# zengyan-97/X2-VLM

Hardware: AMD Instinct MI355X
Metric: image-text pairs/sec (fwd+bwd) X2VLM-base 224px bs=64/GPU (higher is better)
Workload: dtype bf16

## Files before the change

### include/x2vlm_hip.h

```cpp
#ifndef X2VLM_HIP_H
#define X2VLM_HIP_H
#include <stdint.h>
#ifdef __cplusplus
extern "C" {
#endif

const char* x2_last_error(void);
int x2_abi_version(void);
int x2_device_cus(void);
int x2_tune(int key, int value);
int x2_tune_get(int key);

int x2_gemm_nt(const void* A, const void* B, void* C, int M, int N, int K, int lda, int ldb, int ldc,
               const float* bias, const float* gamma, const float* resid, int ldr, void* aux, int ldaux,
               int act, int out_f32, unsigned drop_thr16, unsigned drop_seed, float drop_scale, const unsigned* drop_epoch,
               const float* rowscale, float* colsum, void* stream);

int x2_gemm_nt_dgelu_colparts(const void* A, const void* B, void* C, int M, int N, int K, int lda, int ldb, int ldc,
                              const void* aux, int ldaux, float* colparts, int* nrows_out, void* stream);
int x2_gemm_nt_splitk(const void* A, const void* B, float* C, int M, int N, int K, int lda, int ldb, int ldc,
                      int slices, float* ws, long ws_floats, void* stream);

int x2_gemm_tn_grouped(const int64_t* problems, int count, int accumulate, int split, float* ws, long ws_floats,
                       void* stream);

typedef struct X2AttnArgs {
  const void *Q, *K, *V, *O, *dO;
  void *Out, *dQ, *dK, *dV, *dS;
  float *LSE, *Delta;
  long q_bs, q_rs, k_bs, k_rs, v_bs, v_rs, o_bs, o_rs;
  long dq_bs, dq_rs, dk_bs, dk_rs, dv_bs, dv_rs, do_bs, do_rs;
  int B, Bkv, H, Lq, Lk;
  float scale;
  const float* bias;  int bias_ld;
  const float* biasT; int biasT_ld;
  const float* mask;  int mask_ld;
  const int* kv_idx;
  const int* seq_off; const int* seq_ids;
  int ds_ld;
  unsigned drop_thr16, drop_seed; float drop_scale;
  int dbg;
  int head_dim;
  const unsigned* drop_epoch;
  int grid_nx, grid_ny, grid_nz, grid_map;
  int phase;
  float* ws; long ws_floats;
  float* colsum_ws;
} X2AttnArgs;
int x2_attn_fwd(const X2AttnArgs* args, void* stream);
int x2_attn_bwd(const X2AttnArgs* args, void* stream);
int x2_attn_bwd_one_pass(const X2AttnArgs* args);

int x2_layernorm_fwd(const float* x, const float* w, const float* b, void* y_bf16, float* y_f32, float* mean,
                     float* rstd, int rows, int D, float eps, int period, unsigned drop_thr16, unsigned drop_seed,
                     float drop_scale, const unsigned* drop_epoch, void* stream);
int x2_layernorm_bwd(const void* dy , int dy_is_bf16, const float* x, const float* mean, const float* rstd, const float* w,
                     const float* dres, float* dx, void* dx_bf16, float* dw, float* db, float* dcol, int rows, int D,
                     int period, unsigned in_thr16, unsigned in_seed, float in_scale, unsigned out_thr16,
                     unsigned out_seed, float out_scale, const unsigned* drop_epoch, float* ws ,
                     int defer, int post, const float* post_rowscale, void* stream);
int x2_colsum_bf16(const void* y, float* out, int M, int N, int ld, float* ws , int defer, void* stream);
int x2_reduce_partials(const float* part, int nblk, int nk, int width, float* o0, float* o1, float* o2, void* stream);
int x2_reduce_partials_multi(const int64_t* desc, int count, void* stream);
int x2_layerscale_finish(const int64_t* desc, int count, void* stream);
int x2_rowscale_cast_colsum(const float* dx, const float* rowscale, void* dx_bf16, float* colsum, int M, int D,
                            float* ws , int defer, void* stream);
int x2_cast_bf16(const float* src, void* dst, long n, void* stream);
int x2_cast_transpose_bf16(const float* src, void* dst, void* dstT, int R, int C, int ldt, void* stream);
int x2_cast_transpose_multi(const int64_t* desc, int count, void* stream);
int x2_copy_f32_multi(const int64_t* desc, int count, void* stream);
int x2_patchify(const float* image, void* cols, int B, int R, int ps, void* stream);
int x2_assemble_tokens(const float* patch, const float* cls, float* x, int B, int P, int D, void* stream);
int x2_assemble_tokens_bwd(const float* dx, void* dpatch_bf16, float* dcls, int B, int P, int D, void* stream);
int x2_pool_tokens(float* x, const float* w, int B, int P, int D, int bwd, void* stream);
int x2_relpos_bias(const float* table, const long* index, const long* indexT , float* bias, float* biasT, int N, int H, int ld, int ldT,
                   float scale, void* stream);
int x2_relpos_bias_bwd(const void* dS, const int* inv_off, const int* inv_pos, float* dtable, int B, int N, int H, int ld,
                       int T, float* ws, int slices, void* stream);

int x2_embed_fwd(const long* ids, const float* word, const float* pos, const float* type0, float* out, int R, int L,
                 int D, void* stream);
int x2_embed_bwd(const long* ids, const float* g, float* dword, float* dpos, float* dtype0, int R, int L, int D,
                 float* scratch, void* stream);
int x2_gather_rows(const float* src, const int* idx, float* dst, void* dst_bf16, int R, long len, void* stream);
int x2_scatter_rows(const float* src, const int* idx, float* dst, int R, int D, long len, void* stream);
int x2_linear_f32(const float* A, const float* B, float* C, const float* bias, const float* alpha_ptr, float alpha,
                  int M, int N, int K, long sam, long sak, long sbn, long sbk, long ldc, int accumulate,
                  int ksplit ,
                  float* ws , void* stream);
int x2_l2norm(const float* x, const float* dy, float* out, int R, int D, int bwd, void* stream);
int x2_ce_fwd(const float* logits, long ld, const long* labels, int R, int C, float* lse, float* loss_row, float* out2,
              void* stream);
int x2_ce_bwd(const float* logits, long ld, const long* labels, const float* lse, const float* g, const float* stat,
              float gscale, int R, int C, float* dl_f32, void* dl_bf16, long ldd, void* stream);
int x2_mlm_ce_fwd(const void* X, const void* E, const float* bias, const long* labels, int R, int Vp, int V, int Hd,
                  int ldx, int lde, float* part, float* zlab, void* stream);
int x2_ce_combine(const float* part, int chunks, const float* zlab, const long* labels, int R, float* lse, float* loss_row,
                  float* out2, void* stream);
int x2_mlm_ce_bwd(const void* X, const void* E, const float* bias, const long* labels, const float* lse, const float* g,
                  const float* stat, float gscale, int R, int Vp, int V, int Hd, int ldx, int lde, void* dl_bf16, long ldd,
                  void* stream);
int x2_mask_tokens(const long* text_ids, const long* text_atts, int B, int L, const unsigned char* is_subword, int vocab,
                   const unsigned* words, int words_ld, unsigned seed, const unsigned* epoch, double mask_prob, int max_masks,
                   double skipgram_prb, int skipgram_size, int mask_whole_word, long cls_id, long mask_id, long pad_id, long pad_mask,
                   long* text_ids_masked, long* masked_pos, long* masked_ids, void* stream);
int x2_sample_negatives(const float* sim, int n, const long* group, const float* u, int* out, void* stream);
int x2_additive_mask(const long* atts, float* out, int S, int L, int Lp, float neg, void* stream);

int x2_attn_fwd_mask2d(const X2AttnArgs* args, const float* mask2d, int mask2d_ld, void* stream);
int x2_attn_bwd_mask2d(const X2AttnArgs* args, const float* mask2d, int mask2d_ld, void* stream);
int x2_additive_mask2d(const long* m, float* out, int S, int L, int Lp, float neg, void* stream);
int x2_embed_fwd_pid(const long* ids, const long* pids, const float* word, const float* pos, const float* type0, float* out, int R, int D,
                     void* stream);
int x2_embed_bwd_pid(const long* ids, const long* pids, const float* g, float* dword, float* dpos, float* dtype0, int R, int L, int D,
                     float* scratch, void* stream);
int x2_mlm_ls_fwd(const void* X, const void* E, const float* bias, const long* labels, long ignore, int R, int Vp, int V, int Hd, int ldx,
                  int lde, float* part, float* sumz, float* zlab, float* zign, void* stream);
int x2_ls_combine(const float* part, const float* sumz, int chunks, const float* zlab, const float* zign, const long* labels, const float* w,
                  int R, int V, long ignore, float ls, float* lse, float* kl_row, float* out2, void* stream);
int x2_mlm_ls_bwd(const void* X, const void* E, const float* bias, const long* labels, const float* w, const float* lse, const float* g,
                  const float* stat, float gscale, float ls, long ignore, int R, int Vp, int V, int Hd, int ldx, int lde, void* dl_bf16,
                  long ldd, void* stream);
int x2_kv_csr(const int* kv, int S, int Bi, int* off, int* order, void* stream);
int x2_tail_index(const int* ineg, const int* tneg, const long* text_atts , const long* image_atts , int B, int L,
                  int T, int with_match, int* t_idx, int* kv, long* atts_out , long* enc_out , void* stream);
int x2_droppath_rows(const float* rates, unsigned seed, const unsigned* epoch, int depth, int B, int T, float* out, void* stream);
int x2_frame_mean(const float* x, const float* pos, const float* dy, float* out, float* dpos, int Bc, int F, int T, int D, int bwd,
                  void* stream);
int x2_gelu_f32(const float* x, const float* dy, float* out, long n, void* stream);
int x2_colsum_f32(const float* x, float* out, int M, int N, void* stream);

int x2_grad_norm(const void* table, int ntensors, int nblocks, float max_norm, float* partial, float* out2, void* stream);
int x2_adamw_multi(const void* table, int ntensors, int nblocks, const float* lr, const float* wd, int ngroups, float b1,
                   float b2, float eps, const float* clip2 , void* stream);

int x2_comm_unique_id(void* out128);
int x2_comm_init(const void* id128, int rank, int world, void** comm_out);
int x2_comm_info(void* comm, int* rank, int* world);
int x2_comm_allreduce_bucket(void* comm, void* buf, long count, int dtype, int average, void* done_event, void* stream);
int x2_comm_allgather(void* comm, const void* send, void* recv, long count_per_rank, int dtype, void* done_event, void* stream);
int x2_comm_broadcast(void* comm, void* buf, long count, int dtype, int root, void* done_event, void* stream);
int x2_comm_destroy(void* comm);

#ifdef __cplusplus
}
#endif
#endif
```

### probes/ab_step.py

```python
import argparse, importlib, os, sys, tempfile, time
ROOT = os.path.dirname(os.path.dirname(os.path.abspath(__file__)))
sys.path.insert(0, ROOT)
import torch
import bench

ap = argparse.ArgumentParser()
ap.add_argument("--config", default="base")
ap.add_argument("--variants", nargs="+", default=["default:"])
ap.add_argument("--rounds", type=int, default=3)
ap.add_argument("--steps", type=int, default=20)
ap.add_argument("--warmup", type=int, default=4)
args = ap.parse_args()
conf = bench.CONFIGS[args.config]
mp = importlib.import_module("x2-vlm_amd.model_pretrain")
cfgs = importlib.import_module("x2-vlm_amd.configs")
graph = importlib.import_module("x2-vlm_amd.graph")
lib = importlib.import_module("x2-vlm_amd._lib").lib()
dev = torch.device("cuda", 0)
torch.manual_seed(0)
cfg = cfgs.pretrain_config(tempfile.mkdtemp(), conf["size"], conf["res"])
if conf["frames"]:
    cfg.update(video_encoding="avgpool", frame_len=conf["frames"], add_frame_pos=True)
model = mp.XVLM(config=cfg, load_vision_params=False, load_text_params=False, pretraining=True).to(dev).train()
batch = {k: v.to(dev) for k, v in bench.synthetic_batch(0, conf["batch"], 30, conf["res"], frames=conf["frames"]).items()}
variants = []
for v in args.variants:
    name, _, kv = v.partition(":")
    env = {}
    knobs = {}
    for item in filter(None, kv.split(",")):
        k, val = item.split("=")
        if k.isdigit():
            knobs[int(k)] = int(val)
        else:
            env[k] = val.replace("+", ",")
    variants.append((name, knobs, env))
res = {n: [] for n, _, _ in variants}
for rnd in range(args.rounds):
    for name, knobs, env in variants:
        for k, val in knobs.items():
            assert lib.x2_tune(k, val) == 0, lib.x2_last_error()
        old = {k: os.environ.get(k) for k in env}
        os.environ.update(env)
        step = graph.SegmentedStep(model, batch, warmup=1)
        assert step.mode == "hipgraph-segments", step.error
        for _ in range(args.warmup):
            step()
        torch.cuda.synchronize()
        a, b = torch.cuda.Event(enable_timing=True), torch.cuda.Event(enable_timing=True)
        a.record()
        for _ in range(args.steps):
            step()
        b.record()
        torch.cuda.synchronize()
        res[name].append(a.elapsed_time(b) / args.steps)
        del step
        for k in knobs:
            lib.x2_tune(k, 0)
        for k, v in old.items():
            if v is None:
                os.environ.pop(k, None)
            else:
                os.environ[k] = v
        import gc
        gc.collect()
        torch.cuda.empty_cache()
print("config %s, %d steps per timing, ms per step by round:" % (args.config, args.steps))
for name, knobs, env in variants:
    r = res[name]
    print("  %-12s %-28s %s   min %.3f  mean %.3f" % (name, ",".join("%s=%s" % kv for kv in list(knobs.items()) + list(env.items())) or "-",
                                                       " ".join("%.3f" % x for x in r), min(r), sum(r) / len(r)))
```

### x2-vlm_amd/_lib.py

```python
import ctypes as C
import os

import torch

_HERE = os.path.dirname(os.path.abspath(__file__))
LIB_PATH = os.environ.get("X2VLM_HIP_LIB") or os.path.join(_HERE, "libx2vlm_hip.so")

P, I, L, F, U = C.c_void_p, C.c_int, C.c_long, C.c_float, C.c_uint


class AttnArgs(C.Structure):
    _fields_ = [(n, P) for n in ("Q", "K", "V", "O", "dO", "Out", "dQ", "dK", "dV", "dS", "LSE", "Delta")] + \
               [(n, L) for n in ("q_bs", "q_rs", "k_bs", "k_rs", "v_bs", "v_rs", "o_bs", "o_rs",
                                 "dq_bs", "dq_rs", "dk_bs", "dk_rs", "dv_bs", "dv_rs", "do_bs", "do_rs")] + \
               [(n, I) for n in ("B", "Bkv", "H", "Lq", "Lk")] + [("scale", F)] + \
               [("bias", P), ("bias_ld", I), ("biasT", P), ("biasT_ld", I), ("mask", P), ("mask_ld", I),
                ("kv_idx", P), ("seq_off", P), ("seq_ids", P), ("ds_ld", I),
                ("drop_thr16", C.c_uint), ("drop_seed", C.c_uint), ("drop_scale", F), ("dbg", I), ("head_dim", I), ("drop_epoch", P),
                ("grid_nx", I), ("grid_ny", I), ("grid_nz", I), ("grid_map", I),
                ("phase", I), ("ws", P), ("ws_floats", L), ("colsum_ws", P)]


_SIGS = {
    "x2_gemm_nt": [P, P, P, I, I, I, I, I, I, P, P, P, I, P, I, I, I, U, U, F, P, P, P, P],
    "x2_gemm_nt_splitk": [P, P, P, I, I, I, I, I, I, I, P, L, P],
    "x2_gemm_nt_dgelu_colparts": [P, P, P, I, I, I, I, I, I, P, I, P, C.POINTER(I), P],
    "x2_gemm_tn_grouped": [P, I, I, I, P, L, P],
    "x2_attn_fwd": [C.POINTER(AttnArgs), P],
    "x2_attn_bwd": [C.POINTER(AttnArgs), P],
    "x2_layernorm_fwd": [P, P, P, P, P, P, P, I, I, F, I, U, U, F, P, P],
    "x2_layernorm_bwd": [P, I, P, P, P, P, P, P, P, P, P, P, I, I, I, U, U, F, U, U, F, P, P, I, I, P, P],
    "x2_colsum_bf16": [P, P, I, I, I, P, I, P],
    "x2_reduce_partials": [P, I, I, I, P, P, P, P],
    "x2_reduce_partials_multi": [P, I, P],
    "x2_cast_transpose_multi": [P, I, P],
    "x2_copy_f32_multi": [P, I, P],
    "x2_layerscale_finish": [P, I, P],
    "x2_rowscale_cast_colsum": [P, P, P, P, I, I, P, I, P],
    "x2_cast_bf16": [P, P, L, P],
    "x2_cast_transpose_bf16": [P, P, P, I, I, I, P],
    "x2_patchify": [P, P, I, I, I, P],
    "x2_assemble_tokens": [P, P, P, I, I, I, P],
    "x2_assemble_tokens_bwd": [P, P, P, I, I, I, P],
    "x2_pool_tokens": [P, P, I, I, I, I, P],
    "x2_relpos_bias": [P, P, P, P, P, I, I, I, I, F, P],
    "x2_relpos_bias_bwd": [P, P, P, P, I, I, I, I, I, P, I, P],
    "x2_embed_fwd": [P, P, P, P, P, I, I, I, P],
    "x2_embed_bwd": [P, P, P, P, P, I, I, I, P, P],
    "x2_gather_rows": [P, P, P, P, I, L, P],
    "x2_scatter_rows": [P, P, P, I, I, L, P],
    "x2_linear_f32": [P, P, P, P, P, F, I, I, I, L, L, L, L, L, I, I, P, P],
    "x2_l2norm": [P, P, P, I, I, I, P],
    "x2_ce_fwd": [P, L, P, I, I, P, P, P, P],
    "x2_ce_bwd": [P, L, P, P, P, P, F, I, I, P, P, L, P],
    "x2_mlm_ce_fwd": [P, P, P, P, I, I, I, I, I, I, P, P, P],
    "x2_ce_combine": [P, I, P, P, I, P, P, P, P],
    "x2_mlm_ce_bwd": [P, P, P, P, P, P, P, F, I, I, I, I, I, I, P, L, P],
    "x2_sample_negatives": [P, I, P, P, P, P],
    "x2_mask_tokens": [P, P, I, I, P, I, P, I, U, P, C.c_double, I, C.c_double, I, I, L, L, L, L, P, P, P, P],
    "x2_additive_mask": [P, P, I, I, I, F, P],
    "x2_kv_csr": [P, I, I, P, P, P],
    "x2_tail_index": [P, P, P, P, I, I, I, I, P, P, P, P, P],
    "x2_droppath_rows": [P, U, P, I, I, I, P, P],
    "x2_frame_mean": [P, P, P, P, P, I, I, I, I, I, P],
    "x2_gelu_f32": [P, P, P, L, P],
    "x2_grad_norm": [P, I, I, F, P, P, P],
    "x2_adamw_multi": [P, I, I, P, P, I, F, F, F, P, P],
    "x2_colsum_f32": [P, P, I, I, P],
    "x2_attn_fwd_mask2d": [C.POINTER(AttnArgs), P, I, P],
    "x2_attn_bwd_mask2d": [C.POINTER(AttnArgs), P, I, P],
    "x2_additive_mask2d": [P, P, I, I, I, F, P],
    "x2_embed_fwd_pid": [P, P, P, P, P, P, I, I, P],
    "x2_embed_bwd_pid": [P, P, P, P, P, P, I, I, I, P, P],
    "x2_mlm_ls_fwd": [P, P, P, P, L, I, I, I, I, I, I, P, P, P, P, P],
    "x2_ls_combine": [P, P, I, P, P, P, P, I, I, L, F, P, P, P, P],
    "x2_mlm_ls_bwd": [P, P, P, P, P, P, P, P, F, F, L, I, I, I, I, I, I, P, L, P],
}
_COMM_SIGS = {
    "x2_comm_unique_id": [P],
    "x2_comm_init": [P, I, I, C.POINTER(P)],
    "x2_comm_info": [P, C.POINTER(I), C.POINTER(I)],
    "x2_comm_allreduce_bucket": [P, P, L, I, I, P, P],
    "x2_comm_allgather": [P, P, P, L, I, P, P],
    "x2_comm_broadcast": [P, P, L, I, I, P, P],
    "x2_comm_destroy": [P],
}
EXPORTS = sorted(list(_SIGS) + list(_COMM_SIGS) + ["x2_last_error", "x2_abi_version", "x2_device_cus", "x2_tune", "x2_tune_get",
                                                         "x2_attn_bwd_one_pass"])

_lib = None


class X2HipError(RuntimeError):
    pass


def lib():
    global _lib
    if _lib is None:
        if not os.path.exists(LIB_PATH):
            raise X2HipError("HIP extension %s not built: run `python -c 'import __graft_entry__ as g; g.build()'`"
                             % LIB_PATH)
        try:
            h = C.CDLL(LIB_PATH)
        except OSError as e:
            raise X2HipError("cannot load %s: %s" % (LIB_PATH, e))
        for name, sig in list(_SIGS.items()) + list(_COMM_SIGS.items()):
            fn = getattr(h, name)
            fn.argtypes, fn.restype = sig, I
        h.x2_last_error.restype = C.c_char_p
        h.x2_abi_version.restype = I
        h.x2_device_cus.restype = I
        h.x2_tune.argtypes, h.x2_tune.restype = [I, I], I
        h.x2_tune_get.argtypes, h.x2_tune_get.restype = [I], I
        h.x2_attn_bwd_one_pass.argtypes, h.x2_attn_bwd_one_pass.restype = [C.POINTER(AttnArgs)], I
        for kv in filter(None, os.environ.get("X2_TUNE", "").split(",")):
            k, v = kv.split("=")
            if h.x2_tune(int(k), int(v)) != 0:
                raise X2HipError("X2_TUNE=%s: %s" % (kv, h.x2_last_error().decode()))
        _lib = h
    return _lib


_get_device = torch._C._cuda_getDevice if hasattr(torch._C, "_cuda_getDevice") else None
_get_raw_stream = getattr(torch._C, "_cuda_getCurrentRawStream", None)


def raw_stream():
    return _get_raw_stream(_get_device())


def call(name, *args):
    h = _lib or lib()
    rc = getattr(h, name)(*args, _get_raw_stream(_get_device()))
    if rc != 0:
        raise X2HipError("%s failed (%d): %s" % (name, rc, h.x2_last_error().decode()))


def ptr(t):
    return None if t is None else t.data_ptr()
```

### x2-vlm_amd/csrc/gemm.hip

```cpp
#include "x2_common.h"
#include <type_traits>

#define BM 128
#define BN 128
#define BK 64
#define TILE_BYTES (128 * 128)
#define STAGE_BYTES (2 * TILE_BYTES)
#define GEMM_LDS_BYTES (2 * STAGE_BYTES)

struct GemmNT {
  const bf16_t* A; const bf16_t* B; void* C;
  const float* bias; const float* gamma; const float* resid; bf16_t* aux;
  int M, N, K;
  int lda, ldb, ldc, ldr, ldaux;
  int act;
  int out_f32;
  int group_m;
  DropSpec drop;
  const uint32_t* drop_epoch;
  const float* rowscale;
  float* colsum;
  int dbg;
  int ksplit;
  const long* ce_labels;
  const float* ce_lse;
  const float* ce_g;
  const float* ce_stat;
  float* ce_part;
  float* ce_zlab;
  float ce_gscale;
  int ce_C;
  float* ce_sumz;
  float* ce_zign;
  long ce_ignore;
  float ce_ls;
  const float* ce_w;
};

__device__ __forceinline__ void tile_coords(int t, int tiles_m, int tiles_n, int gm, int& tm, int& tn) {
  const int gsz = gm * tiles_n, g = t / gsz, first = g * gm;
  const int rows = min(gm, tiles_m - first), r = t - g * gsz;
  tm = first + r % rows;
  tn = r / rows;
}

__device__ __forceinline__ void st16(void* p, u32x4 v, bool wt) {
  if (wt) asm volatile("global_store_dwordx4 %0, %1, off sc1\n\ts_nop 1" ::"v"(p), "v"(v) : "memory");
  else *reinterpret_cast<u32x4*>(p) = v;
}

#ifdef X2_PROBE
#define NT_DBG(p, bit) (((p).dbg & (bit)) != 0)
static __device__ unsigned long long* g_nt_probe = nullptr;
#define NT_STAMP(i) do { if (g_nt_probe && threadIdx.x == 0) g_nt_probe[(size_t)blockIdx.x * 4 + (i)] = wall_clock64(); } while (0)
#define NT_ABL_DECL(p) const bool abl_dma_ = NT_DBG(p, 32), abl_rd_ = NT_DBG(p, 64), abl_mm_ = NT_DBG(p, 128); bool rd_ = true
#define NT_ABL_NO_DMA(kt) if (abl_dma_ && (kt) >= 2) return
#define NT_ABL_NO_READ() if (!rd_) return
#define NT_ABL_NO_MFMA() if (abl_mm_) return
#define NT_ABL_STEP(kt) if (abl_rd_ && (kt) > 0) rd_ = false
#else
#define NT_ABL_DECL(p)
#define NT_ABL_NO_DMA(kt)
#define NT_ABL_NO_READ()
#define NT_ABL_NO_MFMA()
#define NT_ABL_STEP(kt)
#define NT_DBG(p, bit) false
#define NT_STAMP(i) do { } while (0)
#endif
typedef __attribute__((ext_vector_type(16))) float f32x16;
template <int TM>
__device__ __forceinline__ void epi_stage_half(f32x4 (&acc)[TM][4], int half, bool full, float* stg, int lane) {
  const int frow = lane & 15, fg = lane >> 4;
#pragma unroll
  for (int ii = 0; ii < 2; ++ii)
#pragma unroll
    for (int j = 0; j < 4; ++j)
      if (full || ii == 0) *reinterpret_cast<f32x4*>(stg + (ii * 16 + frow) * 68 + j * 16 + fg * 4) = acc[full ? half * 2 + ii : half * 2][j];
}
template <int RT>
__device__ __forceinline__ void epi_stage_half(f32x16 (&acc)[RT][2], int half, bool, float* stg, int lane) {
  const int row = lane & 31, h = lane >> 5;
#pragma unroll
  for (int tj = 0; tj < 2; ++tj)
#pragma unroll
    for (int g = 0; g < 4; ++g)
      *reinterpret_cast<f32x4*>(stg + row * 68 + tj * 32 + g * 8 + h * 4) =
          f32x4{acc[half][tj][4 * g], acc[half][tj][4 * g + 1], acc[half][tj][4 * g + 2], acc[half][tj][4 * g + 3]};
}
template <int V> struct EpiTraits {
  static constexpr bool generic = V == 4;
  static constexpr int act = V == 2 ? 1 : (V == 3 || V == 10) ? 2 : 0;
  static constexpr bool out_f32 = V == 1 || V == 5 || V == 6 || V == 7;
  static constexpr bool resid = V == 5 || V == 6;
  static constexpr bool scale = V == 6;
  static constexpr bool aux0 = false;
  static constexpr bool drop = V == 5;
  static constexpr bool colsum = false;
  static constexpr bool colparts = V == 10;
};
template <int TM, int VAR, class Acc>
__device__ __forceinline__ void nt_epilogue(const GemmNT& p, Acc& acc, char* smem, int wave, int lane, int mw0, int nw0, int prow = 0) {
  using E = EpiTraits<VAR>;
  const int act = E::generic ? p.act : E::act;
  const bool out_f32 = E::generic ? p.out_f32 != 0 : E::out_f32;
  const bool has_resid = E::generic ? p.resid != nullptr : E::resid;
  const bool has_scale = E::generic ? (p.gamma != nullptr || p.rowscale != nullptr) : E::scale;
  const bool has_aux0 = E::generic ? (p.act == 0 && p.aux != nullptr) : E::aux0;
  const bool has_drop = (E::generic || E::drop) ? p.drop.thr16 != 0 : false;
  const bool has_colsum = E::generic ? p.colsum != nullptr : (E::colsum && p.colsum != nullptr);
  float* stg = reinterpret_cast<float*>(smem) + wave * (32 * 68);
  const int er = lane >> 3, ec = (lane & 7) * 8;
  const int n = nw0 + ec;
  const bool nok = n < p.N;
  float bb[8], gg[8];
#pragma unroll
  for (int e = 0; e < 8; ++e) { bb[e] = 0.f; gg[e] = 1.f; }
  if (nok && p.bias) { const float4 b0 = *reinterpret_cast<const float4*>(p.bias + n), b1 = *reinterpret_cast<const float4*>(p.bias + n + 4);
    bb[0] = b0.x; bb[1] = b0.y; bb[2] = b0.z; bb[3] = b0.w; bb[4] = b1.x; bb[5] = b1.y; bb[6] = b1.z; bb[7] = b1.w; }
  if (nok && has_scale && p.gamma) { const float4 g0 = *reinterpret_cast<const float4*>(p.gamma + n), g1 = *reinterpret_cast<const float4*>(p.gamma + n + 4);
// ... 26 lines not shown
    }
    epi_stage_half(acc, half, full, stg, lane);
#pragma unroll
    for (int rr = 0; rr < 4; ++rr) {
      if (!full && rr >= 2) continue;
      const int row = rr * 8 + er;
      const int m = mw0 + half * 32 + row;
      const float4 a0 = *reinterpret_cast<const float4*>(stg + row * 68 + ec), a1 = *reinterpret_cast<const float4*>(stg + row * 68 + ec + 4);
      if (m >= p.M || !nok) continue;
      float v[8] = {a0.x + bb[0], a0.y + bb[1], a0.z + bb[2], a0.w + bb[3], a1.x + bb[4], a1.y + bb[5], a1.z + bb[6], a1.w + bb[7]};
      if constexpr (VAR == 8) {
        const long lab = p.ce_labels[m];
        float mx = -INFINITY;
#pragma unroll
        for (int e = 0; e < 8; ++e) mx = n + e < p.ce_C ? fmaxf(mx, v[e]) : mx;
        mx = fmaxf(mx, __shfl_xor(mx, 1, 64)); mx = fmaxf(mx, __shfl_xor(mx, 2, 64)); mx = fmaxf(mx, __shfl_xor(mx, 4, 64));
        float se = 0.f;
#pragma unroll
        for (int e = 0; e < 8; ++e) {
          se += n + e < p.ce_C ? __expf(v[e] - mx) : 0.f;
          if ((long)(n + e) == lab) p.ce_zlab[m] = v[e];
        }
        se += __shfl_xor(se, 1, 64); se += __shfl_xor(se, 2, 64); se += __shfl_xor(se, 4, 64);
        if ((lane & 7) == 0) *reinterpret_cast<float2*>(p.ce_part + ((size_t)m * (p.N >> 6) + (nw0 >> 6)) * 2) = float2{mx, se};
        continue;
      }
      if constexpr (VAR == 11) {
        const long lab = p.ce_labels[m];
        float mx = -INFINITY, sz = 0.f;
#pragma unroll
        for (int e = 0; e < 8; ++e) { mx = n + e < p.ce_C ? fmaxf(mx, v[e]) : mx; sz += n + e < p.ce_C ? v[e] : 0.f; }
        mx = fmaxf(mx, __shfl_xor(mx, 1, 64)); mx = fmaxf(mx, __shfl_xor(mx, 2, 64)); mx = fmaxf(mx, __shfl_xor(mx, 4, 64));
        sz += __shfl_xor(sz, 1, 64); sz += __shfl_xor(sz, 2, 64); sz += __shfl_xor(sz, 4, 64);
        float se = 0.f;
#pragma unroll
        for (int e = 0; e < 8; ++e) {
          se += n + e < p.ce_C ? __expf(v[e] - mx) : 0.f;
          if ((long)(n + e) == lab) p.ce_zlab[m] = v[e];
          if ((long)(n + e) == p.ce_ignore) p.ce_zign[m] = v[e];
        }
        se += __shfl_xor(se, 1, 64); se += __shfl_xor(se, 2, 64); se += __shfl_xor(se, 4, 64);
        if ((lane & 7) == 0) {
          *reinterpret_cast<float2*>(p.ce_part + ((size_t)m * (p.N >> 6) + (nw0 >> 6)) * 2) = float2{mx, se};
          p.ce_sumz[(size_t)m * (p.N >> 6) + (nw0 >> 6)] = sz;
        }
        continue;
      }
      if constexpr (VAR == 12) {
        const long lab = p.ce_labels[m];
        const bool live = lab >= 0 && lab != p.ce_ignore;
        const float conf = 1.f - p.ce_ls, sm = p.ce_ls / (float)(p.ce_C - 2), qsum = conf + sm * (float)(p.ce_C - 2);
        const float sc = live ? p.ce_gscale * p.ce_g[0] * p.ce_w[m] / (p.ce_stat[1] + 1e-5f) : 0.f, l = p.ce_lse[m];
#pragma unroll
        for (int e = 0; e < 8; ++e) {
          const long c = n + e;
          const float q = c == lab ? conf : (c == p.ce_ignore ? 0.f : sm);
          v[e] = c < p.ce_C ? (qsum * __expf(v[e] - l) - q) * sc : 0.f;
        }
        st16(reinterpret_cast<bf16_t*>(p.C) + (size_t)m * p.ldc + n,
             u32x4{pack_bf16(v[0], v[1]), pack_bf16(v[2], v[3]), pack_bf16(v[4], v[5]), pack_bf16(v[6], v[7])}, false);
        continue;
      }
      if constexpr (VAR == 9) {
        const long lab = p.ce_labels[m];
        const float sc = lab >= 0 ? p.ce_gscale * p.ce_g[0] / p.ce_stat[1] : 0.f, l = p.ce_lse[m];
#pragma unroll
        for (int e = 0; e < 8; ++e) v[e] = n + e < p.ce_C ? (__expf(v[e] - l) - ((long)(n + e) == lab ? 1.f : 0.f)) * sc : 0.f;
        st16(reinterpret_cast<bf16_t*>(p.C) + (size_t)m * p.ldc + n,
             u32x4{pack_bf16(v[0], v[1]), pack_bf16(v[2], v[3]), pack_bf16(v[4], v[5]), pack_bf16(v[6], v[7])}, false);
        continue;
      }
      if (act == 1) {
        st16(p.aux + (size_t)m * p.ldaux + n, u32x4{pack_bf16(v[0], v[1]), pack_bf16(v[2], v[3]), pack_bf16(v[4], v[5]), pack_bf16(v[6], v[7])}, wt);
#pragma unroll
        for (int r = 0; r < 8; ++r) v[r] = gelu_f(v[r]);
      } else if (act == 2) {
#pragma unroll
        for (int r = 0; r < 4; ++r) { v[2 * r] *= dgelu_f(bf_lo(pre[rr][r])); v[2 * r + 1] *= dgelu_f(bf_hi(pre[rr][r])); }
      } else if (has_aux0) {
        st16(p.aux + (size_t)m * p.ldaux + n, u32x4{pack_bf16(v[0], v[1]), pack_bf16(v[2], v[3]), pack_bf16(v[4], v[5]), pack_bf16(v[6], v[7])}, wt);
      }
      if (has_drop) {
        float dm[4];
        drop_mul4(drop_, (uint32_t)m * (uint32_t)p.N + (uint32_t)n, dm);
        v[0] *= dm[0]; v[1] *= dm[1]; v[2] *= dm[2]; v[3] *= dm[3];
        drop_mul4(drop_, (uint32_t)m * (uint32_t)p.N + (uint32_t)n + 4u, dm);
        v[4] *= dm[0]; v[5] *= dm[1]; v[6] *= dm[2]; v[7] *= dm[3];
      }
      if (has_scale) {
        const float rs_ = p.rowscale ? p.rowscale[m] : 1.f;
#pragma unroll
        for (int r = 0; r < 8; ++r) v[r] *= gg[r] * rs_;
      }
      if (has_resid) {
        v[0] += r0[rr].x; v[1] += r0[rr].y; v[2] += r0[rr].z; v[3] += r0[rr].w;
        v[4] += r1[rr].x; v[5] += r1[rr].y; v[6] += r1[rr].z; v[7] += r1[rr].w;
      }
      if (has_colsum || E::colparts) {
#pragma unroll
        for (int r = 0; r < 8; ++r) cs[r] += v[r];
      }
      if (out_f32) {
        float* c = reinterpret_cast<float*>(p.C) + (size_t)m * p.ldc + n;
        st16(c, u32x4{__float_as_uint(v[0]), __float_as_uint(v[1]), __float_as_uint(v[2]), __float_as_uint(v[3])}, wt);
        st16(c + 4, u32x4{__float_as_uint(v[4]), __float_as_uint(v[5]), __float_as_uint(v[6]), __float_as_uint(v[7])}, wt);
      } else {
        st16(reinterpret_cast<bf16_t*>(p.C) + (size_t)m * p.ldc + n,
             u32x4{pack_bf16(v[0], v[1]), pack_bf16(v[2], v[3]), pack_bf16(v[4], v[5]), pack_bf16(v[6], v[7])}, wt);
      }
    }
  }
  if constexpr (E::colparts) {
#pragma unroll
    for (int e = 0; e < 8; ++e) { cs[e] += __shfl_xor(cs[e], 8, 64); cs[e] += __shfl_xor(cs[e], 16, 64); cs[e] += __shfl_xor(cs[e], 32, 64); }
    if (er == 0 && nok) {
      float* dst = p.colsum + (size_t)prow * p.N + n;
      *reinterpret_cast<float4*>(dst) = float4{cs[0], cs[1], cs[2], cs[3]};
      *reinterpret_cast<float4*>(dst + 4) = float4{cs[4], cs[5], cs[6], cs[7]};
    }
  }
  if (has_colsum) {
#pragma unroll
    for (int e = 0; e < 8; ++e) { cs[e] += __shfl_xor(cs[e], 8, 64); cs[e] += __shfl_xor(cs[e], 16, 64); cs[e] += __shfl_xor(cs[e], 32, 64); }
    if (er == 0 && nok) {
#pragma unroll
      for (int e = 0; e < 8; ++e) atomicAdd(p.colsum + n + e, cs[e]);
    }
  }
}

template <int TM, int VAR, class Acc>
__device__ __forceinline__ void nt_epilogue_f4(const GemmNT& p, Acc& acc, char* smem, int wave, int lane, int mw0, int nw0) {
  using E = EpiTraits<VAR>;
  static_assert(!E::generic && E::out_f32 && E::act == 0 && VAR <= 6, "nt_epilogue_f4: feature sets 1, 5, 6");
  const bool has_drop = E::drop ? p.drop.thr16 != 0 : false;
  float* stg = reinterpret_cast<float*>(smem) + wave * (32 * 68);
  const int er = lane >> 4, ec = (lane & 15) * 4;
  const int n = nw0 + ec;
  const bool nok = n < p.N;
  float bb[4] = {0.f, 0.f, 0.f, 0.f}, gg[4] = {1.f, 1.f, 1.f, 1.f};
  if (nok && p.bias) { const float4 b0 = *reinterpret_cast<const float4*>(p.bias + n); bb[0] = b0.x; bb[1] = b0.y; bb[2] = b0.z; bb[3] = b0.w; }
  if (E::scale && nok && p.gamma) { const float4 g0 = *reinterpret_cast<const float4*>(p.gamma + n); gg[0] = g0.x; gg[1] = g0.y; gg[2] = g0.z; gg[3] = g0.w; }
  const DropSpec drop_ = drop_at_epoch(p.drop, p.drop_epoch);
#pragma unroll
  for (int half = 0; half < (TM + 1) / 2; ++half) {
    const bool full = half * 2 + 1 < TM;
    float4 rs[4][2];
    const int nc = nok ? n : 0;
    if (E::resid) {
#pragma unroll
      for (int rr = 0; rr < 4; ++rr) {
        if (!full && rr >= 2) continue;
#pragma unroll
        for (int h = 0; h < 2; ++h) {
          const int mc = min(mw0 + half * 32 + rr * 8 + h * 4 + er, p.M - 1);
          rs[rr][h] = *reinterpret_cast<const float4*>(p.resid + (size_t)mc * p.ldr + nc);
        }
      }
    }
    epi_stage_half(acc, half, full, stg, lane);
#pragma unroll
    for (int rr = 0; rr < 4; ++rr) {
      if (!full && rr >= 2) continue;
#pragma unroll
      for (int h = 0; h < 2; ++h) {
        const int row = rr * 8 + h * 4 + er;
        const int m = mw0 + half * 32 + row;
        const float4 a0 = *reinterpret_cast<const float4*>(stg + row * 68 + ec);
        if (m >= p.M || !nok) continue;
        float v[4] = {a0.x + bb[0], a0.y + bb[1], a0.z + bb[2], a0.w + bb[3]};
        if (has_drop) {
          float dm[4];
          drop_mul4(drop_, (uint32_t)m * (uint32_t)p.N + (uint32_t)n, dm);
          v[0] *= dm[0]; v[1] *= dm[1]; v[2] *= dm[2]; v[3] *= dm[3];
        }
        if (E::scale) {
          const float rs_ = p.rowscale ? p.rowscale[m] : 1.f;
#pragma unroll
          for (int r = 0; r < 4; ++r) v[r] *= gg[r] * rs_;
        }
        if (E::resid) { v[0] += rs[rr][h].x; v[1] += rs[rr][h].y; v[2] += rs[rr][h].z; v[3] += rs[rr][h].w; }
        st16(reinterpret_cast<float*>(p.C) + (size_t)m * p.ldc + n,
             u32x4{__float_as_uint(v[0]), __float_as_uint(v[1]), __float_as_uint(v[2]), __float_as_uint(v[3])}, false);
      }
    }
  }
}

template <int TM, int VAR, bool F4 = false>
__global__ __launch_bounds__(256, 2) void gemm_nt_kernel(GemmNT p) {
  constexpr int BMT = 32 * TM;
  if constexpr (VAR == 7) {
    const int koff = blockIdx.y * p.ksplit;
    p.A += koff; p.B += koff;
    p.K = min(p.ksplit, p.K - koff);
    p.C = reinterpret_cast<float*>(p.C) + (size_t)blockIdx.y * p.M * p.ldc;
  }
  constexpr int A_BYTES = BMT * 128, STG = A_BYTES + TILE_BYTES;
  extern __shared__ __attribute__((aligned(16))) char smem[];
  const int tid = threadIdx.x, lane = tid & 63;
  const int wave = __builtin_amdgcn_readfirstlane(tid >> 6);
  const int wm = wave >> 1, wn = wave & 1;
  const int tiles_n = (p.N + BN - 1) / BN, tiles_m = (p.M + BMT - 1) / BMT;
  int tm, tn;
  tile_coords(xcd_remap(blockIdx.x, gridDim.x), tiles_m, tiles_n, p.group_m, tm, tn);
  const int m0 = tm * BMT, n0 = tn * BN;

  const bf16_t* srcA[TM]; const bf16_t* srcB[4];
#pragma unroll
  for (int i = 0; i < TM; ++i) {
    const int q = i * 256 + tid, row = q >> 3, c = (q & 7) ^ (row & 7);
    int ra = m0 + row; ra = ra < p.M ? ra : p.M - 1;
    srcA[i] = p.A + (size_t)ra * p.lda + c * 8;
  }
#pragma unroll
  for (int i = 0; i < 4; ++i) {
    const int q = i * 256 + tid, row = q >> 3, c = (q & 7) ^ (row & 7);
    int rb = n0 + row; rb = rb < p.N ? rb : p.N - 1;
    srcB[i] = p.B + (size_t)rb * p.ldb + c * 8;
  }
  auto stage = [&](int kt, int buf) {
    char* base = smem + buf * STG;
#pragma unroll
    for (int i = 0; i < TM; ++i) glds16(srcA[i] + (size_t)kt * BK, base + (i * 256 + wave * 64) * 16);
#pragma unroll
    for (int i = 0; i < 4; ++i) glds16(srcB[i] + (size_t)kt * BK, base + A_BYTES + (i * 256 + wave * 64) * 16);
  };

  f32x4 acc[TM][4];
#pragma unroll
  for (int i = 0; i < TM; ++i)
#pragma unroll
    for (int j = 0; j < 4; ++j) acc[i][j] = f32x4{0.f, 0.f, 0.f, 0.f};

  const uint32_t lds0 = lds_addr(smem);
  const int frow = lane & 15, fg = lane >> 4, fsw = lane & 7;
  const uint32_t offA = (uint32_t)((wm * 16 * TM + frow) * 128);
  const uint32_t offB = (uint32_t)(A_BYTES + (wn * 64 + frow) * 128);

  const int nk = p.K / BK;
  bf16x8 a0[TM], b0[4], a1[TM], b1[4];
  auto frags = [&](uint32_t sb, int ks, bf16x8 (&a)[TM], bf16x8 (&b)[4]) {
    const uint32_t cs = (uint32_t)(((ks * 4 + fg) ^ fsw) << 4);
#pragma unroll
    for (int j = 0; j < 4; ++j) b[j] = lds_read_b128(sb + offB + j * 2048 + cs);
#pragma unroll
    for (int i = 0; i < TM; ++i) a[i] = lds_read_b128(sb + offA + i * 2048 + cs);
  };
  auto mma = [&](bf16x8 (&a)[TM], bf16x8 (&b)[4], auto first, auto last) {
#pragma unroll
    for (int t = decltype(first)::value; t < decltype(last)::value; ++t)
      acc[t >> 2][t & 3] = __builtin_amdgcn_mfma_f32_16x16x32_bf16(b[t & 3], a[t >> 2], acc[t >> 2][t & 3], 0, 0, 0);
  };
  using I0 = std::integral_constant<int, 0>; using I1 = std::integral_constant<int, 1>; using IN = std::integral_constant<int, 4 * TM>;
  auto step = [&](int kt, auto refill, auto has_next) {
    mma(a0, b0, I0{}, I1{});
// ... 535 lines not shown
extern "C" int x2_tune_get(int key) {
  if (key >= 9 && key <= 15) return g_tune_x[key - 8];
  if (key < 0 || key >= 8) return -1;
  return g_tune[key];
}

static int nt256_plan(int M, int N, double* eff) {
  const int cus = x2_cus(), tiles_n = (N + 255) / 256;
  const double ideal = (double)M * N / (512.0 * 256.0 * cus);
  int best = 8; double best_cost = 1e30;
  for (int t = 8; t >= 5; --t) {
    const long tiles = (long)((M + 32 * t - 1) / (32 * t)) * tiles_n;
    const double cost = (double)((tiles + cus - 1) / cus) * t / 16.0;
    if (cost < best_cost - 1e-9) { best_cost = cost; best = t; }
  }
  if (eff) *eff = ideal / best_cost;
  return best;
}
template <int TMW, int V>
static void launch_nt256(const GemmNT& p, hipStream_t stream) {
  static bool raised = false;
  if (!raised) {
    (void)hipFuncSetAttribute(reinterpret_cast<const void*>(gemm_nt256_kernel<TMW, V>), hipFuncAttributeMaxDynamicSharedMemorySize, N2_LDS_BYTES);
    raised = true;
  }
  const int tiles = ((p.M + 32 * TMW - 1) / (32 * TMW)) * ((p.N + 255) / 256);
  hipLaunchKernelGGL((gemm_nt256_kernel<TMW, V>), dim3(tiles), dim3(512), N2_LDS_BYTES, stream, p);
}
template <int V>
static void launch_nt256s3(const GemmNT& p, hipStream_t stream) {
  static bool raised = false;
  if (!raised) {
    (void)hipFuncSetAttribute(reinterpret_cast<const void*>(gemm_nt256s3_kernel<V, true>), hipFuncAttributeMaxDynamicSharedMemorySize, N3_LDS_BYTES);
    (void)hipFuncSetAttribute(reinterpret_cast<const void*>(gemm_nt256s3_kernel<V, false>), hipFuncAttributeMaxDynamicSharedMemorySize, N3_LDS_BYTES);
    raised = true;
  }
  const int tiles = ((p.M + 159) / 160) * ((p.N + 255) / 256);
  if (g_tune_x[2] == 2) hipLaunchKernelGGL((gemm_nt256s3_kernel<V, false>), dim3(tiles), dim3(512), N3_LDS_BYTES, stream, p);
  else hipLaunchKernelGGL((gemm_nt256s3_kernel<V, true>), dim3(tiles), dim3(512), N3_LDS_BYTES, stream, p);
}
template <int V>
static void launch_nt256_h(const GemmNT& p, int tmw, hipStream_t stream) {
  switch (tmw) {
    case 5: if (g_tune_x[2] == 1) launch_nt256<5, V>(p, stream); else launch_nt256s3<V>(p, stream); break;
    case 6: launch_nt256<6, V>(p, stream); break;
    case 7: launch_nt256<7, V>(p, stream); break;
    default: launch_nt256<8, V>(p, stream); break;
  }
}

template <int RT0, int RT1, int V, int NST>
static void launch_nt_pp(const GemmNT& p, hipStream_t stream) {
  constexpr int lds = NST * ((RT0 + RT1) * 4096 + 2 * PP_BHALF);
  static bool raised = false;
  if (!raised) {
    (void)hipFuncSetAttribute(reinterpret_cast<const void*>(gemm_nt_pp_kernel<RT0, RT1, V, NST>), hipFuncAttributeMaxDynamicSharedMemorySize, lds);
    raised = true;
  }
  constexpr int BMT = 32 * (RT0 + RT1);
  const int tiles = ((p.M + BMT - 1) / BMT) * ((p.N + 255) / 256);
  hipLaunchKernelGGL((gemm_nt_pp_kernel<RT0, RT1, V, NST>), dim3(tiles), dim3(512), lds, stream, p);
}
template <int V>
static void launch_nt_pp_h(const GemmNT& p, int h, hipStream_t stream) {
  switch (h) {
    case 3: launch_nt_pp<1, 2, V, 3>(p, stream); break;
    case 4: if (g_tune_x[2] == 1) launch_nt_pp<2, 2, V, 2>(p, stream); else launch_nt_pp<2, 2, V, 3>(p, stream); break;
    case 5: if (g_tune_x[2] == 1) launch_nt_pp<2, 3, V, 2>(p, stream); else launch_nt_pp<2, 3, V, 3>(p, stream); break;
    default: launch_nt_pp<3, 3, V, 2>(p, stream); break;
  }
}

template <int TM, int V, bool F4>
static void launch_nt(const GemmNT& p, int tiles, hipStream_t stream) {
  constexpr int lds = 2 * (32 * TM * 128 + TILE_BYTES);
  static bool raised = false;
  if (lds > 65536 && !raised) {
    (void)hipFuncSetAttribute(reinterpret_cast<const void*>(gemm_nt_kernel<TM, V, F4>), hipFuncAttributeMaxDynamicSharedMemorySize, lds);
    raised = true;
  }
  hipLaunchKernelGGL((gemm_nt_kernel<TM, V, F4>), dim3(tiles), dim3(256), lds, stream, p);
}

extern "C" int x2_gemm_nt(const void* A, const void* B, void* C, int M, int N, int K, int lda, int ldb, int ldc,
                          const float* bias, const float* gamma, const float* resid, int ldr, void* aux, int ldaux,
                          int act, int out_f32, unsigned drop_thr16, unsigned drop_seed, float drop_scale, const unsigned* drop_epoch,
                          const float* rowscale, float* colsum, void* stream) {
  X2_REQUIRE(M > 0 && N > 0 && K > 0, "x2_gemm_nt: empty problem M=%d N=%d K=%d", M, N, K);
  X2_REQUIRE(drop_thr16 < 65536u, "x2_gemm_nt: drop_thr16=%u", drop_thr16);
  X2_REQUIRE(K % BK == 0, "x2_gemm_nt: K=%d must be a multiple of %d", K, BK);
  X2_REQUIRE(N % 8 == 0, "x2_gemm_nt: N=%d must be a multiple of 8", N);
  X2_REQUIRE(lda % 8 == 0 && ldb % 8 == 0 && ldc % 8 == 0, "x2_gemm_nt: leading dims must keep 16-byte rows");
  X2_REQUIRE(act == 0 || aux, "x2_gemm_nt: act=%d needs aux", act);
  X2_REQUIRE((!resid || ldr % 4 == 0) && (!aux || ldaux % 8 == 0), "x2_gemm_nt: ldr/ldaux alignment");
  GemmNT p{(const bf16_t*)A, (const bf16_t*)B, C, bias, gamma, resid, (bf16_t*)aux, M, N, K, lda, ldb, ldc, ldr, ldaux, act, out_f32,
           g_tune[0] > 0 ? g_tune[0] : 8, DropSpec{drop_thr16, drop_seed, drop_scale}, drop_epoch, rowscale, colsum, g_tune[2], 0};
  int var = 4;
  {
    const bool plain = !gamma && !rowscale && !drop_thr16 && !colsum;
    if (g_tune[6] == 1) var = 4;
    else if (act == 1 && !out_f32 && !resid && plain) var = 2;
    else if (act == 2 && !out_f32 && !resid && plain) var = 3;
    else if (act == 0 && !aux && !resid && plain) var = out_f32 ? 1 : 0;
    else if (act == 0 && !aux && resid && out_f32 && !gamma && !rowscale && !colsum) var = 5;
    else if (act == 0 && !aux && resid && out_f32 && gamma && !drop_thr16 && !colsum) var = 6;
  }
  double eff256 = 0.0;
  int tmw = nt256_plan(M, N, &eff256);
  if (g_tune[3] >= 5 && g_tune[3] <= 8) tmw = g_tune[3];
  const bool light = var == 0 || var == 1;
  bool auto256 = (light || K >= 2048) && eff256 * 100.0 >= (g_tune_x[1] > 0 ? g_tune_x[1] : 80) && !(resid && M < 8192);
  if (g_tune_x[3] != 1) {
    if ((var == 5 || var == 6) && M >= 8192 && eff256 * 100.0 >= (g_tune_x[1] > 0 ? g_tune_x[1] : 80)) auto256 = true;
    if (var == 2 && eff256 * 100.0 >= 90.0) auto256 = true;
  }
  const bool use256 = var != 4 && N % 8 == 0 && (g_tune[1] == 3 || ((g_tune[1] == 0 || g_tune[1] == 4) && g_tune[3] == 0 && auto256));
  const bool pp_ok = var != 4 && ((size_t)(M - 1) * lda + K) * 2 < (1ull << 31) && ((size_t)(N - 1) * ldb + K) * 2 < (1ull << 31);
  int pp_h = 0;
  if (g_tune_x[7] >= 3 && g_tune_x[7] <= 6) pp_h = g_tune_x[7];
  else if (g_tune_x[7] == 0 && g_tune[1] == 0 && g_tune[3] == 0 && !use256 && K >= 2048 && (var == 0 || var == 1 || var == 5)) {
    const int cus = x2_cus(), tn256 = (N + 255) / 256;
    for (int h = 3; h <= 4 && !pp_h; ++h) {
      const int tiles = ((M + 32 * h - 1) / (32 * h)) * tn256;
      if (tiles <= cus && tiles * 10 >= cus * 7) pp_h = h;
    }
  }
  if (pp_ok && pp_h) {
    switch (var) {
      case 0: launch_nt_pp_h<0>(p, pp_h, (hipStream_t)stream); break;
      case 1: launch_nt_pp_h<1>(p, pp_h, (hipStream_t)stream); break;
      case 2: launch_nt_pp_h<2>(p, pp_h, (hipStream_t)stream); break;
      case 3: launch_nt_pp_h<3>(p, pp_h, (hipStream_t)stream); break;
      case 5: launch_nt_pp_h<5>(p, pp_h, (hipStream_t)stream); break;
      default: launch_nt_pp_h<6>(p, pp_h, (hipStream_t)stream); break;
    }
    return x2_check_launch("x2_gemm_nt");
  }
  if (use256) {
    switch (var) {
      case 0: launch_nt256_h<0>(p, tmw, (hipStream_t)stream); break;
      case 1: launch_nt256_h<1>(p, tmw, (hipStream_t)stream); break;
      case 2: launch_nt256_h<2>(p, tmw, (hipStream_t)stream); break;
      case 3: launch_nt256_h<3>(p, tmw, (hipStream_t)stream); break;
      case 5: launch_nt256_h<5>(p, tmw, (hipStream_t)stream); break;
      default: launch_nt256_h<6>(p, tmw, (hipStream_t)stream); break;
    }
  } else {
    const int t128 = ((M + 127) / 128) * ((N + BN - 1) / BN), t192 = ((M + 191) / 192) * ((N + BN - 1) / BN);
    const int t64 = ((M + 63) / 64) * ((N + BN - 1) / BN);
    const int slots = 2 * x2_cus();
    const bool use64 = g_tune[3] == 3 || (g_tune[3] == 0 && (t128 <= slots || (t128 <= slots + slots / 6 && K <= 1024)));
    const bool use192 = !use64 && (g_tune[3] == 2 || (g_tune[3] == 0 && t128 > slots && t192 <= slots));
    const int t160 = ((M + 159) / 160) * ((N + BN - 1) / BN);
    const bool use160 = g_tune[3] == 4 || (use192 && g_tune[3] == 0 && g_tune[7] != 1 && t160 <= slots);
#define X2_NT_LAUNCH(V, SW)                                                                          \
    do {                                                                                              \
      if (use64) launch_nt<2, V, SW>(p, t64, (hipStream_t)stream);                                    \
      else if (use160) launch_nt<5, V, SW>(p, t160, (hipStream_t)stream);                             \
      else if (use192) launch_nt<6, V, SW>(p, t192, (hipStream_t)stream);                             \
      else launch_nt<4, V, SW>(p, t128, (hipStream_t)stream);                                         \
    } while (0)
    switch (var) {
      case 0: X2_NT_LAUNCH(0, false); break;
      case 2: X2_NT_LAUNCH(2, false); break;
      case 3: X2_NT_LAUNCH(3, false); break;
      case 1: X2_NT_LAUNCH(1, true); break;
      case 5: X2_NT_LAUNCH(5, true); break;
      case 6: X2_NT_LAUNCH(6, true); break;
      default: X2_NT_LAUNCH(4, false); break;
    }
#undef X2_NT_LAUNCH
  }
  return x2_check_launch("x2_gemm_nt");
}

extern "C" int x2_gemm_nt_dgelu_colparts(const void* A, const void* B, void* C, int M, int N, int K, int lda, int ldb, int ldc,
                                         const void* aux, int ldaux, float* colparts, int* nrows_out, void* stream) {
  X2_REQUIRE(A && B && C && aux && colparts && nrows_out, "x2_gemm_nt_dgelu_colparts: null argument");
  X2_REQUIRE(M > 0 && N > 0 && K > 0 && K % BK == 0 && N % 8 == 0, "x2_gemm_nt_dgelu_colparts: M=%d N=%d K=%d", M, N, K);
// ... 474 lines not shown
```

### x2-vlm_amd/csrc/heads.hip

```cpp
#include "x2_common.h"
#define SCATTER_MAX_R_E 8192

__global__ __launch_bounds__(256) void embed_fwd_kernel(const long* __restrict__ ids, const float* __restrict__ word,
                                                        const float* __restrict__ pos, const float* __restrict__ type0,
                                                        float* __restrict__ out, int R, int L, int D) {
  const int r = blockIdx.x;
  const long id = ids[r];
  const int l = r % L;
  for (int d = threadIdx.x * 4; d < D; d += 1024) {
    const float4 a = *reinterpret_cast<const float4*>(word + id * D + d), b = *reinterpret_cast<const float4*>(pos + (long)l * D + d),
                 c = *reinterpret_cast<const float4*>(type0 + d);
    *reinterpret_cast<float4*>(out + (long)r * D + d) = float4{a.x + b.x + c.x, a.y + b.y + c.y, a.z + b.z + c.z, a.w + b.w + c.w};
  }
}
extern "C" int x2_embed_fwd(const long* ids, const float* word, const float* pos, const float* type0, float* out, int R, int L, int D,
                            void* stream) {
  X2_REQUIRE(R > 0 && L > 0 && D % 4 == 0, "x2_embed_fwd: R=%d L=%d D=%d", R, L, D);
  hipLaunchKernelGGL(embed_fwd_kernel, dim3(R), dim3(256), 0, (hipStream_t)stream, ids, word, pos, type0, out, R, L, D);
  return x2_check_launch("x2_embed_fwd");
}
__global__ __launch_bounds__(1024) void embed_bwd_word_kernel(const long* __restrict__ ids, const float* __restrict__ g, float* dword, int R,
                                                              int D) {
  __shared__ uint32_t bm[SCATTER_MAX_R_E / 32];
  __shared__ uint16_t lst[SCATTER_MAX_R_E];
// ... 351 lines not shown
    float tot = 0.f;
    for (int c = 0; c < n; ++c) tot += w[c];
    const float t = u[b] * tot;
    float cum = 0.f; int pick = -1;
    for (int c = 0; c < n; ++c) { cum += w[c]; if (w[c] > 0.f && cum > t) { pick = c; break; } }
    if (pick < 0) for (int c = n - 1; c >= 0; --c) if (w[c] > 0.f) { pick = c; break; }
    out[b] = pick < 0 ? b : pick;
  }
}
extern "C" int x2_sample_negatives(const float* sim, int n, const long* group, const float* u, int* out, void* stream) {
  X2_REQUIRE(n > 1 && n <= 1024, "x2_sample_negatives: n=%d not in (1,1024]", n);
  hipLaunchKernelGGL(sample_negatives_kernel, dim3(n), dim3(256), 0, (hipStream_t)stream, sim, n, group, u, out);
  return x2_check_launch("x2_sample_negatives");
}

__global__ __launch_bounds__(256) void additive_mask_kernel(const long* __restrict__ atts, float* __restrict__ out, int S, int L, int Lp, float neg) {
  const long e = blockIdx.x * 256L + threadIdx.x;
  if (e >= (long)S * Lp) return;
  const int s_ = (int)(e / Lp), l = (int)(e % Lp);
  out[e] = l < L ? (1.0f - (float)atts[(long)s_ * L + l]) * neg : 0.f;
}
extern "C" int x2_additive_mask(const long* atts, float* out, int S, int L, int Lp, float neg, void* stream) {
  X2_REQUIRE(atts && out && S > 0 && L > 0 && Lp >= L, "x2_additive_mask: S=%d L=%d Lp=%d", S, L, Lp);
  hipLaunchKernelGGL(additive_mask_kernel, dim3((unsigned)(((long)S * Lp + 255) / 256)), dim3(256), 0, (hipStream_t)stream, atts, out, S, L, Lp, neg);
  return x2_check_launch("x2_additive_mask");
}
__global__ __launch_bounds__(256) void kv_csr_kernel(const int* __restrict__ kv, int S, int Bi, int* __restrict__ off, int* __restrict__ order) {
  extern __shared__ int cnt[];
  __shared__ int part[256];
  for (int b = threadIdx.x; b <= Bi; b += 256) cnt[b] = 0;
  __syncthreads();
  for (int e = threadIdx.x; e < S; e += 256) atomicAdd(&cnt[kv[e]], 1);
  __syncthreads();
  const int per = (Bi + 255) / 256, b0 = threadIdx.x * per, b1 = min(Bi, b0 + per);
  int sum = 0;
  for (int b = b0; b < b1; ++b) sum += cnt[b];
  part[threadIdx.x] = sum;
  __syncthreads();
  if (threadIdx.x == 0) { int run = 0; for (int t = 0; t < 256; ++t) { const int v = part[t]; part[t] = run; run += v; } }
  __syncthreads();
  int run = part[threadIdx.x];
  for (int b = b0; b < b1; ++b) { const int v = cnt[b]; cnt[b] = run; run += v; }
  __syncthreads();
  if (threadIdx.x == 0) cnt[Bi] = S;
  __syncthreads();
  for (int b = threadIdx.x; b <= Bi; b += 256) off[b] = cnt[b];
  for (int b = threadIdx.x; b < Bi; b += 256) {
    int pos = cnt[b];
    const int end = cnt[b + 1];
    for (int e = 0; e < S && pos < end; ++e) if (kv[e] == b) order[pos++] = e;
  }
}
extern "C" int x2_kv_csr(const int* kv, int S, int Bi, int* off, int* order, void* stream) {
  X2_REQUIRE(kv && off && order && S > 0 && Bi > 0 && Bi <= 8192, "x2_kv_csr: S=%d Bi=%d (Bi <= 8192)", S, Bi);
  hipLaunchKernelGGL(kv_csr_kernel, dim3(1), dim3(256), (size_t)(Bi + 1) * sizeof(int), (hipStream_t)stream, kv, S, Bi, off, order);
  return x2_check_launch("x2_kv_csr");
}

__global__ __launch_bounds__(256) void gelu_f32_kernel(const float* __restrict__ x, const float* __restrict__ dy, float* out, long n) {
  const long i = blockIdx.x * 256L + threadIdx.x;
  if (i < n) out[i] = dy ? dy[i] * dgelu_f(x[i]) : gelu_f(x[i]);
}
extern "C" int x2_gelu_f32(const float* x, const float* dy, float* out, long n, void* stream) {
  X2_REQUIRE(n > 0, "x2_gelu_f32: n=%ld", n);
  hipLaunchKernelGGL(gelu_f32_kernel, dim3((int)((n + 255) / 256)), dim3(256), 0, (hipStream_t)stream, x, dy, out, n);
  return x2_check_launch("x2_gelu_f32");
}
__global__ __launch_bounds__(256) void colsum_f32_kernel(const float* __restrict__ x, float* out, int M, int N) {
  const int n = blockIdx.x * 256 + threadIdx.x;
  if (n >= N) return;
  float s = 0.f;
  for (int m = 0; m < M; ++m) s += x[(long)m * N + n];
  out[n] += s;
}
extern "C" int x2_colsum_f32(const float* x, float* out, int M, int N, void* stream) {
  X2_REQUIRE(M > 0 && N > 0, "x2_colsum_f32: M=%d N=%d", M, N);
  hipLaunchKernelGGL(colsum_f32_kernel, dim3((N + 255) / 256), dim3(256), 0, (hipStream_t)stream, x, out, M, N);
  return x2_check_launch("x2_colsum_f32");
}

__global__ __launch_bounds__(256) void tail_index_kernel(const int* __restrict__ ineg, const int* __restrict__ tneg,
                                                         const long* __restrict__ text_atts, const long* __restrict__ image_atts, int B, int L,
                                                         int T, int with_match, int* __restrict__ t_idx, int* __restrict__ kv,
                                                         long* __restrict__ atts_out, long* __restrict__ enc_out) {
  const int r = blockIdx.x, q = with_match ? r / B : 3, b = r % B;
  const int ti = q == 2 ? tneg[b] : (q == 3 ? B + b : b), ki = q == 1 ? ineg[b] : b;
  if (threadIdx.x == 0) { t_idx[r] = ti; kv[r] = ki; }
  const long* ta = text_atts + (long)(ti % B) * L;
  for (int l = threadIdx.x; l < L; l += 256) atts_out[(long)r * L + l] = ta[l];
  const long* ia = image_atts + (long)ki * T;
  for (int t = threadIdx.x; t < T; t += 256) enc_out[(long)r * T + t] = ia[t];
}
extern "C" int x2_tail_index(const int* ineg, const int* tneg, const long* text_atts, const long* image_atts, int B, int L, int T,
                             int with_match, int* t_idx, int* kv, long* atts_out, long* enc_out, void* stream) {
  X2_REQUIRE(text_atts && image_atts && t_idx && kv && atts_out && enc_out && B > 0 && L > 0 && T > 0, "x2_tail_index: B=%d L=%d T=%d", B, L, T);
  X2_REQUIRE(!with_match || (ineg && tneg), "x2_tail_index: with_match needs the negative indices");
  hipLaunchKernelGGL(tail_index_kernel, dim3(with_match ? 4 * B : B), dim3(256), 0, (hipStream_t)stream, ineg, tneg, text_atts, image_atts, B, L, T,
                     with_match, t_idx, kv, atts_out, enc_out);
  return x2_check_launch("x2_tail_index");
}

__global__ __launch_bounds__(256) void droppath_rows_kernel(const float* __restrict__ rates, uint32_t seed, const uint32_t* __restrict__ epoch,
                                                            int depth, int B, int T, float* __restrict__ out) {
  const long e = blockIdx.x * 256L + threadIdx.x, rows = (long)B * T;
  if (e >= 2L * depth * rows) return;
  const int lb = (int)(e / rows), b = (int)((e % rows) / T), l = lb >> 1;
  uint32_t s_ = seed;
  if (epoch) s_ = x2_hash(s_ + 0x9E3779B1u * epoch[0]);
  const uint32_t h = x2_hash(((uint32_t)lb * (uint32_t)B + (uint32_t)b) ^ s_);
  const float rate = rates[l], u = (float)(h >> 8) * (1.0f / 16777216.0f);
  out[e] = u >= rate ? 1.0f / (1.0f - rate) : 0.0f;
}
extern "C" int x2_droppath_rows(const float* rates, unsigned seed, const unsigned* epoch, int depth, int B, int T, float* out, void* stream) {
  X2_REQUIRE(rates && out && depth > 0 && B > 0 && T > 0, "x2_droppath_rows: depth=%d B=%d T=%d", depth, B, T);
  const long n = 2L * depth * B * T;
  hipLaunchKernelGGL(droppath_rows_kernel, dim3((unsigned)((n + 255) / 256)), dim3(256), 0, (hipStream_t)stream, rates, seed, epoch, depth, B, T, out);
  return x2_check_launch("x2_droppath_rows");
}

__global__ __launch_bounds__(256) void frame_mean_fwd_kernel(const float* __restrict__ x, const float* __restrict__ pos, float* __restrict__ out,
                                                             int Bc, int F, long TD, int D) {
  const long e = (blockIdx.x * 256L + threadIdx.x) * 4;
  if (e >= (long)Bc * TD) return;
  const long b = e / TD, o = e % TD;
  const int d = (int)(o % D);
  float4 a = float4{0.f, 0.f, 0.f, 0.f};
  for (int f = 0; f < F; ++f) {
    const float4 v = *reinterpret_cast<const float4*>(x + (b * F + f) * TD + o);
    float4 pp = float4{0.f, 0.f, 0.f, 0.f};
    if (pos) pp = *reinterpret_cast<const float4*>(pos + (long)f * D + d);
    a.x += v.x + pp.x; a.y += v.y + pp.y; a.z += v.z + pp.z; a.w += v.w + pp.w;
  }
  const float inv = 1.0f / (float)F;
  *reinterpret_cast<float4*>(out + e) = float4{a.x * inv, a.y * inv, a.z * inv, a.w * inv};
}
__global__ __launch_bounds__(256) void frame_mean_bwd_kernel(const float* __restrict__ dy, float* __restrict__ dx, int Bc, int F, long TD) {
  const long e = (blockIdx.x * 256L + threadIdx.x) * 4;
  if (e >= (long)Bc * TD) return;
  const long b = e / TD, o = e % TD;
  const float inv = 1.0f / (float)F;
  float4 g = *reinterpret_cast<const float4*>(dy + e);
  g.x *= inv; g.y *= inv; g.z *= inv; g.w *= inv;
  for (int f = 0; f < F; ++f) *reinterpret_cast<float4*>(dx + (b * F + f) * TD + o) = g;
}
__global__ __launch_bounds__(256) void frame_pos_grad_kernel(const float* __restrict__ dy, float* __restrict__ dpos, long rows, int D, int F) {
  __shared__ float sh[4][64];
  const int c = blockIdx.x * 64 + (threadIdx.x & 63), sl = threadIdx.x >> 6;
  float s = 0.f;
  if (c < D) for (long r = sl; r < rows; r += 4) s += dy[r * D + c];
  sh[sl][threadIdx.x & 63] = s;
  __syncthreads();
  if (sl == 0 && c < D) {
    const float v = (sh[0][threadIdx.x] + sh[1][threadIdx.x] + sh[2][threadIdx.x] + sh[3][threadIdx.x]) / (float)F;
    for (int f = 0; f < F; ++f) dpos[(long)f * D + c] = v;
  }
}
extern "C" int x2_frame_mean(const float* x, const float* pos, const float* dy, float* out, float* dpos, int Bc, int F, int T, int D, int bwd,
                             void* stream) {
  X2_REQUIRE(Bc > 0 && F > 0 && T > 0 && D > 0 && D % 4 == 0, "x2_frame_mean: Bc=%d F=%d T=%d D=%d", Bc, F, T, D);
  const long TD = (long)T * D, n4 = (long)Bc * TD / 4;
  if (!bwd) {
    X2_REQUIRE(x && out, "x2_frame_mean: forward needs x and out");
    hipLaunchKernelGGL(frame_mean_fwd_kernel, dim3((unsigned)((n4 + 255) / 256)), dim3(256), 0, (hipStream_t)stream, x, pos, out, Bc, F, TD, D);
  } else {
    X2_REQUIRE(dy && out, "x2_frame_mean: backward needs dy and out (= dx)");
    hipLaunchKernelGGL(frame_mean_bwd_kernel, dim3((unsigned)((n4 + 255) / 256)), dim3(256), 0, (hipStream_t)stream, dy, out, Bc, F, TD);
    if (dpos) hipLaunchKernelGGL(frame_pos_grad_kernel, dim3((D + 63) / 64), dim3(256), 0, (hipStream_t)stream, dy, dpos, (long)Bc * T, D, F);
  }
  return x2_check_launch("x2_frame_mean");
}

__global__ __launch_bounds__(256) void embed_fwd_pid_kernel(const long* __restrict__ ids, const long* __restrict__ pids, const float* __restrict__ word,
                                                            const float* __restrict__ pos, const float* __restrict__ type0, float* __restrict__ out, int D) {
  const int r = blockIdx.x;
  const long id = ids[r], l = pids[r];
  for (int d = threadIdx.x * 4; d < D; d += 1024) {
    const float4 a = *reinterpret_cast<const float4*>(word + id * D + d), b = *reinterpret_cast<const float4*>(pos + l * D + d),
                 c = *reinterpret_cast<const float4*>(type0 + d);
    *reinterpret_cast<float4*>(out + (long)r * D + d) = float4{a.x + b.x + c.x, a.y + b.y + c.y, a.z + b.z + c.z, a.w + b.w + c.w};
  }
}
extern "C" int x2_embed_fwd_pid(const long* ids, const long* pids, const float* word, const float* pos, const float* type0, float* out, int R, int D,
// ... 93 lines not shown
```

### x2-vlm_amd/csrc/rowwise.hip

```cpp
#include "x2_common.h"

__device__ __forceinline__ long remap_row(int r, int period) { return period > 0 ? (long)r + r / period + 1 : r; }

#define LN_MAXV 8
#define LN_DISPATCH(D, CALL) do { const int nv_ = ((D) + 255) / 256; \
  if (nv_ <= 1) { CALL(1); } else if (nv_ == 2) { CALL(2); } else if (nv_ == 3) { CALL(3); } else if (nv_ == 4) { CALL(4); } \
  else if (nv_ <= 6) { CALL(6); } else { CALL(8); } } while (0)
template <int NV>
__global__ __launch_bounds__(256) void layernorm_fwd_kernel(const float* __restrict__ x, const float* __restrict__ w,
                                                            const float* __restrict__ bsh, bf16_t* yb, float* yf,
                                                            float* mean, float* rstd, int rows, int D, float eps, int period,
                                                            DropSpec drop_in_, const uint32_t* __restrict__ epoch) {
  const int row = blockIdx.x * 4 + (threadIdx.x >> 6), lane = threadIdx.x & 63;
  if (row >= rows) return;
  const DropSpec drop = drop_at_epoch(drop_in_, epoch);
  const long gr = remap_row(row, period);
  const float* xr = x + gr * D;
  float4 v[NV];
  float s = 0.f;
  const int nv = D >> 2;
#pragma unroll
  for (int i = 0; i < NV; ++i) {
    const int c = lane + i * 64;
    if (c < nv) { v[i] = *reinterpret_cast<const float4*>(xr + c * 4); s += v[i].x + v[i].y + v[i].z + v[i].w; }
// ... 122 lines not shown
}
extern "C" int x2_reduce_partials(const float* part, int nblk, int nk, int width, float* o0, float* o1, float* o2, void* stream) {
  X2_REQUIRE(part && nblk > 0 && nk >= 1 && nk <= 3 && width > 0, "x2_reduce_partials: nblk=%d nk=%d width=%d", nblk, nk, width);
  launch_reduce(part, nblk, nk, width, o0, o1, o2, (hipStream_t)stream);
  return x2_check_launch("x2_reduce_partials");
}

#define RPM_MAX 16
struct ReduceDesc { const float* part; float* o[4]; int nblk, nk, width, blk0; };
struct ReduceGroup { ReduceDesc d[RPM_MAX]; int count; };
#define RPM_COLS 16
__global__ __launch_bounds__(256) void reduce_partials_multi_kernel(ReduceGroup g) {
  int e = 0;
#pragma unroll
  for (int i = 1; i < RPM_MAX; ++i) if (i < g.count && (int)blockIdx.x >= g.d[i].blk0) e = i;
  const ReduceDesc d = g.d[e];
  const int local = blockIdx.x - d.blk0, ctiles = (d.width + RPM_COLS - 1) / RPM_COLS;
  const int k = local / ctiles, cg = threadIdx.x & 3, sl = threadIdx.x >> 2;
  const int c = (local % ctiles) * RPM_COLS + cg * 4;
  __shared__ float4 red[63][4];
  float4 s = float4{0.f, 0.f, 0.f, 0.f};
  float* o = d.o[k];
  const bool vec = (d.width & 3) == 0;
  if (o && c < d.width) {
    const float* base = d.part + (size_t)k * d.width + c;
    const size_t rs = (size_t)d.nk * d.width;
    if (vec) {
      int b = sl;
      for (; b + 192 < d.nblk; b += 256) {
        const float4 v0 = *reinterpret_cast<const float4*>(base + (size_t)b * rs), v1 = *reinterpret_cast<const float4*>(base + (size_t)(b + 64) * rs),
                     v2 = *reinterpret_cast<const float4*>(base + (size_t)(b + 128) * rs), v3 = *reinterpret_cast<const float4*>(base + (size_t)(b + 192) * rs);
        s.x += (v0.x + v1.x) + (v2.x + v3.x); s.y += (v0.y + v1.y) + (v2.y + v3.y);
        s.z += (v0.z + v1.z) + (v2.z + v3.z); s.w += (v0.w + v1.w) + (v2.w + v3.w);
      }
      for (; b < d.nblk; b += 64) {
        const float4 v = *reinterpret_cast<const float4*>(base + (size_t)b * rs);
        s.x += v.x; s.y += v.y; s.z += v.z; s.w += v.w;
      }
    } else {
      for (int b = sl; b < d.nblk; b += 64) {
        const float* r = base + (size_t)b * rs;
        s.x += r[0]; if (c + 1 < d.width) s.y += r[1]; if (c + 2 < d.width) s.z += r[2]; if (c + 3 < d.width) s.w += r[3];
      }
    }
  }
  if (sl > 0) red[sl - 1][cg] = s;
  __syncthreads();
  if (sl == 0 && o && c < d.width) {
#pragma unroll 9
    for (int i = 0; i < 63; ++i) { const float4 v = red[i][cg]; s.x += v.x; s.y += v.y; s.z += v.z; s.w += v.w; }
    o[c] += s.x;
    if (c + 1 < d.width) o[c + 1] += s.y;
    if (c + 2 < d.width) o[c + 2] += s.z;
    if (c + 3 < d.width) o[c + 3] += s.w;
  }
}
extern "C" int x2_reduce_partials_multi(const int64_t* desc, int count, void* stream) {
  X2_REQUIRE(desc && count >= 1, "x2_reduce_partials_multi: count=%d", count);
  for (int i0 = 0; i0 < count; i0 += RPM_MAX) {
    ReduceGroup g; g.count = count - i0 < RPM_MAX ? count - i0 : RPM_MAX;
    int blocks = 0;
    for (int i = 0; i < g.count; ++i) {
      const int64_t* q = desc + (size_t)(i0 + i) * 8;
      ReduceDesc& d = g.d[i];
      d.part = (const float*)q[0]; d.nblk = (int)q[1]; d.nk = (int)q[2]; d.width = (int)q[3];
      d.o[0] = (float*)q[4]; d.o[1] = (float*)q[5]; d.o[2] = (float*)q[6]; d.o[3] = (float*)q[7];
      X2_REQUIRE(d.part && d.nblk > 0 && d.nk >= 1 && d.nk <= 4 && d.width > 0, "x2_reduce_partials_multi[%d]: nblk=%d nk=%d width=%d",
                 i0 + i, d.nblk, d.nk, d.width);
      d.blk0 = blocks;
      blocks += ((d.width + RPM_COLS - 1) / RPM_COLS) * d.nk;
    }
    hipLaunchKernelGGL(reduce_partials_multi_kernel, dim3(blocks), dim3(256), 0, (hipStream_t)stream, g);
  }
  return x2_check_launch("x2_reduce_partials_multi");
}

#define LNB_ROWS 16
template <int NV, int MODE>
__global__ __launch_bounds__(256, NV <= 3 ? 4 : 1) void layernorm_bwd_kernel(const void* __restrict__ dy_, const float* __restrict__ x,
                                                            const float* __restrict__ mean, const float* __restrict__ rstd,
                                                            const float* __restrict__ w, const float* dres, float* dx, bf16_t* dxb,
                                                            float* ws, int rows, int D, int period,
                                                            DropSpec din_, DropSpec dout_, const uint32_t* __restrict__ epoch,
                                                            const float* __restrict__ post_rs) {
  constexpr int NSET = 3;
  constexpr bool DYB = MODE != 0;
  extern __shared__ __attribute__((aligned(16))) float red[];
  const DropSpec din = drop_at_epoch(din_, epoch), dout = drop_at_epoch(dout_, epoch);
  const int lane = threadIdx.x & 63, wv = threadIdx.x >> 6;
  const int nv = D >> 2;
  float4 ww[NV], aw[NV], ab[NV], ac[NV];
#pragma unroll
  for (int i = 0; i < NV; ++i) {
    const int c = lane + i * 64;
    ww[i] = c < nv ? *reinterpret_cast<const float4*>(w + c * 4) : float4{0.f, 0.f, 0.f, 0.f};
    aw[i] = float4{0.f, 0.f, 0.f, 0.f}; ab[i] = float4{0.f, 0.f, 0.f, 0.f}; ac[i] = float4{0.f, 0.f, 0.f, 0.f};
  }
  const int r0 = blockIdx.x * LNB_ROWS, r1 = min(rows, r0 + LNB_ROWS);
  for (int row = r0 + wv; row < r1; row += 4) {
    const long gr = remap_row(row, period);
    const float mu = mean[row], rs = rstd[row];
    float4 g[NV], xh[NV];
    float s1 = 0.f, s2 = 0.f;
#pragma unroll
    for (int i = 0; i < NV; ++i) {
      const int c = lane + i * 64;
      if (c < nv) {
        float4 d;
        if constexpr (DYB) {
          const u32x2 raw = *reinterpret_cast<const u32x2*>(reinterpret_cast<const bf16_t*>(dy_) + gr * D + c * 4);
          d = float4{bf_lo(raw.x), bf_hi(raw.x), bf_lo(raw.y), bf_hi(raw.y)};
        } else {
          d = *reinterpret_cast<const float4*>(reinterpret_cast<const float*>(dy_) + gr * D + c * 4);
        }
        const float4 xv = *reinterpret_cast<const float4*>(x + gr * D + c * 4);
        if (din.thr16) {
          float dm[4];
          drop_mul4(din, (uint32_t)gr * (uint32_t)D + (uint32_t)(c * 4), dm);
          d.x *= dm[0]; d.y *= dm[1]; d.z *= dm[2]; d.w *= dm[3];
        }
        xh[i] = float4{(xv.x - mu) * rs, (xv.y - mu) * rs, (xv.z - mu) * rs, (xv.w - mu) * rs};
        g[i] = float4{d.x * ww[i].x, d.y * ww[i].y, d.z * ww[i].z, d.w * ww[i].w};
        s1 += g[i].x + g[i].y + g[i].z + g[i].w;
        s2 += g[i].x * xh[i].x + g[i].y * xh[i].y + g[i].z * xh[i].z + g[i].w * xh[i].w;
        aw[i].x += d.x * xh[i].x; aw[i].y += d.y * xh[i].y; aw[i].z += d.z * xh[i].z; aw[i].w += d.w * xh[i].w;
        ab[i].x += d.x; ab[i].y += d.y; ab[i].z += d.z; ab[i].w += d.w;
      }
    }
    const float m1 = wave_sum(s1) / D, m2 = wave_sum(s2) / D;
#pragma unroll
    for (int i = 0; i < NV; ++i) {
      const int c = lane + i * 64;
      if (c < nv) {
        float4 o{rs * (g[i].x - m1 - xh[i].x * m2), rs * (g[i].y - m1 - xh[i].y * m2), rs * (g[i].z - m1 - xh[i].z * m2), rs * (g[i].w - m1 - xh[i].w * m2)};
        float4 om = o;
        if (dout.thr16) {
          float dm[4];
          drop_mul4(dout, (uint32_t)gr * (uint32_t)D + (uint32_t)(c * 4), dm);
          om.x *= dm[0]; om.y *= dm[1]; om.z *= dm[2]; om.w *= dm[3];
        }
        if (dres) { const float4 rr = *reinterpret_cast<const float4*>(dres + gr * D + c * 4); o.x += rr.x; o.y += rr.y; o.z += rr.z; o.w += rr.w; }
        if (dx) *reinterpret_cast<float4*>(dx + gr * D + c * 4) = o;
        if constexpr (MODE == 2) { om = o; if (post_rs) { const float f = post_rs[gr]; om.x *= f; om.y *= f; om.z *= f; om.w *= f; } }
        ac[i].x += om.x; ac[i].y += om.y; ac[i].z += om.z; ac[i].w += om.w;
        if (dxb) *reinterpret_cast<u32x2*>(dxb + gr * D + c * 4) = u32x2{pack_bf16(om.x, om.y), pack_bf16(om.z, om.w)};
      }
    }
  }
  if (wv > 0) {
#pragma unroll
    for (int i = 0; i < NV; ++i) {
      const int c = lane + i * 64;
      if (c < nv) {
        *reinterpret_cast<float4*>(red + ((0 * 3 + wv - 1) * D) + c * 4) = aw[i];
        *reinterpret_cast<float4*>(red + ((1 * 3 + wv - 1) * D) + c * 4) = ab[i];
        *reinterpret_cast<float4*>(red + ((2 * 3 + wv - 1) * D) + c * 4) = ac[i];
      }
    }
  }
  __syncthreads();
  if (wv == 0) {
#pragma unroll
    for (int i = 0; i < NV; ++i) {
      const int c = lane + i * 64;
      if (c < nv) {
#pragma unroll
        for (int k = 0; k < 3; ++k) {
          const float4 a = *reinterpret_cast<const float4*>(red + ((0 * 3 + k) * D) + c * 4), b = *reinterpret_cast<const float4*>(red + ((1 * 3 + k) * D) + c * 4),
                       cc = *reinterpret_cast<const float4*>(red + ((2 * 3 + k) * D) + c * 4);
          aw[i].x += a.x; aw[i].y += a.y; aw[i].z += a.z; aw[i].w += a.w;
          ab[i].x += b.x; ab[i].y += b.y; ab[i].z += b.z; ab[i].w += b.w;
          ac[i].x += cc.x; ac[i].y += cc.y; ac[i].z += cc.z; ac[i].w += cc.w;
        }
        float* wp = ws + (long)blockIdx.x * NSET * D + c * 4;
        *reinterpret_cast<float4*>(wp) = aw[i];
        *reinterpret_cast<float4*>(wp + D) = ab[i];
        *reinterpret_cast<float4*>(wp + 2 * D) = ac[i];
      }
    }
  }
}

extern "C" int x2_layernorm_bwd(const void* dy, int dy_is_bf16, const float* x, const float* mean, const float* rstd, const float* w,
                                const float* dres, float* dx, void* dx_bf16, float* dw, float* db, float* dcol, int rows, int D,
                                int period, unsigned in_thr16, unsigned in_seed, float in_scale, unsigned out_thr16,
                                unsigned out_seed, float out_scale, const unsigned* drop_epoch, float* ws, int defer, int post,
                                const float* post_rowscale, void* stream) {
  X2_REQUIRE(rows > 0 && D > 0 && D % 4 == 0 && D <= 256 * LN_MAXV, "x2_layernorm_bwd: rows=%d D=%d", rows, D);
  X2_REQUIRE(dw && db && ws, "x2_layernorm_bwd: dw/db and the workspace ws[ceil(rows/%d)*3*D] are required", LNB_ROWS);
  X2_REQUIRE(post || !(dcol && dres), "x2_layernorm_bwd: dcol sums the LN-input gradient, which excludes dres (post = 0)");
  X2_REQUIRE(!(out_thr16 && dres), "x2_layernorm_bwd: an output mask applies to the bf16 copy, which excludes dres");
  X2_REQUIRE(!post || (dy_is_bf16 && dx_bf16 && dcol && !out_thr16 && period == 0),
             "x2_layernorm_bwd: post = 1 (by-products of the final output) takes a bf16 dy, dx_bf16 and dcol, no output mask, period 0");
#define X2_LNB_T(NV, B) hipLaunchKernelGGL((layernorm_bwd_kernel<NV, B>), dim3((rows + LNB_ROWS - 1) / LNB_ROWS), dim3(256), 9 * D * sizeof(float), \
                     (hipStream_t)stream, dy, x, mean, rstd, w, dres, dx, (bf16_t*)dx_bf16, ws, rows, D, period,                \
                     DropSpec{in_thr16, in_seed, in_scale}, DropSpec{out_thr16, out_seed, out_scale}, drop_epoch, post_rowscale)
#define X2_LNB(NV) do { if (post) X2_LNB_T(NV, 2); else if (dy_is_bf16) X2_LNB_T(NV, 1); else X2_LNB_T(NV, 0); } while (0)
  LN_DISPATCH(D, X2_LNB);
  if (!defer) launch_reduce(ws, (rows + LNB_ROWS - 1) / LNB_ROWS, 3, D, dw, db, dcol, (hipStream_t)stream);
  return x2_check_launch("x2_layernorm_bwd");
}

#define CS_ROWS 64
__global__ __launch_bounds__(256) void colsum_bf16_kernel(const bf16_t* __restrict__ y, float* ws, int M, int N, int ld) {
  __shared__ float red[3][512];
  const int tx = threadIdx.x & 63, ty = threadIdx.x >> 6;
  const int c0 = blockIdx.y * 512 + tx * 8;
  const int r0 = blockIdx.x * CS_ROWS, r1 = min(M, r0 + CS_ROWS);
  float acc[8] = {0.f, 0.f, 0.f, 0.f, 0.f, 0.f, 0.f, 0.f};
  if (c0 < N) {
#pragma unroll 4
    for (int r = r0 + ty; r < r1; r += 4) {
      const u32x4 v = *reinterpret_cast<const u32x4*>(y + (long)r * ld + c0);
#pragma unroll
      for (int e = 0; e < 4; ++e) { acc[2 * e] += bf_lo(v[e]); acc[2 * e + 1] += bf_hi(v[e]); }
    }
  }
  if (ty > 0) {
#pragma unroll
    for (int e = 0; e < 8; ++e) red[ty - 1][tx * 8 + e] = acc[e];
  }
  __syncthreads();
  if (ty == 0 && c0 < N) {
#pragma unroll
    for (int e = 0; e < 8; ++e) {
      const float v = acc[e] + red[0][tx * 8 + e] + red[1][tx * 8 + e] + red[2][tx * 8 + e];
      if (c0 + e < N) ws[(long)blockIdx.x * N + c0 + e] = v;
    }
  }
}
extern "C" int x2_colsum_bf16(const void* y, float* out, int M, int N, int ld, float* ws, int defer, void* stream) {
  X2_REQUIRE(M > 0 && N > 0 && N % 8 == 0 && ld % 8 == 0, "x2_colsum_bf16: M=%d N=%d ld=%d (N, ld multiples of 8)", M, N, ld);
  X2_REQUIRE(ws, "x2_colsum_bf16: workspace ws[ceil(M/%d)*N] required", CS_ROWS);
  hipLaunchKernelGGL(colsum_bf16_kernel, dim3((M + CS_ROWS - 1) / CS_ROWS, (N + 511) / 512), dim3(256), 0, (hipStream_t)stream,
                     (const bf16_t*)y, ws, M, N, ld);
  if (!defer) launch_reduce(ws, (M + CS_ROWS - 1) / CS_ROWS, 1, N, out, nullptr, nullptr, (hipStream_t)stream);
  return x2_check_launch("x2_colsum_bf16");
}

#define LS_ROWS 32
__global__ __launch_bounds__(256) void rowscale_cast_colsum_kernel(const float* __restrict__ dx, const float* __restrict__ rowscale,
                                                                   bf16_t* dxb, float* ws, int M, int D) {
  __shared__ float red[3][256];
  const int tx = threadIdx.x & 63, ty = threadIdx.x >> 6;
  const int c0 = blockIdx.y * 256 + tx * 4;
  const int r0 = blockIdx.x * LS_ROWS, r1 = min(M, r0 + LS_ROWS);
  float ab[4] = {0.f, 0.f, 0.f, 0.f};
  if (c0 < D) {
#pragma unroll 4
    for (int r = r0 + ty; r < r1; r += 4) {
      float4 d = *reinterpret_cast<const float4*>(dx + (long)r * D + c0);
      if (rowscale) { const float rs_ = rowscale[r]; d.x *= rs_; d.y *= rs_; d.z *= rs_; d.w *= rs_; }
      *reinterpret_cast<u32x2*>(dxb + (long)r * D + c0) = u32x2{pack_bf16(d.x, d.y), pack_bf16(d.z, d.w)};
      ab[0] += d.x; ab[1] += d.y; ab[2] += d.z; ab[3] += d.w;
    }
  }
  if (ty > 0) {
#pragma unroll
    for (int e = 0; e < 4; ++e) red[ty - 1][tx * 4 + e] = ab[e];
  }
  __syncthreads();
  if (ty == 0 && c0 < D) {
#pragma unroll
    for (int e = 0; e < 4; ++e) ws[(long)blockIdx.x * D + c0 + e] = ab[e] + red[0][tx * 4 + e] + red[1][tx * 4 + e] + red[2][tx * 4 + e];
  }
}
extern "C" int x2_rowscale_cast_colsum(const float* dx, const float* rowscale, void* dx_bf16, float* colsum, int M, int D, float* ws,
                                       int defer, void* stream) {
  X2_REQUIRE(dx && dx_bf16 && colsum && M > 0 && D > 0 && D % 4 == 0 && ws,
             "x2_rowscale_cast_colsum: M=%d D=%d (workspace ws[ceil(M/%d)*D] required)", M, D, LS_ROWS);
  hipLaunchKernelGGL(rowscale_cast_colsum_kernel, dim3((M + LS_ROWS - 1) / LS_ROWS, (D + 255) / 256), dim3(256), 0, (hipStream_t)stream, dx,
                     rowscale, (bf16_t*)dx_bf16, ws, M, D);
  if (!defer) launch_reduce(ws, (M + LS_ROWS - 1) / LS_ROWS, 1, D, colsum, nullptr, nullptr, (hipStream_t)stream);
  return x2_check_launch("x2_rowscale_cast_colsum");
}

#define LSF_MAX 8
struct LsfDesc { float* G; const float* W; const float* bias; const float* gamma; const float* cs; float* dgamma; float* dbias; int N, K, blk0; };
struct LsfGroup { LsfDesc d[LSF_MAX]; int count; };
// ... 410 lines not shown
```

### x2-vlm_amd/engine.py

```python
import itertools
import math
import os
import weakref

import torch

from . import kernels as K
from ._lib import raw_stream

BF16, F32 = torch.bfloat16, torch.float32



_SERIAL = itertools.count(1)


def _tok(w):
    t = w.__dict__.get("_x2_serial")
    if t is None:
        t = w.__dict__["_x2_serial"] = next(_SERIAL)
    return t


class TScale:
# ... 68 lines not shown
        if not todo:
            return
        total = sum(2 * t[3] * t[4] for t in todo)
        flat = torch.empty(total, device=todo[0][2][0].device, dtype=BF16)
        desc, o = [], 0
        for key, vers, ws, R, C_, sc, own in todo:
            plain = flat[o:o + R * C_].view(R, C_)
            tr = flat[o + R * C_:o + 2 * R * C_].view(C_, R)
            o += 2 * R * C_
            roff = 0
            for w in ws:
                desc.append((w.data_ptr(), plain.data_ptr(), tr.data_ptr(), w.shape[0], C_, R, roff, 0 if sc is None else sc.data_ptr()))
                roff += w.shape[0]
            self._c[key] = (vers, (plain, tr), tuple(weakref.ref(w) for w in own))
        K.cast_transpose_multi(desc)

    def prepare_vectors(self, groups):
        self._maybe_expire()
        todo, total = [], 0
        for items in groups:
            key = ("vec",) + tuple(it if isinstance(it, int) else _tok(it) for it in items)
            vers = tuple(0 if isinstance(it, int) else (it._version, it.data_ptr()) for it in items)
            ent = self._c.get(key)
            if ent is not None and ent[0] == vers:
                continue
            if any(not isinstance(it, int) and (it.dtype != F32 or not it.is_contiguous()) for it in items):
                continue
            n = sum(it if isinstance(it, int) else it.numel() for it in items)
            todo.append((key, vers, items, n))
            total += (n + 3) // 4 * 4
        if not todo:
            return
        dev = next(it for _, _, items, _ in todo for it in items if not isinstance(it, int)).device
        flat = torch.empty(total, device=dev, dtype=F32)
        desc, o = [], 0
        for key, vers, items, n in todo:
            out = flat[o:o + n]
            oo = o
            for it in items:
                m = it if isinstance(it, int) else it.numel()
                desc.append((0 if isinstance(it, int) else it.data_ptr(), flat.data_ptr() + 4 * oo, m))
                oo += m
            o += (n + 3) // 4 * 4
            self._c[key] = (vers, out, tuple(weakref.ref(it) for it in items if not isinstance(it, int)))
        K.copy_f32_multi(desc)

    def vector(self, *items):
        self._maybe_expire()
        key = ("vec",) + tuple(it if isinstance(it, int) else _tok(it) for it in items)
        vers = tuple(0 if isinstance(it, int) else (it._version, it.data_ptr()) for it in items)

        ent = self._c.get(key)
        if ent is None or ent[0] != vers:
            tens = [it for it in items if not isinstance(it, int)]
            if tens[0].is_cuda and all(it.dtype == F32 and it.is_contiguous() for it in tens):
                self.prepare_vectors([items])
                ent = self._c[key]
            else:
                dev = next(it for it in items if not isinstance(it, int)).device
                val = torch.cat([torch.zeros(it, device=dev, dtype=F32) if isinstance(it, int) else it.detach().reshape(-1).to(F32) for it in items])
                ent = self._c[key] = (vers, val, tuple(weakref.ref(it) for it in items if not isinstance(it, int)))
        return ent[1]

    def vocab(self, w):
        self._maybe_expire()

        def build():
            V, Hd = w.shape
            Vp = K.round_up(V, 64)
            src = torch.zeros(Vp, Hd, device=w.device, dtype=F32)
            src[:V] = w.detach()
            return K.cast_transpose_bf16(src)
        return self._get(("vocab", _tok(w)), (w._version, w.data_ptr()), build, (w,))

    def invalidate(self):
        self._c.clear()
        self.backward_seen = False


BANK = WeightBank()
SPLIT_DECODER_DGRAD = os.environ.get("X2_SPLIT_DECODER_DGRAD", "1") == "1"
FUSED_MLM_CE = os.environ.get("X2_FUSED_MLM_CE", "1") == "1"
FUSE_DGELU_COLSUM = os.environ.get("X2_FUSE_DGELU_COLSUM", "1") == "1"
KEEP_MLM_LOGITS = False
TIE_WORD_GRAD = False
_TIED_DWORD = {}


class Grads:

    def __init__(self, device, spec, key=None, params=(), zero=True):
        self.params = list(params)
        spec = [s for s in spec if s[2]] + [s for s in spec if not s[2]]
        offs, o = [], 0
        for _, shape, _z in spec:
            offs.append(o)
            o += (int(torch.Size(shape).numel()) + 3) // 4 * 4
        self.nzero = sum((int(torch.Size(sh).numel()) + 3) // 4 * 4 for _, sh, z in spec if z)
        self.flat = torch.empty(o, device=device, dtype=F32)
        if zero and self.nzero:
            self.flat[:self.nzero].zero_()
        self.g = {n: self.flat[of:of + torch.Size(sh).numel()].view(sh) for (n, sh, _z), of in zip(spec, offs)}
        self.key = key

    @staticmethod
    def zero_all(arenas, extra=()):
        desc = [(0, g.flat.data_ptr(), g.nzero) for g in arenas if g.nzero] + [(0, t.data_ptr(), t.numel()) for t in extra]
        if not desc:
            return
        if arenas[0].flat.is_cuda if arenas else extra[0].is_cuda:
            K.copy_f32_multi(desc)
        else:
            for g in arenas:
                g.flat[:g.nzero].zero_()
            for t in extra:
                t.zero_()

    def __getitem__(self, name):
        return self.g[name]

    def alias(self, name, view):
        self.g[name] = view

    def publish(self, also_after=None):
        if GRAD_READY_HOOK is not None:
            GRAD_READY_HOOK(self.flat, self.key, also_after, self.params)

    def take(self, names):
        return [self.g.pop(n) for n in names]


class SideStream:

    def __init__(self):
        self.streams = {}
        self.held = {}
        self.enabled = True
        self.only_from = None

    @property
    def stream(self):
        key = raw_stream()
        if key not in self.streams:
            self.streams[key] = torch.cuda.Stream()
        return self.streams[key]

    def launch(self, fn, tensors):
        if not self.enabled or not torch.cuda.is_available() or (self.only_from is not None and raw_stream() != self.only_from):
            fn()
            return None
        side = self.stream
        ev = torch.cuda.Event()
        ev.record()
        side.wait_event(ev)
        done = torch.cuda.Event()
        with torch.cuda.stream(side):
            fn()
            done.record()
        self.held.setdefault(raw_stream(), []).append(tensors)
        return done

    def join(self):
        if self.enabled and torch.cuda.is_available():
            key = raw_stream()
            if key in self.streams and (self.only_from is None or key == self.only_from):
                torch.cuda.current_stream().wait_stream(self.streams[key])
# ... 320 lines not shown
            K.colsum_bf16(dpatch, Gs["patch_embed.proj.bias"])
            K.gemm_tn_grouped([(dpatch, ctx.cols, Gs["patch_embed.proj.weight"].view(D, -1))], accumulate=True,
                              split=8 if B * P_ >= 4096 else 1)
            SIDE.join()
            Gs.publish()
            out.update(Gs.g)
            return (None, None) + tuple(out[n] for n in names)
        SIDE.join()
        return (dx.view(B, T, D), None) + tuple(out[n] for n in names)



_ATT = ("self.query.weight", "self.query.bias", "self.key.weight", "self.key.bias", "self.value.weight", "self.value.bias",
        "output.dense.weight", "output.dense.bias", "output.LayerNorm.weight", "output.LayerNorm.bias")
_FFN = ("intermediate.dense.weight", "intermediate.dense.bias", "output.dense.weight", "output.dense.bias",
        "output.LayerNorm.weight", "output.LayerNorm.bias")


def bert_layer_param_names(lo, hi, fusion_at, with_cross):
    names = []
    for i in range(lo, hi):
        b = "layer.%d." % i
        names += [b + "attention." + s for s in _ATT]
        if with_cross and i >= fusion_at:
            names += [b + "crossattention." + s for s in _ATT]
        names += [b + s for s in _FFN]
    return names


class BertLayersFn(torch.autograd.Function):

    @staticmethod
    def prepare_weights(p, lo, hi, fusion_at, cross):
        groups, vecs = [], []
        for i in range(lo, hi):
            b = "layer.%d." % i
            a, c = b + "attention.", b + "crossattention."
            groups += [(p[a + "self.query.weight"], p[a + "self.key.weight"], p[a + "self.value.weight"]),
                       (p[a + "output.dense.weight"],), (p[b + "intermediate.dense.weight"],), (p[b + "output.dense.weight"],)]
            vecs.append((p[a + "self.query.bias"], p[a + "self.key.bias"], p[a + "self.value.bias"]))
            if cross and i >= fusion_at:
                groups += [(p[c + "self.query.weight"],), (p[c + "self.key.weight"], p[c + "self.value.weight"]),
                           (p[c + "output.dense.weight"],)]
                vecs.append((p[c + "self.key.bias"], p[c + "self.value.bias"]))
        BANK.prepare(groups)
        BANK.prepare_vectors(vecs)

    @staticmethod
    def _drop(meta, layer, kind):
        d = meta.get("drop")
        if not d:
            return K.NO_DROP
        return K.dropout_spec(d["p_attn"] if kind in (0, 2) else d["p_hidden"], d["seed"], 8 * layer + kind)

    @staticmethod
    def forward(ctx, hidden, enc, meta, *params):
        cross = enc is not None
        names = bert_layer_param_names(meta["lo"], meta["hi"], meta["fusion_at"], cross)
        p = dict(zip(names, params))
        S, L, Hd = hidden.shape
        H, eps = meta["heads"], meta["eps"]
        M = S * L
        assert Hd == 64 * H, "hidden size %d / %d heads: the attention kernels are built for head dim 64" % (Hd, H)
        scale = 1.0 / math.sqrt(Hd // H)
        dev = hidden.device
        h = hidden.contiguous().view(M, Hd)
        hb = K.cast_bf16(h)
        encb = None
        if cross:
            Bi, T, Dv = enc.shape
            encb = K.cast_bf16(enc.contiguous().view(Bi * T, Dv))
        BertLayersFn.prepare_weights(p, meta["lo"], meta["hi"], meta["fusion_at"], cross)
        saved = []
        kv_ahead = {}
        use_aux = cross and AUX.enabled and not (AUX.auto and K.attn_bwd_form(L, enc.shape[1], shared_kv=meta.get("seq_off") is not None,
                                                                               dropout=BertLayersFn._drop(meta, meta["hi"] - 1, 2)[0] != 0) == 2)
        if use_aux:
            for i in range(max(meta["lo"], meta["fusion_at"]), meta["hi"]):
                c = "layer.%d.crossattention." % i
                wkv, _ = BANK.linear(p[c + "self.key.weight"], p[c + "self.value.weight"])
                bkv = BANK.vector(p[c + "self.key.bias"], p[c + "self.value.bias"])
                kv = torch.empty(Bi * T, wkv.shape[0], device=dev, dtype=BF16)
                kv_ahead[i] = (kv, AUX.launch(lambda kv=kv, wkv=wkv, bkv=bkv: K.gemm_nt(encb, wkv, bias=bkv, out=kv), [encb, wkv, bkv, kv]))
        for i in range(meta["lo"], meta["hi"]):
            b = "layer.%d." % i
            a = b + "attention."
            wqkv, _ = BANK.linear(p[a + "self.query.weight"], p[a + "self.key.weight"], p[a + "self.value.weight"])
            bqkv = BANK.vector(p[a + "self.query.bias"], p[a + "self.key.bias"], p[a + "self.value.bias"])
            qkv = K.gemm_nt(hb, wqkv, bias=bqkv)
            att = torch.empty(M, Hd, device=dev, dtype=BF16)
            lse = torch.empty(S * H * L, device=dev, dtype=F32)
            dr = BertLayersFn._drop
            if meta.get("self_mask2d") is not None:
                K.attn_fwd_mask2d(K.view3(qkv, S, L, 0), K.view3(qkv, S, L, Hd), K.view3(qkv, S, L, 2 * Hd), S, H, L, scale,
                                  K.view3(att, S, L), lse, meta["self_mask2d"], drop=dr(meta, i, 0))
            else:
                K.attn_fwd(K.view3(qkv, S, L, 0), K.view3(qkv, S, L, Hd), K.view3(qkv, S, L, 2 * Hd), S, S, H, L, L, scale,
                           K.view3(att, S, L), lse, mask=meta["self_mask"], drop=dr(meta, i, 0))
            wo, _ = BANK.linear(p[a + "output.dense.weight"])
            s1 = K.gemm_nt(att, wo, bias=p[a + "output.dense.bias"], resid=h, out_dtype=F32, drop=dr(meta, i, 1))
            h1b, h1, m1, r1 = K.layernorm_fwd(s1, p[a + "output.LayerNorm.weight"], p[a + "output.LayerNorm.bias"], eps, want_f32=True)
            cr = None
            h2b, h2 = h1b, h1
            if cross and i >= meta["fusion_at"]:
                c = b + "crossattention."
                wq, _ = BANK.linear(p[c + "self.query.weight"])
                wkv, _ = BANK.linear(p[c + "self.key.weight"], p[c + "self.value.weight"])
                bkv = BANK.vector(p[c + "self.key.bias"], p[c + "self.value.bias"])
                q2 = K.gemm_nt(h1b, wq, bias=p[c + "self.query.bias"])
                if i in kv_ahead:
                    kv, ev = kv_ahead.pop(i)
                    if ev is not None:
                        torch.cuda.current_stream().wait_event(ev)
                else:
                    kv = K.gemm_nt(encb, wkv, bias=bkv)
                att2 = torch.empty(M, Hd, device=dev, dtype=BF16)
                lse2 = torch.empty(S * H * L, device=dev, dtype=F32)
                K.attn_fwd(K.view3(q2, S, L), K.view3(kv, Bi, T, 0), K.view3(kv, Bi, T, Hd), S, Bi, H, L, T, scale,
                           K.view3(att2, S, L), lse2, mask=meta["enc_mask"], kv_idx=meta["kv_idx"], seq_off=meta.get("seq_off"),
                           seq_ids=meta.get("seq_ids"), drop=dr(meta, i, 2))
                wo2, _ = BANK.linear(p[c + "output.dense.weight"])
                s2 = K.gemm_nt(att2, wo2, bias=p[c + "output.dense.bias"], resid=h1, out_dtype=F32, drop=dr(meta, i, 3))
                h2b, h2, m2, r2 = K.layernorm_fwd(s2, p[c + "output.LayerNorm.weight"], p[c + "output.LayerNorm.bias"], eps, want_f32=True)
                cr = (q2, kv, att2, lse2, s2, m2, r2)
            wi, _ = BANK.linear(p[b + "intermediate.dense.weight"])
            wout, _ = BANK.linear(p[b + "output.dense.weight"])
            pre = torch.empty(M, wi.shape[0], device=dev, dtype=BF16)
            act = K.gemm_nt(h2b, wi, bias=p[b + "intermediate.dense.bias"], aux=pre, act=1)
            s3 = K.gemm_nt(act, wout, bias=p[b + "output.dense.bias"], resid=h2, out_dtype=F32, drop=dr(meta, i, 4))
            h3b, h3, m3, r3 = K.layernorm_fwd(s3, p[b + "output.LayerNorm.weight"], p[b + "output.LayerNorm.bias"], eps, want_f32=True)
            saved.append((hb, qkv, att, lse, s1, m1, r1, h1b, cr, h2b, pre, act, s3, m3, r3))
            h, hb = h3, h3b
        AUX.join()
        for i in range(meta["lo"], meta["hi"]):
            _count_call(("bert", id(p["layer.%d.attention.self.query.weight" % i])))
        ctx.meta, ctx.saved, ctx.params, ctx.encb = meta, saved, params, encb
        ctx.dims = (S, L, Hd, H, M, scale, cross, enc.shape if cross else None)
        return h.view(S, L, Hd)

    @staticmethod
    def backward(ctx, dh_out):
        meta, params, encb = ctx.meta, ctx.params, ctx.encb
        BANK.note_backward()
        S, L, Hd, H, M, scale, cross, enc_shape = ctx.dims
        names = bert_layer_param_names(meta["lo"], meta["hi"], meta["fusion_at"], cross)
        p = dict(zip(names, params))
        dev = dh_out.device
        dh = dh_out.contiguous().view(M, Hd)
        denc = None
        out = {}
        if cross:
            Bi, T, Dv = enc_shape
        pairs = _LayerPairs()
        arenas = {}
        for li, i in enumerate(range(meta["lo"], meta["hi"])):
            b = "layer.%d." % i
            Ff = p[b + "intermediate.dense.weight"].shape[0]
            spec = [("a.qkv_bias", (3 * Hd,), True), ("attention.output.dense.bias", (Hd,), True),
                    ("attention.output.LayerNorm.weight", (Hd,), True), ("attention.output.LayerNorm.bias", (Hd,), True),
                    ("intermediate.dense.bias", (Ff,), True), ("output.dense.bias", (Hd,), True),
                    ("output.LayerNorm.weight", (Hd,), True), ("output.LayerNorm.bias", (Hd,), True),
                    ("a.qkv_weight", (3 * Hd, Hd), False), ("attention.output.dense.weight", (Hd, Hd), False),
                    ("intermediate.dense.weight", (Ff, Hd), False), ("output.dense.weight", (Hd, Ff), False)]
            if ctx.saved[li][8] is not None:
                spec += [("crossattention.self.query.bias", (Hd,), True), ("c.kv_bias", (2 * Hd,), True),
                         ("crossattention.output.dense.bias", (Hd,), True), ("crossattention.output.LayerNorm.weight", (Hd,), True),
                         ("crossattention.output.LayerNorm.bias", (Hd,), True), ("crossattention.self.query.weight", (Hd, Hd), False),
                         ("c.kv_weight", (2 * Hd, Dv), False), ("crossattention.output.dense.weight", (Hd, Hd), False)]
            arenas[i] = Grads(dev, spec, key=("bert", id(p[b + "attention.self.query.weight"])), params=[p[n] for n in names if n.startswith(b)],
                              zero=False)
        Grads.zero_all(list(arenas.values()))
        for li, i in reversed(list(enumerate(range(meta["lo"], meta["hi"])))):
            b = "layer.%d." % i
            a = b + "attention."
            hb, qkv, att, lse, s1, m1, r1, h1b, cr, h2b, pre, act, s3, m3, r3 = ctx.saved[li]
            ctx.saved[li] = None
            Ff = p[b + "intermediate.dense.weight"].shape[0]
            G = arenas.pop(i)
            tn, po = [], []
            _begin_layer_backward()
            ds3, ds3b = K.layernorm_bwd(dh, s3, m3, r3, p[b + "output.LayerNorm.weight"], G["output.LayerNorm.weight"],
                                        G["output.LayerNorm.bias"], dcol=G["output.dense.bias"], want_bf16=True,
                                        drop_out=BertLayersFn._drop(meta, i, 4))
            _, woutT = BANK.linear(p[b + "output.dense.weight"])
            _, wiT = BANK.linear(p[b + "intermediate.dense.weight"])
            if FUSE_DGELU_COLSUM:
                dpre = K.gemm_nt_dgelu_colsum(ds3b, woutT, pre, G["intermediate.dense.bias"])
            else:
                dpre = K.gemm_nt(ds3b, woutT, aux=pre, act=2)
                K.colsum_bf16(dpre, G["intermediate.dense.bias"])
            dh2 = K.gemm_nt(dpre, wiT, resid=ds3, out_dtype=F32)
            tn += [(ds3b, act, G["output.dense.weight"]), (dpre, h2b, G["intermediate.dense.weight"])]
            if cr is not None:
                c = b + "crossattention."
                q2, kv, att2, lse2, s2, m2, r2 = cr
                ds2, ds2b = K.layernorm_bwd(dh2, s2, m2, r2, p[c + "output.LayerNorm.weight"], G["crossattention.output.LayerNorm.weight"],
                                            G["crossattention.output.LayerNorm.bias"], dcol=G["crossattention.output.dense.bias"],
                                            want_bf16=True, drop_out=BertLayersFn._drop(meta, i, 3))
                _, wo2T = BANK.linear(p[c + "output.dense.weight"])
                datt2 = K.gemm_nt(ds2b, wo2T)
                dq2 = torch.empty_like(q2)
                dkv = torch.empty_like(kv)
                delta2 = torch.empty_like(lse2)
                kv_done = None

                def attn2(phase, ask_form=False):
                    return K.attn_bwd(K.view3(q2, S, L), K.view3(kv, Bi, T, 0), K.view3(kv, Bi, T, Hd), K.view3(att2, S, L),
                                      K.view3(datt2, S, L), S, Bi, H, L, T, scale, lse2, delta2, K.view3(dq2, S, L), K.view3(dkv, Bi, T, 0),
                                      K.view3(dkv, Bi, T, Hd), mask=meta["enc_mask"], kv_idx=meta["kv_idx"], seq_off=meta["seq_off"],
                                      seq_ids=meta["seq_ids"], drop=BertLayersFn._drop(meta, i, 2), phase=phase, ask_form=ask_form)
                one_pass = attn2(0, ask_form=True) != 0
                aux = AUX.enabled and not (AUX.auto and one_pass)
                attn2(1 if aux and not one_pass else 0)
                _param_only(po, K.colsum_bf16, dq2, G["crossattention.self.query.bias"])
                G.alias("crossattention.self.key.bias", G["c.kv_bias"][:Hd])
                G.alias("crossattention.self.value.bias", G["c.kv_bias"][Hd:])
                G.alias("crossattention.self.key.weight", G["c.kv_weight"][:Hd])
                G.alias("crossattention.self.value.weight", G["c.kv_weight"][Hd:])
                _, wqT = BANK.linear(p[c + "self.query.weight"])
                _, wkvT = BANK.linear(p[c + "self.key.weight"], p[c + "self.value.weight"])
                dh1 = K.gemm_nt(dq2, wqT, resid=ds2, out_dtype=F32)
                if aux:
                    first = denc is None
                    if first:
                        denc = torch.empty(Bi * T, Dv, device=dev, dtype=F32)

                    def kv_side(attn2=attn2, dkv=dkv, wkvT=wkvT, first=first, denc=denc, one_pass=one_pass):
                        if not one_pass:
                            attn2(2)
                        K.gemm_nt(dkv, wkvT, resid=None if first else denc, out=denc)
                    kv_done = AUX.launch(kv_side, [q2, kv, att2, datt2, lse2, delta2, dq2, dkv, wkvT, denc])
                else:
                    denc = K.gemm_nt(dkv, wkvT, resid=denc, out_dtype=F32)
                tn = [(dkv, encb, G["c.kv_weight"])] + tn + [(ds2b, att2, G["crossattention.output.dense.weight"]),
                                                            (dq2, h1b, G["crossattention.self.query.weight"])]
            else:
                dh1 = dh2
            ds1, ds1b = K.layernorm_bwd(dh1, s1, m1, r1, p[a + "output.LayerNorm.weight"], G["attention.output.LayerNorm.weight"],
                                        G["attention.output.LayerNorm.bias"], dcol=G["attention.output.dense.bias"], want_bf16=True,
                                        drop_out=BertLayersFn._drop(meta, i, 1))
            _, woT = BANK.linear(p[a + "output.dense.weight"])
            datt = K.gemm_nt(ds1b, woT)
            dqkv = torch.empty_like(qkv)
            delta = torch.empty_like(lse)
            if meta.get("self_mask2d") is not None:
                K.attn_bwd_mask2d(K.view3(qkv, S, L, 0), K.view3(qkv, S, L, Hd), K.view3(qkv, S, L, 2 * Hd), K.view3(att, S, L),
                                  K.view3(datt, S, L), S, H, L, scale, lse, delta, K.view3(dqkv, S, L, 0), K.view3(dqkv, S, L, Hd),
                                  K.view3(dqkv, S, L, 2 * Hd), meta["self_mask2d"], drop=BertLayersFn._drop(meta, i, 0))
            else:
                K.attn_bwd(K.view3(qkv, S, L, 0), K.view3(qkv, S, L, Hd), K.view3(qkv, S, L, 2 * Hd), K.view3(att, S, L), K.view3(datt, S, L),
                           S, S, H, L, L, scale, lse, delta, K.view3(dqkv, S, L, 0), K.view3(dqkv, S, L, Hd), K.view3(dqkv, S, L, 2 * Hd),
                           mask=meta["self_mask"], drop=BertLayersFn._drop(meta, i, 0))
            _param_only(po, K.colsum_bf16, dqkv, G["a.qkv_bias"])
            for k3, nm in enumerate(("query", "key", "value")):
                G.alias("attention.self.%s.bias" % nm, G["a.qkv_bias"][k3 * Hd:(k3 + 1) * Hd])
                G.alias("attention.self.%s.weight" % nm, G["a.qkv_weight"][k3 * Hd:(k3 + 1) * Hd])
            _, wqkvT = BANK.linear(p[a + "self.query.weight"], p[a + "self.key.weight"], p[a + "self.value.weight"])
            dh = K.gemm_nt(dqkv, wqkvT, resid=ds1, out_dtype=F32)
            tn += [(ds1b, att, G["attention.output.dense.weight"]), (dqkv, hb, G["a.qkv_weight"])]
            if cr is not None:
                if kv_done is not None and WGRAD_QUEUE is None:
                    torch.cuda.current_stream().wait_event(kv_done)
                _param_only(po, K.colsum_bf16, dkv, G["c.kv_bias"])
            pairs.add(G, tn, po)
            for n in names:
                if n.startswith(b):
                    out[n] = G.g[n[len(b):]]
        pairs.flush()
        SIDE.join()
        AUX.join()
        d_enc = denc.view(enc_shape) if denc is not None else None
        return (dh.view(S, L, Hd), d_enc, None) + tuple(out[n] for n in names)


# ... 231 lines not shown
```

### x2-vlm_amd/kernels.py

```python
import ctypes as C

import torch

from . import _lib
from ._lib import AttnArgs, call, ptr, raw_stream

BF16, F32 = torch.bfloat16, torch.float32


GEMM_TIMER = None


class _timed:

    def __init__(self, flops, name="gemm_nt"):
        self.flops = flops
        self.name = name

    def __enter__(self):
        if GEMM_TIMER is not None:
            self.a = torch.cuda.Event(enable_timing=True)
            self.b = torch.cuda.Event(enable_timing=True)
            self.a.record()

# ... 17 lines not shown

def _hash32_int(x):
    x &= 0xFFFFFFFF
    x ^= x >> 16; x = (x * 0x7feb352d) & 0xFFFFFFFF
    x ^= x >> 15; x = (x * 0x846ca68b) & 0xFFFFFFFF
    x ^= x >> 16
    return x


def dropout_keep(spec, index):
    thr, seed, scale = spec[:3]
    if len(spec) > 3 and spec[3] is not None:
        seed = _hash32_int((seed + 0x9E3779B1 * (int(spec[3].item()) & 0xFFFFFFFF)) & 0xFFFFFFFF)
    e = index.to(torch.int64) & 0xFFFFFFFF
    x = ((e >> 1) ^ seed) & 0xFFFFFFFF
    x = x ^ (x >> 16); x = (x * 0x7feb352d) & 0xFFFFFFFF
    x = x ^ (x >> 15); x = (x * 0x846ca68b) & 0xFFFFFFFF
    x = x ^ (x >> 16)
    u = torch.where((e & 1) == 1, x >> 16, x & 0xFFFF)
    return (u >= thr).to(torch.float32) * scale


_WS = {}
_WS_RETIRED = []
_WS_CAPTURED = set()


def workspace(device, nfloats):
    key = (device, raw_stream())
    buf = _WS.get(key)
    if buf is None or buf.numel() < nfloats:
        if buf is not None and buf.data_ptr() in _WS_CAPTURED:
            _WS_RETIRED.append(buf)
        buf = torch.empty(max(nfloats, 1 << 22, 0 if buf is None else 2 * buf.numel()), device=device, dtype=F32)
        _WS[key] = buf
    if buf.is_cuda and torch.cuda.is_current_stream_capturing():
        _WS_CAPTURED.add(buf.data_ptr())
    return buf


DEFERRED = None


def _ws_and_defer(device, nfloats):
    if DEFERRED is not None:
        return torch.empty(nfloats, device=device, dtype=F32), 1
    return workspace(device, nfloats), 0


def reduce_partials(ws, nblk, nk, width, outs):
    o = list(outs) + [None] * (3 - len(outs))
    call("x2_reduce_partials", ptr(ws), nblk, nk, width, ptr(o[0]), ptr(o[1]), ptr(o[2]))


def reduce_partials_multi(items):
    flat = []
    for ws, nblk, nk, width, outs in items:
        o = list(outs) + [None] * (4 - len(outs))
        flat += [ws.data_ptr(), nblk, nk, width] + [0 if t is None else t.data_ptr() for t in o]
    call("x2_reduce_partials_multi", (C.c_int64 * len(flat))(*flat), len(items))


def cast_transpose_multi(desc):
    flat = [v for d in desc for v in (tuple(d) + (0,) if len(d) == 7 else d)]
    call("x2_cast_transpose_multi", (C.c_int64 * len(flat))(*flat), len(desc))


def copy_f32_multi(desc):
    flat = [v for d in desc for v in d]
    call("x2_copy_f32_multi", (C.c_int64 * len(flat))(*flat), len(desc))


def _rows(t):
    assert t.dim() == 2 and t.stride(1) == 1, "expected a row-major 2-D tensor (got strides %s)" % (t.stride(),)
    return t.stride(0)


def round_up(x, m):
    return (x + m - 1) // m * m



def gemm_nt(A, B, *, bias=None, gamma=None, resid=None, aux=None, act=0, out=None, out_dtype=BF16, drop=NO_DROP,
            rowscale=None, colsum=None):
    assert A.dtype == BF16 and B.dtype == BF16 and A.shape[1] == B.shape[1]
    M, K = A.shape
    N = B.shape[0]
    if out is None:
        out = torch.empty(M, N, device=A.device, dtype=out_dtype)
    assert out.shape == (M, N) and out.dtype in (BF16, F32)
    for t in (bias, gamma):
        assert t is None or (t.dtype == F32 and t.numel() == N and t.is_contiguous())
    assert resid is None or (resid.dtype == F32 and resid.shape == (M, N))
    assert aux is None or (aux.dtype == BF16 and aux.shape == (M, N))
    assert rowscale is None or (rowscale.dtype == F32 and rowscale.numel() == M and rowscale.is_contiguous())
    with _timed(2.0 * M * N * K):
        call("x2_gemm_nt", ptr(A), ptr(B), ptr(out), M, N, K, _rows(A), _rows(B), _rows(out), ptr(bias), ptr(gamma),
             ptr(resid), _rows(resid) if resid is not None else 0, ptr(aux), _rows(aux) if aux is not None else 0,
             act, 1 if out.dtype == F32 else 0, drop[0], drop[1], drop[2], ptr(drop[3]), ptr(rowscale), ptr(colsum))
    return out


def gemm_nt_dgelu_colsum(A, B, pre, colsum):
    assert A.dtype == BF16 and B.dtype == BF16 and A.shape[1] == B.shape[1] and pre.dtype == BF16
    M, K = A.shape
    N = B.shape[0]
    assert pre.shape == (M, N) and colsum.dtype == F32 and colsum.numel() == N
    out = torch.empty(M, N, device=A.device, dtype=BF16)
    ws, defer = _ws_and_defer(A.device, 2 * ((M + 63) // 64) * N)
    nrows = C.c_int(0)
    with _timed(2.0 * M * N * K):
        call("x2_gemm_nt_dgelu_colparts", ptr(A), ptr(B), ptr(out), M, N, K, _rows(A), _rows(B), _rows(out), ptr(pre), _rows(pre),
             ptr(ws), C.byref(nrows))
    if defer:
        DEFERRED.append((ws, nrows.value, 1, N, (colsum,)))
    else:
        reduce_partials(ws, nrows.value, 1, N, (colsum,))
    return out


def gemm_nt_splitk(A, B, out=None, slices=0):
    assert A.dtype == BF16 and B.dtype == BF16 and A.shape[1] == B.shape[1]
    M, K = A.shape
    N = B.shape[0]
    if out is None:
        out = torch.empty(M, N, device=A.device, dtype=F32)
    assert out.shape == (M, N) and out.dtype == F32
    ws = workspace(A.device, min(32, max(1, K // 64)) * M * N)
    with _timed(2.0 * M * N * K):
        call("x2_gemm_nt_splitk", ptr(A), ptr(B), ptr(out), M, N, K, _rows(A), _rows(B), _rows(out), slices, ptr(ws), ws.numel())
    return out


def gemm_tn_grouped(problems, accumulate=False, split=0):
    rows = []
    for pr in problems:
        dY, X, dW = pr[:3]
        assert dY.dtype == BF16 and X.dtype == BF16 and dW.dtype == F32 and dY.shape[0] == X.shape[0]
        N, K = dW.shape
        n_ld, k_ld = (pr[3], pr[4]) if len(pr) == 5 else (dY.shape[1], X.shape[1])
        assert dY.shape[1] >= N or n_ld >= N
        rows.append([dY.data_ptr(), X.data_ptr(), dW.data_ptr(), dY.shape[0], N, K, _rows(dY), _rows(X), _rows(dW),
                     n_ld, k_ld])
    dev = problems[0][0].device
    for i in range(0, len(rows), 8):
        chunk = rows[i:i + 8]
        arr = (C.c_int64 * (11 * len(chunk)))(*[v for r in chunk for v in r])
        tiles256 = sum(((r[4] + 255) // 256) * ((r[5] + 255) // 256) for r in chunk)
        want = (split if split else 4) * tiles256 * 65536
        ws = workspace(dev, want) if split != 1 else None
        with _timed(sum(2.0 * r[3] * r[4] * r[5] for r in chunk), "gemm_tn"):
            call("x2_gemm_tn_grouped", arr, len(chunk), 1 if accumulate else 0, split, ptr(ws), 0 if ws is None else ws.numel())



def _attn_args(q, k, v, B, Bkv, H, Lq, Lk, scale, bias=None, biasT=None, mask=None, kv_idx=None, seq_off=None,
               seq_ids=None, drop=NO_DROP, head_dim=64, bias_log2=False):
    a = AttnArgs()
    a.Q, a.q_bs, a.q_rs = q
    a.K, a.k_bs, a.k_rs = k
    a.V, a.v_bs, a.v_rs = v
    a.B, a.Bkv, a.H, a.Lq, a.Lk, a.scale = B, Bkv, H, Lq, Lk, scale
    a.head_dim = head_dim
    a.dbg = 16 if bias_log2 else 0
    a.drop_thr16, a.drop_seed, a.drop_scale = drop[:3]
    a.drop_epoch = ptr(drop[3])
    if bias is not None:
        assert bias.dtype == F32 and bias.dim() == 3 and bias.is_contiguous()
        a.bias, a.bias_ld = bias.data_ptr(), bias.shape[2]
    if biasT is not None:
        assert biasT.dtype == F32 and biasT.dim() == 3 and biasT.is_contiguous()
        a.biasT, a.biasT_ld = biasT.data_ptr(), biasT.shape[2]
    if mask is not None:
        assert mask.dtype == F32 and mask.dim() == 2 and mask.is_contiguous() and mask.shape[0] == B
        a.mask, a.mask_ld = mask.data_ptr(), mask.shape[1]
    if kv_idx is not None:
        assert kv_idx.dtype == torch.int32 and kv_idx.numel() == B
        a.kv_idx = kv_idx.data_ptr()
    if seq_off is not None:
        assert seq_off.dtype == torch.int32 and seq_ids.dtype == torch.int32
        a.seq_off, a.seq_ids = seq_off.data_ptr(), seq_ids.data_ptr()
    return a
# ... 18 lines not shown
    a.Lq, a.Lk, a.head_dim, a.scale = Lq, Lk, 64, 0.125
    for f in ("q_bs", "q_rs", "k_bs", "k_rs", "v_bs", "v_rs", "o_bs", "o_rs", "dq_bs", "dq_rs", "dk_bs", "dk_rs", "dv_bs", "dv_rs", "do_bs", "do_rs"):
        setattr(a, f, 64)
    if shared_kv:
        a.kv_idx = a.seq_off = a.seq_ids = 8
    a.drop_thr16 = 1 if dropout else 0
    if workspace:
        a.ws, a.ws_floats = 8, ((Lq + 127) // 128) * 8192
    return _lib.lib().x2_attn_bwd_one_pass(C.byref(a))


def attn_bwd(q, k, v, o, do, B, Bkv, H, Lq, Lk, scale, lse, delta, dq, dk, dv, dS=None, phase=0, ask_form=False, colsum_ws=None, **kw):
    a = _attn_args(q, k, v, B, Bkv, H, Lq, Lk, scale, **kw)
    a.phase = phase
    a.O, a.o_bs, a.o_rs = o
    a.dO, a.do_bs, a.do_rs = do
    a.dQ, a.dq_bs, a.dq_rs = dq
    a.dK, a.dk_bs, a.dk_rs = dk
    a.dV, a.dv_bs, a.dv_rs = dv
    a.LSE, a.Delta = lse.data_ptr(), delta.data_ptr()
    if dS is not None:
        assert dS.dtype == BF16 and dS.is_contiguous() and dS.shape[:3] == (B, H, Lq)
        a.dS, a.ds_ld = dS.data_ptr(), dS.shape[3]
    if phase == 0 and Lq > 208 and Lk > 208 and a.kv_idx is None and not a.drop_thr16:
        ws = workspace(lse.device, B * H * ((Lq + 127) // 128) * 8192)
        a.ws, a.ws_floats = ws.data_ptr(), ws.numel()
    if ask_form:
        return _lib.lib().x2_attn_bwd_one_pass(C.byref(a))
    if colsum_ws is not None:
        assert colsum_ws.dtype == F32 and colsum_ws.is_contiguous() and colsum_ws.shape == (B, 2, H * 64)
        form = _lib.lib().x2_attn_bwd_one_pass(C.byref(a))
        if form in (1, 3):
            a.colsum_ws = colsum_ws.data_ptr()
        call("x2_attn_bwd", C.byref(a))
        return form
    call("x2_attn_bwd", C.byref(a))


def _check_mask2d(mask2d, B, L):
    assert mask2d.dtype == F32 and mask2d.dim() == 3 and mask2d.is_contiguous() and mask2d.shape[:2] == (B, L)
    assert mask2d.shape[2] % 64 == 0 and mask2d.shape[2] >= L


def attn_fwd_mask2d(q, k, v, B, H, L, scale, out, lse, mask2d, drop=NO_DROP, head_dim=64):
    _check_mask2d(mask2d, B, L)
    a = _attn_args(q, k, v, B, B, H, L, L, scale, drop=drop, head_dim=head_dim)
    a.Out, a.o_bs, a.o_rs = out
    assert lse.dtype == F32 and lse.numel() == B * H * L
    a.LSE = lse.data_ptr()
    call("x2_attn_fwd_mask2d", C.byref(a), mask2d.data_ptr(), mask2d.shape[2])


def attn_bwd_mask2d(q, k, v, o, do, B, H, L, scale, lse, delta, dq, dk, dv, mask2d, drop=NO_DROP, head_dim=64):
    _check_mask2d(mask2d, B, L)
    a = _attn_args(q, k, v, B, B, H, L, L, scale, drop=drop, head_dim=head_dim)
    a.O, a.o_bs, a.o_rs = o
    a.dO, a.do_bs, a.do_rs = do
    a.dQ, a.dq_bs, a.dq_rs = dq
    a.dK, a.dk_bs, a.dk_rs = dk
    a.dV, a.dv_bs, a.dv_rs = dv
    a.LSE, a.Delta = lse.data_ptr(), delta.data_ptr()
    call("x2_attn_bwd_mask2d", C.byref(a), mask2d.data_ptr(), mask2d.shape[2])



def layernorm_fwd(x, w, b, eps, *, rows=None, period=0, want_bf16=True, want_f32=False, y_bf16=None, y_f32=None,
                  drop=NO_DROP):
    assert x.dtype == F32 and x.is_contiguous()
    D = x.shape[-1]
    x2 = x.view(-1, D)
    R = x2.shape[0] if rows is None else rows
    if want_bf16 and y_bf16 is None:
        y_bf16 = torch.empty_like(x2, dtype=BF16)
    if want_f32 and y_f32 is None:
        y_f32 = torch.empty_like(x2)
    mean = torch.empty(R, device=x.device, dtype=F32)
    rstd = torch.empty(R, device=x.device, dtype=F32)
    call("x2_layernorm_fwd", ptr(x2), ptr(w), ptr(b), ptr(y_bf16), ptr(y_f32), ptr(mean), ptr(rstd), R, D, eps, period,
         drop[0], drop[1], drop[2], ptr(drop[3]))
    return y_bf16, y_f32, mean, rstd


def layernorm_bwd(dy, x, mean, rstd, w, dw, db, *, dres=None, dcol=None, period=0, want_f32=True, want_bf16=False, dx=None,
                  drop_in=NO_DROP, drop_out=NO_DROP, post=None):
    assert dy.dtype in (F32, BF16) and x.dtype == F32 and dy.is_contiguous() and x.is_contiguous()
    D = x.shape[-1]
    R = mean.numel()
    if want_f32 and dx is None:
        dx = torch.empty_like(x) if period == 0 else torch.zeros_like(x)
    prs = None
    if post is not None:
        assert dcol is None and dy.dtype == BF16 and period == 0
        prs, dcol = post
        assert prs is None or (prs.dtype == F32 and prs.numel() == R and prs.is_contiguous())
        want_bf16 = True
    dxb = torch.empty(x.shape, device=x.device, dtype=BF16) if want_bf16 else None
    nblk = (R + 15) // 16
    ws, defer = _ws_and_defer(x.device, nblk * 3 * D)
    call("x2_layernorm_bwd", ptr(dy), 1 if dy.dtype == BF16 else 0, ptr(x), ptr(mean), ptr(rstd), ptr(w), ptr(dres), ptr(dx), ptr(dxb), ptr(dw), ptr(db),
         ptr(dcol), R, D, period, drop_in[0], drop_in[1], drop_in[2], drop_out[0], drop_out[1], drop_out[2],
         ptr(drop_in[3] if drop_in[3] is not None else drop_out[3]), ptr(ws), defer, 0 if post is None else 1, ptr(prs))
    if defer:
        DEFERRED.append((ws, nblk, 3, D, (dw, db, dcol)))
    return dx, dxb


def colsum_bf16(y, out):
    nblk = (y.shape[0] + 63) // 64
    ws, defer = _ws_and_defer(y.device, nblk * y.shape[1])
    call("x2_colsum_bf16", ptr(y), ptr(out), y.shape[0], y.shape[1], _rows(y), ptr(ws), defer)
    if defer:
        DEFERRED.append((ws, nblk, 1, y.shape[1], (out,)))


def rowscale_cast_colsum(dx, colsum, rowscale=None):
    assert dx.dtype == F32 and dx.is_contiguous() and dx.dim() == 2
    dxb = torch.empty_like(dx, dtype=BF16)
    nblk = (dx.shape[0] + 31) // 32
    ws, defer = _ws_and_defer(dx.device, nblk * dx.shape[1])
    call("x2_rowscale_cast_colsum", ptr(dx), ptr(rowscale), ptr(dxb), ptr(colsum), dx.shape[0], dx.shape[1], ptr(ws), defer)
    if defer:
        DEFERRED.append((ws, nblk, 1, dx.shape[1], (colsum,)))
    return dxb


def layerscale_finish(items):
    flat = []
    for G, W, bias, gamma, cs, dgamma, dbias in items:
        N, Kd = G.shape
        assert G.dtype == F32 and W.dtype == F32 and G.is_contiguous() and W.is_contiguous() and W.numel() == G.numel() and Kd % 4 == 0
        flat += [G.data_ptr(), W.data_ptr(), 0 if bias is None else bias.data_ptr(), gamma.data_ptr(), cs.data_ptr(), dgamma.data_ptr(),
                 0 if dbias is None else dbias.data_ptr(), N, Kd]
    call("x2_layerscale_finish", (C.c_int64 * len(flat))(*flat), len(items))


def cast_bf16(src, out=None):
    assert src.dtype == F32 and src.is_contiguous() and src.numel() % 4 == 0
    if out is None:
        out = torch.empty_like(src, dtype=BF16)
    call("x2_cast_bf16", ptr(src), ptr(out), src.numel())
    return out


def cast_transpose_bf16(src, want_plain=True, ldt=None):
    assert src.dtype == F32 and src.dim() == 2 and src.is_contiguous()
    R, Cc = src.shape
    ldt = R if ldt is None else ldt
    plain = torch.empty(R, Cc, device=src.device, dtype=BF16) if want_plain else None
    tr = (torch.zeros if ldt > R else torch.empty)(Cc, ldt, device=src.device, dtype=BF16)
    call("x2_cast_transpose_bf16", ptr(src), ptr(plain), ptr(tr), R, Cc, ldt)
    return plain, tr


def patchify(image, ps):
    assert image.dtype == F32 and image.is_contiguous() and image.dim() == 4 and image.shape[1] == 3
    B, _, R, _ = image.shape
    g = R // ps
    cols = torch.empty(B * g * g, 3 * ps * ps, device=image.device, dtype=BF16)
    call("x2_patchify", ptr(image), ptr(cols), B, R, ps)
    return cols


def assemble_tokens(patch, cls, B, P):
    D = patch.shape[1]
    x = torch.empty(B, P + 1, D, device=patch.device, dtype=F32)
    call("x2_assemble_tokens", ptr(patch), ptr(cls), ptr(x), B, P, D)
    return x


def assemble_tokens_bwd(dx, dcls):
    B, T, D = dx.shape
    dpatch = torch.empty(B * (T - 1), D, device=dx.device, dtype=BF16)
    call("x2_assemble_tokens_bwd", ptr(dx), ptr(dpatch), ptr(dcls), B, T - 1, D)
    return dpatch


def pool_tokens(x, w=None, bwd=False):
    B, T, D = x.shape
    assert x.dtype == F32 and x.is_contiguous() and (w is None or (w.dtype == F32 and w.shape == (B, T - 1) and w.is_contiguous()))
    call("x2_pool_tokens", ptr(x), ptr(w), B, T - 1, D, 1 if bwd else 0)
    return x


LOG2E = 1.4426950408889634
# ... 177 lines not shown
        call("x2_mlm_ls_fwd", ptr(x), ptr(E), ptr(bias), ptr(labels), int(ignore), R, Vp, V, Hd, _rows(x), _rows(E), ptr(part), ptr(sumz),
             ptr(zlab), ptr(zign))
    call("x2_ls_combine", ptr(part), ptr(sumz), Vp // 64, ptr(zlab), ptr(zign), ptr(labels), ptr(weights), R, V, int(ignore), float(ls),
         ptr(lse), ptr(rows), ptr(stat))
    return stat, lse


def mlm_ls_bwd(x, E, bias, labels, weights, lse, g, stat, V, ignore, ls, gscale=1.0):
    R, Hd = x.shape
    Vp = E.shape[0]
    dl = torch.empty(R, Vp, device=x.device, dtype=BF16)
    with _timed(2.0 * R * Vp * Hd, "gemm_nt_recompute"):
        call("x2_mlm_ls_bwd", ptr(x), ptr(E), ptr(bias), ptr(labels), ptr(weights), ptr(lse), ptr(g), ptr(stat), gscale, float(ls), int(ignore),
             R, Vp, V, Hd, _rows(x), _rows(E), ptr(dl), Vp)
    return dl


def mask_words(seed, epoch, batch, count):
    seed = int(seed) & 0xFFFFFFFF
    if epoch is not None:
        seed = _hash32_int((seed + 0x9E3779B1 * (int(epoch) & 0xFFFFFFFF)) & 0xFFFFFFFF)
    out = torch.empty(batch, count, dtype=torch.int64)
    for b in range(batch):
        hb = _hash32_int((seed + 0x9E3779B1 * (b + 1)) & 0xFFFFFFFF)
        for k in range(count):
            out[b, k] = _hash32_int(hb ^ ((0x85EBCA6B * (k + 1)) & 0xFFFFFFFF))
    return out


def mask_tokens(text_ids, text_atts, is_subword, *, words=None, seed=0, epoch=None, mask_prob=0.5, max_masks=12, skipgram_prb=0.2, skipgram_size=3,
                mask_whole_word=True, cls_id=101, mask_id=103, pad_id=0, pad_mask=-100, out=None):
    assert text_ids.dtype == torch.int64 and text_atts.dtype == torch.int64 and text_ids.shape == text_atts.shape and text_ids.dim() == 2
    assert text_ids.is_contiguous() and text_atts.is_contiguous() and is_subword.dtype == torch.uint8 and is_subword.is_contiguous()
    B, L = text_ids.shape
    dev = text_ids.device
    if out is not None:
        idm, mpos, mids = out
        assert idm.shape == (B, L) and mpos.shape == (B, max_masks) and mids.shape == (B, max_masks)
        assert all(t.dtype == torch.int64 and t.is_contiguous() for t in out)
    else:
        idm = torch.empty(B, L, device=dev, dtype=torch.int64)
        mpos = torch.empty(B, max_masks, device=dev, dtype=torch.int64)
        mids = torch.empty(B, max_masks, device=dev, dtype=torch.int64)
    if words is not None:
        assert words.dtype in (torch.int32, torch.uint32) and words.dim() == 2 and words.shape[0] == B and words.is_contiguous()
    call("x2_mask_tokens", ptr(text_ids), ptr(text_atts), B, L, ptr(is_subword), is_subword.numel(), ptr(words), words.shape[1] if words is not None else 0,
         int(seed) & 0xFFFFFFFF, ptr(epoch), float(mask_prob), int(max_masks), float(skipgram_prb), int(skipgram_size), 1 if mask_whole_word else 0,
         int(cls_id), int(mask_id), int(pad_id), int(pad_mask), ptr(idm), ptr(mpos), ptr(mids))
    return idm, mpos, mids


def sample_negatives(sim, u, group=None):
    n = sim.shape[0]
    out = torch.empty(n, device=sim.device, dtype=torch.int32)
    call("x2_sample_negatives", ptr(sim), n, ptr(group), ptr(u), ptr(out))
    return out


def additive_mask(atts, neg):
    assert atts.dtype == torch.int64 and atts.dim() == 2 and atts.is_contiguous()
    S, L = atts.shape
    out = torch.empty(S, round_up(L, 64), device=atts.device, dtype=F32)
    call("x2_additive_mask", ptr(atts), ptr(out), S, L, out.shape[1], float(neg))
    return out


def additive_mask2d(atts, neg):
    assert atts.dtype == torch.int64 and atts.dim() == 3 and atts.shape[1] == atts.shape[2] and atts.is_contiguous()
    S, L = atts.shape[:2]
    out = torch.empty(S, L, round_up(L, 64), device=atts.device, dtype=F32)
    call("x2_additive_mask2d", ptr(atts), ptr(out), S, L, out.shape[2], float(neg))
    return out


def kv_csr(kv, Bi):
    assert kv.dtype == torch.int32 and kv.dim() == 1 and kv.is_contiguous()
    S = kv.numel()
    off = torch.empty(Bi + 1, device=kv.device, dtype=torch.int32)
    order = torch.empty(S, device=kv.device, dtype=torch.int32)
    call("x2_kv_csr", ptr(kv), S, Bi, ptr(off), ptr(order))
    return off, order


def tail_index(ineg, tneg, text_atts, image_atts, with_match=True):
    B, L = text_atts.shape
    T = image_atts.shape[1]
    assert text_atts.dtype == torch.int64 and image_atts.dtype == torch.int64 and text_atts.is_contiguous() and image_atts.is_contiguous()
    assert not with_match or (ineg.dtype == torch.int32 and tneg.dtype == torch.int32 and ineg.numel() == B and tneg.numel() == B)
    R = 4 * B if with_match else B
    dev = text_atts.device
    t_idx = torch.empty(R, device=dev, dtype=torch.int32)
    kv = torch.empty(R, device=dev, dtype=torch.int32)
    atts = torch.empty(R, L, device=dev, dtype=torch.int64)
    enc = torch.empty(R, T, device=dev, dtype=torch.int64)
    call("x2_tail_index", ptr(ineg) if with_match else None, ptr(tneg) if with_match else None, ptr(text_atts), ptr(image_atts), B, L, T,
         1 if with_match else 0, ptr(t_idx), ptr(kv), ptr(atts), ptr(enc))
    return t_idx, kv, atts, enc


def droppath_rows(rates, seed, B, T):
    depth = rates.numel()
    out = torch.empty(depth, 2, B * T, device=rates.device, dtype=F32)
    call("x2_droppath_rows", ptr(rates), int(seed) & 0xFFFFFFFF, ptr(DROP_EPOCH), depth, B, T, ptr(out))
    return out


def droppath_keep(rates, seed, B, epoch=None):
    s_ = int(seed) & 0xFFFFFFFF
    if epoch is not None:
        s_ = _hash32_int((s_ + 0x9E3779B1 * (int(epoch) & 0xFFFFFFFF)) & 0xFFFFFFFF)
    depth = len(rates)
    keep = torch.zeros(depth, 2, B)
    for lb in range(2 * depth):
        for b in range(B):
            h = _hash32_int(((lb * B + b) & 0xFFFFFFFF) ^ s_)
            u = torch.tensor(float(h >> 8), dtype=torch.float32) * torch.tensor(1.0 / 16777216.0, dtype=torch.float32)
            keep[lb >> 1, lb & 1, b] = 1.0 if float(u) >= float(torch.tensor(rates[lb >> 1], dtype=torch.float32)) else 0.0
    return keep


def frame_mean(x, pos, frames):
    BF, T, D = x.shape
    assert x.dtype == F32 and x.is_contiguous() and BF % frames == 0 and (pos is None or (pos.is_contiguous() and pos.numel() == frames * D))
    out = torch.empty(BF // frames, T, D, device=x.device, dtype=F32)
    call("x2_frame_mean", ptr(x), ptr(pos), None, ptr(out), None, BF // frames, frames, T, D, 0)
    return out


def frame_mean_bwd(dy, frames, want_dpos=True):
    B, T, D = dy.shape
    assert dy.dtype == F32 and dy.is_contiguous()
    dx = torch.empty(B * frames, T, D, device=dy.device, dtype=F32)
    dpos = torch.empty(frames, D, device=dy.device, dtype=F32) if want_dpos else None
    call("x2_frame_mean", None, None, ptr(dy), ptr(dx), ptr(dpos), B, frames, T, D, 1)
    return dx, dpos


def gelu_f32(x, dy=None):
    out = torch.empty_like(x)
    call("x2_gelu_f32", ptr(x), ptr(dy), ptr(out), x.numel())
    return out


def colsum_f32(x, out):
    call("x2_colsum_f32", ptr(x), ptr(out), x.shape[0], x.shape[1])
```

### x2-vlm_amd/model_pretrain.py

```python
import torch

from . import kernels as K
from . import ops
from .xvlm import XVLMBase


class XVLM(XVLMBase):
    def __init__(self, config, load_vision_params=True, load_text_params=True, pretraining=True):
        super().__init__(config, load_vision_params=load_vision_params, load_text_params=load_text_params,
                         use_contrastive_loss=True, use_matching_loss=True, use_mlm_loss=True, use_bbox_loss=True,
                         config_text=None, pretraining=pretraining)
        self.overlap_towers = True
        self._text_stream = None

    def tower_text(self, text_ids, text_atts, text_ids_masked):
        return self.get_text_embeds(torch.cat([text_ids, text_ids_masked]), torch.cat([text_atts, text_atts]))

    def tower_vision(self, image, image_atts=None, idx_to_group_img=None, ret_bbox_loss=False):
        if ret_bbox_loss:
            return self.get_vision_embeds(image, image_atts=image_atts, idx_to_group_img=idx_to_group_img)
        return self.get_vision_embeds(image) + (None,)

    def tail_features(self, image_embeds, both):
        return self.get_features(image_embeds, both[:image_embeds.shape[0]])

    def tail_losses(self, image_embeds, image_atts, both, image_feat, text_feat, text_atts, masked_pos, masked_ids,
                    image_embeds_fullatts=None, target_bbox=None, is_image=None, ret_bbox_loss=False, ret_match_loss=True,
                    gathered=None):
        B = image_embeds.shape[0]
        dev = both.device
        text_embeds = both[:B]
        loss_itc = self.get_contrastive_loss(image_feat, text_feat, gathered=gathered)
        ineg, tneg = self.get_hard_negatives(image_feat, text_feat) if ret_match_loss else (None, None)
        if both.is_cuda:
            t_idx, kv, atts, enc_atts = K.tail_index(ineg, tneg, text_atts.contiguous(), image_atts.contiguous(), with_match=ret_match_loss)
        else:
            ar = torch.arange(B, device=dev, dtype=torch.int32)
            t_idx, kv = (torch.cat([ar, ar, tneg, ar + B]), torch.cat([ar, ineg, ar, ar])) if ret_match_loss else (ar + B, ar)
            atts, enc_atts = torch.cat([text_atts, text_atts])[t_idx.long()], image_atts[kv.long()]
        h0 = ops.gather_rows(both, t_idx)
        fused = self.get_cross_embeds(image_embeds, enc_atts, text_embeds=h0, text_atts=atts, kv_idx=kv)
        if ret_match_loss:
            loss_itm = self._itm_loss(fused[:3 * B, 0, :], B)
        else:
            loss_itm = torch.tensor(0.0)
        loss_mlm, self.last_mlm_lse, self.last_mlm_logits = self.text_encoder.mlm_loss_from_hidden(fused[-B:], masked_pos, masked_ids)
        loss = {"loss_itc": loss_itc, "loss_itm": loss_itm, "loss_mlm": loss_mlm}
        self.last = dict(image_embeds=image_embeds.detach(), text_embeds=text_embeds.detach(), image_feat=image_feat.detach(),
                         text_feat=text_feat.detach())
        if ret_bbox_loss:
            output_coord = self.predict_bbox(image_embeds_fullatts, text_embeds, text_atts)
            self.last["bbox_coord"] = output_coord.detach()
            loss["loss_bbox"], loss["loss_giou"] = self.get_bbox_loss(output_coord, target_bbox, is_image=is_image)
        return loss

    def forward_multimodal(self, image, text_ids, text_atts, text_ids_masked=None, masked_pos=None, masked_ids=None,
                           image_atts=None, idx_to_group_img=None, target_bbox=None, is_image=None,
                           ret_bbox_loss=False, ret_match_loss=True):
        overlap = self.overlap_towers and image.is_cuda
        if overlap:
            if self._text_stream is None:
                self._text_stream = torch.cuda.Stream()
            main = torch.cuda.current_stream()
            self._text_stream.wait_stream(main)
            with torch.cuda.stream(self._text_stream):
                both = self.tower_text(text_ids, text_atts, text_ids_masked)
        image_embeds, image_atts, image_embeds_fullatts = self.tower_vision(image, image_atts, idx_to_group_img, ret_bbox_loss)
        if overlap:
            main.wait_stream(self._text_stream)
            both.record_stream(main)
        else:
            both = self.tower_text(text_ids, text_atts, text_ids_masked)
        image_feat, text_feat = self.tail_features(image_embeds, both)
        return self.tail_losses(image_embeds, image_atts, both, image_feat, text_feat, text_atts, masked_pos, masked_ids,
                                image_embeds_fullatts=image_embeds_fullatts, target_bbox=target_bbox, is_image=is_image,
                                ret_bbox_loss=ret_bbox_loss, ret_match_loss=ret_match_loss)

    def forward_text(self, text_ids=None, text_atts=None, text_ids_masked=None, masked_pos=None, masked_ids=None):
        seq = self._bert(text_ids_masked, attention_mask=text_atts, mode="multi_modal").last_hidden_state
        loss, self.last_mlm_lse, self.last_mlm_logits = self.text_encoder.mlm_loss_from_hidden(seq, masked_pos, masked_ids)
        self.last = dict(text_embeds=seq.detach())
        return {"loss_mlm": loss}

    def forward(self, image=None, text_ids=None, text_atts=None, text_ids_masked=None, masked_pos=None, masked_ids=None,
                image_atts=None, idx_to_group_img=None, target_bbox=None, is_image=None, ret_bbox_loss=False,
                ret_match_loss=True):
        if image is None:
            return self.forward_text(text_ids, text_atts, text_ids_masked, masked_pos, masked_ids)
        return self.forward_multimodal(image, text_ids, text_atts, text_ids_masked, masked_pos, masked_ids, image_atts,
                                       idx_to_group_img, target_bbox, is_image, ret_bbox_loss, ret_match_loss=ret_match_loss)
```

### x2-vlm_amd/xbert.py

```python
import json
import os
from types import SimpleNamespace

import torch
import torch.nn as nn

from . import kernels as K
from . import ops
from .engine import BertLayersFn, EmbeddingsFn, MlmLossFn, _mask_pad, bert_layer_param_names


_FIXED_SEEDS = []


def _key_mask(atts, neg):
    if atts.is_cuda and atts.dtype == torch.int64:
        return K.additive_mask(atts.contiguous(), neg)
    return _mask_pad((1.0 - atts.float()) * neg, atts.shape[1])


def _text_masks(atts):
    if atts.dim() == 3:
        return None, K.additive_mask2d(atts.to(torch.int64).contiguous(), -10000.0)
    return _key_mask(atts, -10000.0), None
# ... 19 lines not shown
    def from_json_file(cls, path):
        with open(path) as f:
            return cls(**json.load(f))


class BertEmbeddings(nn.Module):
    def __init__(self, config):
        super().__init__()
        self.word_embeddings = nn.Embedding(config.vocab_size, config.hidden_size, padding_idx=config.pad_token_id)
        self.position_embeddings = nn.Embedding(config.max_position_embeddings, config.hidden_size)
        self.token_type_embeddings = nn.Embedding(config.type_vocab_size, config.hidden_size)
        self.LayerNorm = nn.LayerNorm(config.hidden_size, eps=config.layer_norm_eps)
        self.register_buffer("position_ids", torch.arange(config.max_position_embeddings).expand((1, -1)))
        self.eps = config.layer_norm_eps
        self.config = config

    def forward(self, input_ids, position_ids=None):
        drop = K.NO_DROP
        if self.training and self.config.hidden_dropout_prob > 0:
            drop = K.dropout_spec(self.config.hidden_dropout_prob, next_dropout_seed(), 1000)
        args = (input_ids, self.eps, drop, self.word_embeddings.weight, self.position_embeddings.weight,
                self.token_type_embeddings.weight, self.LayerNorm.weight, self.LayerNorm.bias)
        if position_ids is None:
            return EmbeddingsFn.apply(*args)
        return EmbeddingsFn.apply(*args, position_ids)


class BertSelfAttention(nn.Module):
    def __init__(self, config, is_cross_attention):
        super().__init__()
        kin = config.encoder_width if is_cross_attention else config.hidden_size
        self.query = nn.Linear(config.hidden_size, config.hidden_size)
        self.key = nn.Linear(kin, config.hidden_size)
        self.value = nn.Linear(kin, config.hidden_size)


class BertSelfOutput(nn.Module):
    def __init__(self, config):
        super().__init__()
        self.dense = nn.Linear(config.hidden_size, config.hidden_size)
        self.LayerNorm = nn.LayerNorm(config.hidden_size, eps=config.layer_norm_eps)


class BertAttention(nn.Module):
    def __init__(self, config, is_cross_attention=False):
        super().__init__()
        self.self = BertSelfAttention(config, is_cross_attention)
        self.output = BertSelfOutput(config)


class BertIntermediate(nn.Module):
    def __init__(self, config):
        super().__init__()
        self.dense = nn.Linear(config.hidden_size, config.intermediate_size)


class BertOutput(nn.Module):
    def __init__(self, config):
        super().__init__()
        self.dense = nn.Linear(config.intermediate_size, config.hidden_size)
        self.LayerNorm = nn.LayerNorm(config.hidden_size, eps=config.layer_norm_eps)


class BertLayer(nn.Module):
    def __init__(self, config, layer_num):
        super().__init__()
        self.attention = BertAttention(config)
        self.has_cross_attention = layer_num >= config.fusion_layer
        if self.has_cross_attention:
            self.crossattention = BertAttention(config, is_cross_attention=True)
        self.intermediate = BertIntermediate(config)
        self.output = BertOutput(config)


_IDENTITY_CSR = {}


class BertEncoder(nn.Module):
    def __init__(self, config):
        super().__init__()
        self.config = config
        self.layer = nn.ModuleList([BertLayer(config, i) for i in range(config.num_hidden_layers)])

    def run(self, hidden, text_atts, enc=None, enc_atts=None, mode="multi_modal", kv_idx=None):
        cfg = self.config
        lo, hi = {"text": (0, cfg.fusion_layer), "fusion": (cfg.fusion_layer, cfg.num_hidden_layers),
                  "multi_modal": (0, cfg.num_hidden_layers)}[mode]
        S, L, _ = hidden.shape
        drop = None
        if self.training and (cfg.hidden_dropout_prob > 0 or cfg.attention_probs_dropout_prob > 0):
            drop = dict(seed=next_dropout_seed(), p_hidden=cfg.hidden_dropout_prob, p_attn=cfg.attention_probs_dropout_prob)
        meta = dict(lo=lo, hi=hi, fusion_at=cfg.fusion_layer, heads=cfg.num_attention_heads, eps=cfg.layer_norm_eps,
                    self_mask=None, self_mask2d=None, enc_mask=None, kv_idx=None,
                    seq_off=None, seq_ids=None, drop=drop)
        meta["self_mask"], meta["self_mask2d"] = _text_masks(text_atts)
        cross = enc is not None and hi > cfg.fusion_layer
        if cross:
            Bi = enc.shape[0]
            meta["enc_mask"] = _key_mask(enc_atts, -1e9)
            if kv_idx is None:
                assert Bi == S, "encoder batch %d != text batch %d and no kv_idx given" % (Bi, S)
                if enc.is_cuda and torch.is_grad_enabled() and (hidden.requires_grad or enc.requires_grad or self.training) \
                        and K.attn_bwd_form(L, enc.shape[1], shared_kv=True) == 2:
                    ident = _IDENTITY_CSR.get((S, enc.device))
                    if ident is None:
                        ar = torch.arange(S + 1, device=enc.device, dtype=torch.int32)
                        ident = (ar[:S].contiguous(), ar, ar[:S].contiguous())
                        if not torch.cuda.is_current_stream_capturing():
                            _IDENTITY_CSR[(S, enc.device)] = ident
                    meta.update(kv_idx=ident[0], seq_off=ident[1], seq_ids=ident[2])
            else:
                kv = kv_idx.to(torch.int32).contiguous()
                if kv.is_cuda:
                    off, order = K.kv_csr(kv, Bi)
                else:
                    order = torch.argsort(kv, stable=True).to(torch.int32).contiguous()
                    off = torch.zeros(Bi + 1, device=kv.device, dtype=torch.int32)
                    off[1:] = torch.cumsum(torch.bincount(kv, minlength=Bi), 0)
                meta.update(kv_idx=kv, seq_off=off, seq_ids=order)
        cache = self.__dict__.setdefault("_param_lists", {})
        params = cache.get((lo, hi, cross))
        if params is None:
            sd = dict(self.named_parameters())
            params = cache[(lo, hi, cross)] = [sd[n] for n in bert_layer_param_names(lo, hi, cfg.fusion_layer, cross)]
        return BertLayersFn.apply(hidden, enc if cross else None, meta, *params)


class BertModel(nn.Module):
    def __init__(self, config, add_pooling_layer=False):
        super().__init__()
        assert not add_pooling_layer
        self.config = config
        self.embeddings = BertEmbeddings(config)
        self.encoder = BertEncoder(config)
        self.apply(lambda m: _bert_init(m, config.initializer_range))

    def get_input_embeddings(self):
        return self.embeddings.word_embeddings

    def forward(self, input_ids=None, attention_mask=None, encoder_embeds=None, encoder_hidden_states=None,
                encoder_attention_mask=None, return_dict=True, mode="multi_modal", kv_idx=None, position_ids=None, **unused):
        _refuse_unused("BertModel", unused)
        hidden = self.embeddings(input_ids, position_ids) if encoder_embeds is None else encoder_embeds
        S, L = hidden.shape[:2]
        if attention_mask is None:
            attention_mask = torch.ones(S, L, device=hidden.device)
        if encoder_hidden_states is not None and encoder_attention_mask is None:
            encoder_attention_mask = torch.ones(S, encoder_hidden_states.shape[1], device=hidden.device)
        out = self.encoder.run(hidden, attention_mask, encoder_hidden_states, encoder_attention_mask, mode, kv_idx)
        return SimpleNamespace(last_hidden_state=out) if return_dict else (out,)


class BertPredictionHeadTransform(nn.Module):
    def __init__(self, config):
        super().__init__()
        self.dense = nn.Linear(config.hidden_size, config.hidden_size)
        self.LayerNorm = nn.LayerNorm(config.hidden_size, eps=config.layer_norm_eps)


class BertLMPredictionHead(nn.Module):
    def __init__(self, config):
        super().__init__()
        self.transform = BertPredictionHeadTransform(config)
        self.decoder = nn.Linear(config.hidden_size, config.vocab_size, bias=False)
        self.bias = nn.Parameter(torch.zeros(config.vocab_size))


class BertOnlyMLMHead(nn.Module):
    def __init__(self, config):
        super().__init__()
        self.predictions = BertLMPredictionHead(config)


class BertForMaskedLM(nn.Module):

    def __init__(self, config):
        super().__init__()
        self.config = config
        self.bert = BertModel(config)
        self.cls = BertOnlyMLMHead(config)
        self.apply(lambda m: _bert_init(m, config.initializer_range))
        self.cls.predictions.decoder.weight = self.bert.embeddings.word_embeddings.weight

    def mlm_loss_from_hidden(self, sequence_output, masked_pos, labels, keep_logits=False):
        B, L, Hd = sequence_output.shape
        flat = (torch.arange(B, device=masked_pos.device).unsqueeze(1) * L + masked_pos).reshape(-1)
        rows = ops.gather_rows(sequence_output.reshape(B * L, Hd), flat)
        pr = self.cls.predictions
        return MlmLossFn.apply(rows, labels, self.config.layer_norm_eps, keep_logits, pr.transform.dense.weight, pr.transform.dense.bias,
                               pr.transform.LayerNorm.weight, pr.transform.LayerNorm.bias, pr.bias,
                               self.bert.embeddings.word_embeddings.weight)

    def smoothed_mlm_loss_from_hidden(self, sequence_output, masked_pos, labels, weights, ignore_index, label_smoothing, keep_logits=False):
        B, L, Hd = sequence_output.shape
        flat = (torch.arange(B, device=masked_pos.device).unsqueeze(1) * L + masked_pos).reshape(-1)
        rows = ops.gather_rows(sequence_output.reshape(B * L, Hd), flat)
        pr = self.cls.predictions
        w = weights.reshape(-1).to(torch.float32).contiguous()
        return MlmLossFn.apply(rows, labels, self.config.layer_norm_eps, keep_logits, pr.transform.dense.weight, pr.transform.dense.bias,
                               pr.transform.LayerNorm.weight, pr.transform.LayerNorm.bias, pr.bias,
                               self.bert.embeddings.word_embeddings.weight, (w, int(ignore_index), float(label_smoothing)))

    def forward(self, input_ids=None, attention_mask=None, encoder_hidden_states=None, encoder_attention_mask=None,
                labels=None, return_dict=True, mode="multi_modal", masked_pos=None, return_logits=False, position_ids=None, **unused):
        _refuse_unused("BertForMaskedLM", unused)
        if masked_pos is None:
            raise NotImplementedError("need check!")
        h = self.bert(input_ids, attention_mask=attention_mask, encoder_hidden_states=encoder_hidden_states,
                      encoder_attention_mask=encoder_attention_mask, mode=mode, position_ids=position_ids).last_hidden_state
        lab = labels if labels is not None else torch.full_like(masked_pos, -100)
        loss, _, logits = self.mlm_loss_from_hidden(h, masked_pos, lab, keep_logits=return_logits)
        if logits is not None:
            logits = logits[:, :self.config.vocab_size].view(masked_pos.shape[0], masked_pos.shape[1], -1)
        if return_logits:
            return logits
        return SimpleNamespace(loss=loss if labels is not None else None, logits=logits)


def _refuse_unused(who, unused):
    for k, v in unused.items():
        if v not in (None, False):
            raise NotImplementedError("%s.forward(%s=...) is not supported by the HIP path" % (who, k))


def _bert_init(m, std):
    if isinstance(m, (nn.Linear, nn.Embedding)):
        m.weight.data.normal_(mean=0.0, std=std)
    elif isinstance(m, nn.LayerNorm):
        m.bias.data.zero_()
        m.weight.data.fill_(1.0)
    if isinstance(m, nn.Linear) and m.bias is not None:
        m.bias.data.zero_()


def get_bert_config(encoder_rpath, num_hidden_layers=12, cross_start_at=12):
    config = BertConfig.from_json_file(os.path.join(encoder_rpath, "config.json"))
    config.num_hidden_layers = num_hidden_layers
    config.fusion_layer = cross_start_at
    config.embedding_dim = config.hidden_size
    return config
```

### x2-vlm_amd/xvlm.py

```python
import os

import torch
import torch.distributed as dist
import torch.nn as nn

from . import box_ops, checkpoint, ops
from . import kernels as K
from .beit2 import beit_base_patch16, beit_large_patch16, read_json, trunc_normal_
from .xbert import BertForMaskedLM, BertModel, get_bert_config


class AllGather(torch.autograd.Function):

    @staticmethod
    def forward(ctx, tensor, rank, world_size):
        out = [torch.empty_like(tensor) for _ in range(world_size)]
        dist.all_gather(out, tensor.contiguous())
        ctx.rank, ctx.batch_size = rank, tensor.shape[0]
        return torch.cat(out, 0)

    @staticmethod
    def backward(ctx, grad_output):
        return grad_output[ctx.batch_size * ctx.rank: ctx.batch_size * (ctx.rank + 1)], None, None

# ... 71 lines not shown
            self.update_init_params(["text_proj." + n for n, _ in self.text_proj.named_parameters()])
            if config.get("fix_temp", False):
                self.temp = torch.ones([]) * config["temp"]
            else:
                self.temp = nn.Parameter(torch.ones([]) * config["temp"])
                self.update_init_params(["temp"])
        self.use_matching_loss = use_matching_loss
        if use_matching_loss:
            self.itm_head = build_mlp(self.text_width, 2)
            self.update_init_params(["itm_head." + n for n, _ in self.itm_head.named_parameters()])
        self.use_bbox_loss = use_bbox_loss
        if use_bbox_loss:
            self.bbox_head = build_mlp(self.text_width, 4)
            self.update_init_params(["bbox_head." + n for n, _ in self.bbox_head.named_parameters()])
        if not pretraining:
            self.init_params = []
        self.injected_negatives = None

    def update_init_params(self, missing_keys=None):
        for k in missing_keys or []:
            if k not in self.init_params:
                self.init_params.append(k)
        named = set(n for n, _ in self.named_parameters())
        self.init_params = [n for n in self.init_params if n in named]

    def load_pretrained(self, ckpt_rpath, config, is_eval=False, is_domain_pretrain=False):
        if is_domain_pretrain:
            state = checkpoint._model_state(ckpt_rpath)
            if config.get("init_timesformer", False):
                checkpoint.init_timesformer_keys(state)
        else:
            state = checkpoint.load_pretrained(self, ckpt_rpath, config, is_eval=is_eval, load_text=True)
        own = getattr(self, "absolute_frame_pos_embed", None)
        given = state.get("absolute_frame_pos_embed")
        if own is not None and given is not None and given.shape != own.shape:
            n = min(given.shape[1], own.shape[1])
            with torch.no_grad():
                own[:, :n] = given[:, :n]
            del state["absolute_frame_pos_embed"]
            print("frame position embedding: %d of %d checkpoint frames used" % (n, given.shape[1]), flush=True)
        result = self.load_state_dict(state, strict=False)
        self.update_init_params(list(result.missing_keys))
        print("checkpoint %s: %d unexpected keys; trained from scratch: %s"
              % (ckpt_rpath, len(result.unexpected_keys), sorted(self.init_params)), flush=True)
        return result

    @property
    def _bert(self):
        return self.text_encoder.bert if hasattr(self.text_encoder, "bert") else self.text_encoder

    def get_frame_embeds(self, frame, **unused):
        assert frame.dim() == 5
        B, Fr = frame.shape[:2]
        e = self.vision_encoder(frame.reshape(B * Fr, *frame.shape[2:]))
        pos = self.absolute_frame_pos_embed if self.add_frame_pos else torch.zeros(1, Fr, 1, e.shape[-1], device=e.device)
        e = ops.frame_mean(e, pos, Fr)
        return e, torch.ones(e.shape[:2], dtype=torch.long, device=e.device)

    def get_image_embeds(self, image, image_atts=None, idx_to_group_img=None, **unused):
        assert image.dim() == 4
        if idx_to_group_img is None:
            e = self.vision_encoder(image)
            return e, torch.ones(e.shape[:2], dtype=torch.long, device=image.device)
        if image_atts is None:
            full = ops.gather_rows(self.vision_encoder(image), idx_to_group_img)
            return full, torch.ones(full.shape[:2], dtype=torch.long, device=image.device)
        assert image_atts.size(0) == idx_to_group_img.size(0)
        e, full = self.vision_encoder(image, idx_to_group_img=idx_to_group_img, image_atts=image_atts)
        return e, image_atts, ops.gather_rows(full, idx_to_group_img)

    def get_vision_embeds(self, image, image_atts=None, idx_to_group_img=None, output_hidden_states=None, output_attentions=None):
        assert output_hidden_states == output_attentions
        if image.dim() == 5:
            assert idx_to_group_img is None, "not supported"
            return self.get_frame_embeds(image)
        return self.get_image_embeds(image, image_atts=image_atts, idx_to_group_img=idx_to_group_img)

    def get_text_embeds(self, text_ids, text_atts, **unused):
        return self._bert(text_ids, attention_mask=text_atts, mode="text").last_hidden_state

    def get_text_embeds_12L(self, text_ids, text_atts, **unused):
        return self._bert(text_ids, attention_mask=text_atts).last_hidden_state

    def get_cross_embeds(self, image_embeds, image_atts, text_ids=None, text_embeds=None, text_atts=None, kv_idx=None, **unused):
        assert text_atts is not None
        if text_embeds is not None:
            return self._bert(encoder_embeds=text_embeds, attention_mask=text_atts, encoder_hidden_states=image_embeds,
                              encoder_attention_mask=image_atts, mode="fusion", kv_idx=kv_idx).last_hidden_state
        if text_ids is not None:
            return self._bert(text_ids, attention_mask=text_atts, encoder_hidden_states=image_embeds,
                              encoder_attention_mask=image_atts, kv_idx=kv_idx).last_hidden_state
        raise ValueError

    def get_features(self, image_embeds=None, text_embeds=None):
        fi = ft = None
        if image_embeds is not None:
            fi = ops.normalize(ops.linear(image_embeds[:, 0, :], self.vision_proj.weight, self.vision_proj.bias))
        if text_embeds is not None:
            ft = ops.normalize(ops.linear(text_embeds[:, 0, :], self.text_proj.weight, self.text_proj.bias))
        if image_embeds is None:
            return ft
        if text_embeds is None:
            return fi
        return fi, ft

    def _sim(self, a, b):
        return ops.linear(a, b) / self.temp

    def get_contrastive_loss(self, image_feat, text_feat, idx=None, gathered=None):
        assert image_feat.size(-1) == self.embed_dim and text_feat.size(-1) == self.embed_dim
        fi, ft = gathered if gathered is not None else (allgather(image_feat), allgather(text_feat))
        logits = self._sim(fi, ft)
        n = logits.shape[0]
        if idx is None:
            labels = torch.arange(n, device=logits.device)
            return (ops.cross_entropy(logits, labels) + ops.cross_entropy(logits.t(), labels)) / 2
        idx = idx.view(-1, 1)
        idx_all = allgather(idx)
        pos = torch.eq(idx_all, idx_all.t()).float()
        lab = pos / pos.sum(1, keepdim=True)
        li = -torch.sum(torch.log_softmax(logits, dim=1) * lab, dim=1).mean()
        lt = -torch.sum(torch.log_softmax(logits.t(), dim=1) * lab, dim=1).mean()
        return (li + lt) / 2

    def get_hard_negatives(self, image_feat, text_feat, idx=None):
        if self.injected_negatives is not None:
            return tuple(torch.as_tensor(n, dtype=torch.int32, device=image_feat.device) for n in self.injected_negatives)
        with torch.no_grad():
            fi, ft = image_feat.detach(), text_feat.detach()
            temp = self.temp.detach().reshape(1).float()
            bs = fi.shape[0]
            sim_i2t = K.linear_f32(fi, ft, alpha_ptr=None) / temp
            sim_t2i = K.linear_f32(ft, fi, alpha_ptr=None) / temp
            u = torch.rand(2, bs, device=fi.device)
            grp = idx.view(-1).long().contiguous() if idx is not None else None
            if grp is not None and bool((grp.view(-1, 1) == grp.view(1, -1)).all(1).any()):
                raise RuntimeError("get_hard_negatives: a row has no candidate with a different idx (invalid multinomial distribution)")
            return K.sample_negatives(sim_t2i, u[0].contiguous(), grp), K.sample_negatives(sim_i2t, u[1].contiguous(), grp)

    def get_matching_loss(self, image_embeds, image_atts, image_feat, text_embeds, text_atts, text_feat, idx=None):
        ineg, tneg = self.get_hard_negatives(image_feat, text_feat, idx=idx)
        B = image_embeds.shape[0]
        ar = torch.arange(B, device=image_embeds.device, dtype=torch.int32)
        t_idx = torch.cat([ar, ar, tneg])
        kv = torch.cat([ar, ineg, ar])
        cls = self._fusion_cls(image_embeds, image_atts, text_embeds, text_atts, t_idx, kv)
        return self._itm_loss(cls, B)

    def _fusion_cls(self, image_embeds, image_atts, text_embeds, text_atts, t_idx, kv):
        h0 = ops.gather_rows(text_embeds, t_idx)
        out = self.get_cross_embeds(image_embeds, image_atts[kv.long()], text_embeds=h0, text_atts=text_atts[t_idx.long()], kv_idx=kv)
        return out[:, 0, :]

    def _itm_loss(self, cls, B):
        logits = ops.mlp_head(self.itm_head, cls)
        cache = self.__dict__.setdefault("_itm_labels", {})
        labels = cache.get((B, cls.device))
        if labels is None:
            labels = torch.zeros(3 * B, dtype=torch.long, device=cls.device)
            labels[:B] = 1
            cache[(B, cls.device)] = labels
        self.last_itm_logits = logits.detach()
        return ops.cross_entropy(logits, labels)

    def get_mlm_loss(self, text_ids_masked, text_atts, image_embeds, image_atts, masked_pos, masked_ids):
        return self.text_encoder(text_ids_masked, attention_mask=text_atts, encoder_hidden_states=image_embeds,
                                 encoder_attention_mask=image_atts, labels=masked_ids, masked_pos=masked_pos).loss

    def predict_bbox(self, image_embeds, text_embeds, text_atts):
        assert image_embeds.size(0) == text_embeds.size(0)
        ones = torch.ones(image_embeds.shape[:2], device=image_embeds.device)
        cls = self.get_cross_embeds(image_embeds, ones, text_embeds=text_embeds, text_atts=text_atts)[:, 0, :]
        return ops.mlp_head(self.bbox_head, cls).sigmoid()

# ... 16 lines not shown
```

Measured before the change: 2913.

## Prune last fusion layer to CLS and masked-token rows only

Adds a row-table path so the final fusion layer computes its tail (dense GEMMs, layernorm and dropout) only for the rows actually consumed: CLS rows for ITM and masked positions for MLM. The tail-index kernel emits the row ids, and the GEMM and layernorm-backward kernels use the original row ids for dropout hashing so the masks stay consistent. This avoids FFN and output work on unused tokens in the last layer, at the cost of extra plumbing and a new gather path. It is enabled through an engine flag that defaults on in the probe.

```diff
diff --git a/include/x2vlm_hip.h b/include/x2vlm_hip.h
--- a/include/x2vlm_hip.h
+++ b/include/x2vlm_hip.h
@@ -15,6 +15,10 @@
                const float* bias, const float* gamma, const float* resid, int ldr, void* aux, int ldaux,
                int act, int out_f32, unsigned drop_thr16, unsigned drop_seed, float drop_scale, const unsigned* drop_epoch,
                const float* rowscale, float* colsum, void* stream);
+int x2_gemm_nt_rows(const void* A, const void* B, void* C, int M, int N, int K, int lda, int ldb, int ldc,
+                    const float* bias, const float* gamma, const float* resid, int ldr, void* aux, int ldaux,
+                    int act, int out_f32, unsigned drop_thr16, unsigned drop_seed, float drop_scale, const unsigned* drop_epoch,
+                    const float* rowscale, float* colsum, const int* row_ids , void* stream);
 
 int x2_gemm_nt_dgelu_colparts(const void* A, const void* B, void* C, int M, int N, int K, int lda, int ldb, int ldc,
                               const void* aux, int ldaux, float* colparts, int* nrows_out, void* stream);
@@ -59,6 +63,11 @@
                      int period, unsigned in_thr16, unsigned in_seed, float in_scale, unsigned out_thr16,
                      unsigned out_seed, float out_scale, const unsigned* drop_epoch, float* ws ,
                      int defer, int post, const float* post_rowscale, void* stream);
+int x2_layernorm_bwd_rows(const void* dy, int dy_is_bf16, const float* x, const float* mean, const float* rstd, const float* w,
+                          const float* dres, float* dx, void* dx_bf16, float* dw, float* db, float* dcol, int rows, int D,
+                          int period, unsigned in_thr16, unsigned in_seed, float in_scale, unsigned out_thr16,
+                          unsigned out_seed, float out_scale, const unsigned* drop_epoch, float* ws, int defer, int post,
+                          const float* post_rowscale, const int* row_ids , void* stream);
 int x2_colsum_bf16(const void* y, float* out, int M, int N, int ld, float* ws , int defer, void* stream);
 int x2_reduce_partials(const float* part, int nblk, int nk, int width, float* o0, float* o1, float* o2, void* stream);
 int x2_reduce_partials_multi(const int64_t* desc, int count, void* stream);
@@ -124,6 +133,8 @@
 int x2_kv_csr(const int* kv, int S, int Bi, int* off, int* order, void* stream);
 int x2_tail_index(const int* ineg, const int* tneg, const long* text_atts , const long* image_atts , int B, int L,
                   int T, int with_match, int* t_idx, int* kv, long* atts_out , long* enc_out , void* stream);
+int x2_tail_index_rows(const int* ineg, const int* tneg, const long* text_atts, const long* image_atts, int B, int L, int T, int with_match,
+                       int* t_idx, int* kv, long* atts_out, long* enc_out, const long* masked_pos, int Mm, int* rows, void* stream);
 int x2_droppath_rows(const float* rates, unsigned seed, const unsigned* epoch, int depth, int B, int T, float* out, void* stream);
 int x2_frame_mean(const float* x, const float* pos, const float* dy, float* out, float* dpos, int Bc, int F, int T, int D, int bwd,
                   void* stream);
diff --git a/probes/ab_step.py b/probes/ab_step.py
--- a/probes/ab_step.py
+++ b/probes/ab_step.py
@@ -36,12 +36,15 @@
             env[k] = val.replace("+", ",")
     variants.append((name, knobs, env))
 res = {n: [] for n, _, _ in variants}
+seg = {n: [] for n, _, _ in variants}
+engine = importlib.import_module("x2-vlm_amd.engine")
 for rnd in range(args.rounds):
     for name, knobs, env in variants:
         for k, val in knobs.items():
             assert lib.x2_tune(k, val) == 0, lib.x2_last_error()
         old = {k: os.environ.get(k) for k in env}
         os.environ.update(env)
+        engine.PRUNE_LAST_ROWS = os.environ.get("X2_PRUNE_LAST", "1") == "1"
         step = graph.SegmentedStep(model, batch, warmup=1)
         assert step.mode == "hipgraph-segments", step.error
         for _ in range(args.warmup):
@@ -54,6 +57,8 @@
         b.record()
         torch.cuda.synchronize()
         res[name].append(a.elapsed_time(b) / args.steps)
+        if os.environ.get("X2_SEG_TIMES") == "1":
+            seg[name].append({k: v for k, v in step.segment_times().items() if not k.startswith("start:")})
         del step
         for k in knobs:
             lib.x2_tune(k, 0)
@@ -70,3 +75,5 @@
     r = res[name]
     print("  %-12s %-28s %s   min %.3f  mean %.3f" % (name, ",".join("%s=%s" % kv for kv in list(knobs.items()) + list(env.items())) or "-",
                                                        " ".join("%.3f" % x for x in r), min(r), sum(r) / len(r)))
+    for i, t in enumerate(seg[name]):
+        print("      round %d segments (ms): %s" % (i, "  ".join("%s %.3f" % kv for kv in sorted(t.items()))))
diff --git a/x2-vlm_amd/_lib.py b/x2-vlm_amd/_lib.py
--- a/x2-vlm_amd/_lib.py
+++ b/x2-vlm_amd/_lib.py
@@ -75,6 +75,9 @@
     "x2_mlm_ls_fwd": [P, P, P, P, L, I, I, I, I, I, I, P, P, P, P, P],
     "x2_ls_combine": [P, P, I, P, P, P, P, I, I, L, F, P, P, P, P],
     "x2_mlm_ls_bwd": [P, P, P, P, P, P, P, P, F, F, L, I, I, I, I, I, I, P, L, P],
+    "x2_gemm_nt_rows": [P, P, P, I, I, I, I, I, I, P, P, P, I, P, I, I, I, U, U, F, P, P, P, P, P],
+    "x2_layernorm_bwd_rows": [P, I, P, P, P, P, P, P, P, P, P, P, I, I, I, U, U, F, U, U, F, P, P, I, I, P, P, P],
+    "x2_tail_index_rows": [P, P, P, P, I, I, I, I, P, P, P, P, P, I, P, P],
 }
 _COMM_SIGS = {
     "x2_comm_unique_id": [P],
diff --git a/x2-vlm_amd/csrc/gemm.hip b/x2-vlm_amd/csrc/gemm.hip
--- a/x2-vlm_amd/csrc/gemm.hip
+++ b/x2-vlm_amd/csrc/gemm.hip
@@ -35,6 +35,7 @@
   long ce_ignore;
   float ce_ls;
   const float* ce_w;
+  const int* row_ids;
 };
 
 __device__ __forceinline__ void tile_coords(int t, int tiles_m, int tiles_n, int gm, int& tm, int& tn) {
@@ -227,9 +228,10 @@
       }
       if (has_drop) {
         float dm[4];
-        drop_mul4(drop_, (uint32_t)m * (uint32_t)p.N + (uint32_t)n, dm);
+        const uint32_t e0 = (uint32_t)(p.row_ids ? p.row_ids[m] : m) * (uint32_t)p.N + (uint32_t)n;
+        drop_mul4(drop_, e0, dm);
         v[0] *= dm[0]; v[1] *= dm[1]; v[2] *= dm[2]; v[3] *= dm[3];
-        drop_mul4(drop_, (uint32_t)m * (uint32_t)p.N + (uint32_t)n + 4u, dm);
+        drop_mul4(drop_, e0 + 4u, dm);
         v[4] *= dm[0]; v[5] *= dm[1]; v[6] *= dm[2]; v[7] *= dm[3];
       }
       if (has_scale) {
@@ -316,7 +318,7 @@
         float v[4] = {a0.x + bb[0], a0.y + bb[1], a0.z + bb[2], a0.w + bb[3]};
         if (has_drop) {
           float dm[4];
-          drop_mul4(drop_, (uint32_t)m * (uint32_t)p.N + (uint32_t)n, dm);
+          drop_mul4(drop_, (uint32_t)(p.row_ids ? p.row_ids[m] : m) * (uint32_t)p.N + (uint32_t)n, dm);
           v[0] *= dm[0]; v[1] *= dm[1]; v[2] *= dm[2]; v[3] *= dm[3];
         }
         if (E::scale) {
@@ -1018,10 +1020,21 @@
   hipLaunchKernelGGL((gemm_nt_kernel<TM, V, F4>), dim3(tiles), dim3(256), lds, stream, p);
 }
 
+extern "C" int x2_gemm_nt_rows(const void* A, const void* B, void* C, int M, int N, int K, int lda, int ldb, int ldc,
+                               const float* bias, const float* gamma, const float* resid, int ldr, void* aux, int ldaux,
+                               int act, int out_f32, unsigned drop_thr16, unsigned drop_seed, float drop_scale, const unsigned* drop_epoch,
+                               const float* rowscale, float* colsum, const int* row_ids, void* stream);
 extern "C" int x2_gemm_nt(const void* A, const void* B, void* C, int M, int N, int K, int lda, int ldb, int ldc,
                           const float* bias, const float* gamma, const float* resid, int ldr, void* aux, int ldaux,
                           int act, int out_f32, unsigned drop_thr16, unsigned drop_seed, float drop_scale, const unsigned* drop_epoch,
                           const float* rowscale, float* colsum, void* stream) {
+  return x2_gemm_nt_rows(A, B, C, M, N, K, lda, ldb, ldc, bias, gamma, resid, ldr, aux, ldaux, act, out_f32, drop_thr16, drop_seed, drop_scale,
+                         drop_epoch, rowscale, colsum, nullptr, stream);
+}
+extern "C" int x2_gemm_nt_rows(const void* A, const void* B, void* C, int M, int N, int K, int lda, int ldb, int ldc,
+                               const float* bias, const float* gamma, const float* resid, int ldr, void* aux, int ldaux,
+                               int act, int out_f32, unsigned drop_thr16, unsigned drop_seed, float drop_scale, const unsigned* drop_epoch,
+                               const float* rowscale, float* colsum, const int* row_ids, void* stream) {
   X2_REQUIRE(M > 0 && N > 0 && K > 0, "x2_gemm_nt: empty problem M=%d N=%d K=%d", M, N, K);
   X2_REQUIRE(drop_thr16 < 65536u, "x2_gemm_nt: drop_thr16=%u", drop_thr16);
   X2_REQUIRE(K % BK == 0, "x2_gemm_nt: K=%d must be a multiple of %d", K, BK);
@@ -1031,6 +1044,7 @@
   X2_REQUIRE((!resid || ldr % 4 == 0) && (!aux || ldaux % 8 == 0), "x2_gemm_nt: ldr/ldaux alignment");
   GemmNT p{(const bf16_t*)A, (const bf16_t*)B, C, bias, gamma, resid, (bf16_t*)aux, M, N, K, lda, ldb, ldc, ldr, ldaux, act, out_f32,
            g_tune[0] > 0 ? g_tune[0] : 8, DropSpec{drop_thr16, drop_seed, drop_scale}, drop_epoch, rowscale, colsum, g_tune[2], 0};
+  p.row_ids = drop_thr16 ? row_ids : nullptr;
   int var = 4;
   {
     const bool plain = !gamma && !rowscale && !drop_thr16 && !colsum;
diff --git a/x2-vlm_amd/csrc/heads.hip b/x2-vlm_amd/csrc/heads.hip
--- a/x2-vlm_amd/csrc/heads.hip
+++ b/x2-vlm_amd/csrc/heads.hip
@@ -457,8 +457,17 @@
 __global__ __launch_bounds__(256) void tail_index_kernel(const int* __restrict__ ineg, const int* __restrict__ tneg,
                                                          const long* __restrict__ text_atts, const long* __restrict__ image_atts, int B, int L,
                                                          int T, int with_match, int* __restrict__ t_idx, int* __restrict__ kv,
-                                                         long* __restrict__ atts_out, long* __restrict__ enc_out) {
+                                                         long* __restrict__ atts_out, long* __restrict__ enc_out,
+                                                         const long* __restrict__ masked_pos, int Mm, int* __restrict__ rows) {
   const int r = blockIdx.x, q = with_match ? r / B : 3, b = r % B;
+  if (rows) {
+    const int ncls = with_match ? 3 * B : 0;
+    if (q < 3) { if (threadIdx.x == 0) rows[r] = r * L; }
+    else for (int j = threadIdx.x; j < Mm; j += 256) {
+      const long pos = masked_pos[(long)b * Mm + j];
+      rows[ncls + b * Mm + j] = r * L + (int)(pos < 0 ? 0 : (pos >= L ? L - 1 : pos));
+    }
+  }
   const int ti = q == 2 ? tneg[b] : (q == 3 ? B + b : b), ki = q == 1 ? ineg[b] : b;
   if (threadIdx.x == 0) { t_idx[r] = ti; kv[r] = ki; }
   const long* ta = text_atts + (long)(ti % B) * L;
@@ -471,8 +480,19 @@
   X2_REQUIRE(text_atts && image_atts && t_idx && kv && atts_out && enc_out && B > 0 && L > 0 && T > 0, "x2_tail_index: B=%d L=%d T=%d", B, L, T);
   X2_REQUIRE(!with_match || (ineg && tneg), "x2_tail_index: with_match needs the negative indices");
   hipLaunchKernelGGL(tail_index_kernel, dim3(with_match ? 4 * B : B), dim3(256), 0, (hipStream_t)stream, ineg, tneg, text_atts, image_atts, B, L, T,
-                     with_match, t_idx, kv, atts_out, enc_out);
+                     with_match, t_idx, kv, atts_out, enc_out, nullptr, 0, nullptr);
   return x2_check_launch("x2_tail_index");
+}
+extern "C" int x2_tail_index_rows(const int* ineg, const int* tneg, const long* text_atts, const long* image_atts, int B, int L, int T,
+                                  int with_match, int* t_idx, int* kv, long* atts_out, long* enc_out, const long* masked_pos, int Mm,
+                                  int* rows, void* stream) {
+  X2_REQUIRE(text_atts && image_atts && t_idx && kv && atts_out && enc_out && B > 0 && L > 0 && T > 0, "x2_tail_index_rows: B=%d L=%d T=%d", B, L, T);
+  X2_REQUIRE(!with_match || (ineg && tneg), "x2_tail_index_rows: with_match needs the negative indices");
+  X2_REQUIRE(masked_pos && rows && Mm > 0, "x2_tail_index_rows: masked_pos / rows / Mm=%d", Mm);
+  X2_REQUIRE((long)4 * B * L <= 2147483647L, "x2_tail_index_rows: B=%d x L=%d rows exceed int32", B, L);
+  hipLaunchKernelGGL(tail_index_kernel, dim3(with_match ? 4 * B : B), dim3(256), 0, (hipStream_t)stream, ineg, tneg, text_atts, image_atts, B, L, T,
+                     with_match, t_idx, kv, atts_out, enc_out, masked_pos, Mm, rows);
+  return x2_check_launch("x2_tail_index_rows");
 }
 
 __global__ __launch_bounds__(256) void droppath_rows_kernel(const float* __restrict__ rates, uint32_t seed, const uint32_t* __restrict__ epoch,
diff --git a/x2-vlm_amd/csrc/rowwise.hip b/x2-vlm_amd/csrc/rowwise.hip
--- a/x2-vlm_amd/csrc/rowwise.hip
+++ b/x2-vlm_amd/csrc/rowwise.hip
@@ -228,7 +228,7 @@
                                                             const float* __restrict__ w, const float* dres, float* dx, bf16_t* dxb,
                                                             float* ws, int rows, int D, int period,
                                                             DropSpec din_, DropSpec dout_, const uint32_t* __restrict__ epoch,
-                                                            const float* __restrict__ post_rs) {
+                                                            const float* __restrict__ post_rs, const int* __restrict__ row_ids) {
   constexpr int NSET = 3;
   constexpr bool DYB = MODE != 0;
   extern __shared__ __attribute__((aligned(16))) float red[];
@@ -282,7 +282,7 @@
         float4 om = o;
         if (dout.thr16) {
           float dm[4];
-          drop_mul4(dout, (uint32_t)gr * (uint32_t)D + (uint32_t)(c * 4), dm);
+          drop_mul4(dout, (uint32_t)(row_ids ? row_ids[gr] : (int)gr) * (uint32_t)D + (uint32_t)(c * 4), dm);
           om.x *= dm[0]; om.y *= dm[1]; om.z *= dm[2]; om.w *= dm[3];
         }
         if (dres) { const float4 rr = *reinterpret_cast<const float4*>(dres + gr * D + c * 4); o.x += rr.x; o.y += rr.y; o.z += rr.z; o.w += rr.w; }
@@ -327,11 +327,25 @@
   }
 }
 
+extern "C" int x2_layernorm_bwd_rows(const void* dy, int dy_is_bf16, const float* x, const float* mean, const float* rstd, const float* w,
+                                     const float* dres, float* dx, void* dx_bf16, float* dw, float* db, float* dcol, int rows, int D,
+                                     int period, unsigned in_thr16, unsigned in_seed, float in_scale, unsigned out_thr16,
+                                     unsigned out_seed, float out_scale, const unsigned* drop_epoch, float* ws, int defer, int post,
+                                     const float* post_rowscale, const int* row_ids, void* stream);
 extern "C" int x2_layernorm_bwd(const void* dy, int dy_is_bf16, const float* x, const float* mean, const float* rstd, const float* w,
                                 const float* dres, float* dx, void* dx_bf16, float* dw, float* db, float* dcol, int rows, int D,
                                 int period, unsigned in_thr16, unsigned in_seed, float in_scale, unsigned out_thr16,
                                 unsigned out_seed, float out_scale, const unsigned* drop_epoch, float* ws, int defer, int post,
                                 const float* post_rowscale, void* stream) {
+  return x2_layernorm_bwd_rows(dy, dy_is_bf16, x, mean, rstd, w, dres, dx, dx_bf16, dw, db, dcol, rows, D, period, in_thr16, in_seed, in_scale,
+                               out_thr16, out_seed, out_scale, drop_epoch, ws, defer, post, post_rowscale, nullptr, stream);
+}
+extern "C" int x2_layernorm_bwd_rows(const void* dy, int dy_is_bf16, const float* x, const float* mean, const float* rstd, const float* w,
+                                     const float* dres, float* dx, void* dx_bf16, float* dw, float* db, float* dcol, int rows, int D,
+                                     int period, unsigned in_thr16, unsigned in_seed, float in_scale, unsigned out_thr16,
+                                     unsigned out_seed, float out_scale, const unsigned* drop_epoch, float* ws, int defer, int post,
+                                     const float* post_rowscale, const int* row_ids, void* stream) {
+  X2_REQUIRE(!row_ids || period == 0, "x2_layernorm_bwd_rows: a row table excludes period=%d", period);
   X2_REQUIRE(rows > 0 && D > 0 && D % 4 == 0 && D <= 256 * LN_MAXV, "x2_layernorm_bwd: rows=%d D=%d", rows, D);
   X2_REQUIRE(dw && db && ws, "x2_layernorm_bwd: dw/db and the workspace ws[ceil(rows/%d)*3*D] are required", LNB_ROWS);
   X2_REQUIRE(post || !(dcol && dres), "x2_layernorm_bwd: dcol sums the LN-input gradient, which excludes dres (post = 0)");
@@ -340,7 +354,7 @@
              "x2_layernorm_bwd: post = 1 (by-products of the final output) takes a bf16 dy, dx_bf16 and dcol, no output mask, period 0");
 #define X2_LNB_T(NV, B) hipLaunchKernelGGL((layernorm_bwd_kernel<NV, B>), dim3((rows + LNB_ROWS - 1) / LNB_ROWS), dim3(256), 9 * D * sizeof(float), \
                      (hipStream_t)stream, dy, x, mean, rstd, w, dres, dx, (bf16_t*)dx_bf16, ws, rows, D, period,                \
-                     DropSpec{in_thr16, in_seed, in_scale}, DropSpec{out_thr16, out_seed, out_scale}, drop_epoch, post_rowscale)
+                     DropSpec{in_thr16, in_seed, in_scale}, DropSpec{out_thr16, out_seed, out_scale}, drop_epoch, post_rowscale, row_ids)
 #define X2_LNB(NV) do { if (post) X2_LNB_T(NV, 2); else if (dy_is_bf16) X2_LNB_T(NV, 1); else X2_LNB_T(NV, 0); } while (0)
   LN_DISPATCH(D, X2_LNB);
   if (!defer) launch_reduce(ws, (rows + LNB_ROWS - 1) / LNB_ROWS, 3, D, dw, db, dcol, (hipStream_t)stream);
diff --git a/x2-vlm_amd/engine.py b/x2-vlm_amd/engine.py
--- a/x2-vlm_amd/engine.py
+++ b/x2-vlm_amd/engine.py
@@ -174,6 +174,7 @@
 SPLIT_DECODER_DGRAD = os.environ.get("X2_SPLIT_DECODER_DGRAD", "1") == "1"
 FUSED_MLM_CE = os.environ.get("X2_FUSED_MLM_CE", "1") == "1"
 FUSE_DGELU_COLSUM = os.environ.get("X2_FUSE_DGELU_COLSUM", "1") == "1"
+PRUNE_LAST_ROWS = os.environ.get("X2_PRUNE_LAST", "1") == "1"
 KEEP_MLM_LOGITS = False
 TIE_WORD_GRAD = False
 _TIED_DWORD = {}
@@ -660,6 +661,9 @@
                 bkv = BANK.vector(p[c + "self.key.bias"], p[c + "self.value.bias"])
                 kv = torch.empty(Bi * T, wkv.shape[0], device=dev, dtype=BF16)
                 kv_ahead[i] = (kv, AUX.launch(lambda kv=kv, wkv=wkv, bkv=bkv: K.gemm_nt(encb, wkv, bias=bkv, out=kv), [encb, wkv, bkv, kv]))
+        rows = meta.get("out_rows")
+        if rows is not None:
+            assert rows.dtype == torch.int32 and rows.dim() == 1 and rows.is_contiguous() and rows.device == dev and meta["hi"] > meta["lo"]
         for i in range(meta["lo"], meta["hi"]):
             b = "layer.%d." % i
             a = b + "attention."
@@ -703,10 +707,14 @@
                 cr = (q2, kv, att2, lse2, s2, m2, r2)
             wi, _ = BANK.linear(p[b + "intermediate.dense.weight"])
             wout, _ = BANK.linear(p[b + "output.dense.weight"])
-            pre = torch.empty(M, wi.shape[0], device=dev, dtype=BF16)
+            rid = rows if i == meta["hi"] - 1 else None
+            if rid is not None:
+                h2, h2b = K.gather_rows(h2, rid, Hd, want_f32=True, want_bf16=True)
+            pre = torch.empty(h2b.shape[0], wi.shape[0], device=dev, dtype=BF16)
             act = K.gemm_nt(h2b, wi, bias=p[b + "intermediate.dense.bias"], aux=pre, act=1)
-            s3 = K.gemm_nt(act, wout, bias=p[b + "output.dense.bias"], resid=h2, out_dtype=F32, drop=dr(meta, i, 4))
-            h3b, h3, m3, r3 = K.layernorm_fwd(s3, p[b + "output.LayerNorm.weight"], p[b + "output.LayerNorm.bias"], eps, want_f32=True)
+            s3 = K.gemm_nt(act, wout, bias=p[b + "output.dense.bias"], resid=h2, out_dtype=F32, drop=dr(meta, i, 4), row_ids=rid)
+            h3b, h3, m3, r3 = K.layernorm_fwd(s3, p[b + "output.LayerNorm.weight"], p[b + "output.LayerNorm.bias"], eps, want_bf16=rid is None,
+                                              want_f32=True)
             saved.append((hb, qkv, att, lse, s1, m1, r1, h1b, cr, h2b, pre, act, s3, m3, r3))
             h, hb = h3, h3b
         AUX.join()
@@ -714,7 +722,7 @@
             _count_call(("bert", id(p["layer.%d.attention.self.query.weight" % i])))
         ctx.meta, ctx.saved, ctx.params, ctx.encb = meta, saved, params, encb
         ctx.dims = (S, L, Hd, H, M, scale, cross, enc.shape if cross else None)
-        return h.view(S, L, Hd)
+        return h.view(S, L, Hd) if rows is None else h
 
     @staticmethod
     def backward(ctx, dh_out):
@@ -724,7 +732,8 @@
         names = bert_layer_param_names(meta["lo"], meta["hi"], meta["fusion_at"], cross)
         p = dict(zip(names, params))
         dev = dh_out.device
-        dh = dh_out.contiguous().view(M, Hd)
+        rows = meta.get("out_rows")
+        dh = dh_out.contiguous().view(M if rows is None else rows.numel(), Hd)
         denc = None
         out = {}
         if cross:
@@ -757,9 +766,10 @@
             G = arenas.pop(i)
             tn, po = [], []
             _begin_layer_backward()
+            rid = rows if i == meta["hi"] - 1 else None
             ds3, ds3b = K.layernorm_bwd(dh, s3, m3, r3, p[b + "output.LayerNorm.weight"], G["output.LayerNorm.weight"],
                                         G["output.LayerNorm.bias"], dcol=G["output.dense.bias"], want_bf16=True,
-                                        drop_out=BertLayersFn._drop(meta, i, 4))
+                                        drop_out=BertLayersFn._drop(meta, i, 4), row_ids=rid)
             _, woutT = BANK.linear(p[b + "output.dense.weight"])
             _, wiT = BANK.linear(p[b + "intermediate.dense.weight"])
             if FUSE_DGELU_COLSUM:
@@ -768,6 +778,8 @@
                 dpre = K.gemm_nt(ds3b, woutT, aux=pre, act=2)
                 K.colsum_bf16(dpre, G["intermediate.dense.bias"])
             dh2 = K.gemm_nt(dpre, wiT, resid=ds3, out_dtype=F32)
+            if rid is not None:
+                dh2 = K.scatter_rows(dh2, rid, M, Hd)
             tn += [(ds3b, act, G["output.dense.weight"]), (dpre, h2b, G["intermediate.dense.weight"])]
             if cr is not None:
                 c = b + "crossattention."
diff --git a/x2-vlm_amd/kernels.py b/x2-vlm_amd/kernels.py
--- a/x2-vlm_amd/kernels.py
+++ b/x2-vlm_amd/kernels.py
@@ -123,7 +123,7 @@
 
 
 def gemm_nt(A, B, *, bias=None, gamma=None, resid=None, aux=None, act=0, out=None, out_dtype=BF16, drop=NO_DROP,
-            rowscale=None, colsum=None):
+            rowscale=None, colsum=None, row_ids=None):
     assert A.dtype == BF16 and B.dtype == BF16 and A.shape[1] == B.shape[1]
     M, K = A.shape
     N = B.shape[0]
@@ -135,10 +135,15 @@
     assert resid is None or (resid.dtype == F32 and resid.shape == (M, N))
     assert aux is None or (aux.dtype == BF16 and aux.shape == (M, N))
     assert rowscale is None or (rowscale.dtype == F32 and rowscale.numel() == M and rowscale.is_contiguous())
+    assert row_ids is None or (row_ids.dtype == torch.int32 and row_ids.numel() == M and row_ids.is_contiguous())
     with _timed(2.0 * M * N * K):
-        call("x2_gemm_nt", ptr(A), ptr(B), ptr(out), M, N, K, _rows(A), _rows(B), _rows(out), ptr(bias), ptr(gamma),
-             ptr(resid), _rows(resid) if resid is not None else 0, ptr(aux), _rows(aux) if aux is not None else 0,
-             act, 1 if out.dtype == F32 else 0, drop[0], drop[1], drop[2], ptr(drop[3]), ptr(rowscale), ptr(colsum))
+        args = (ptr(A), ptr(B), ptr(out), M, N, K, _rows(A), _rows(B), _rows(out), ptr(bias), ptr(gamma),
+                ptr(resid), _rows(resid) if resid is not None else 0, ptr(aux), _rows(aux) if aux is not None else 0,
+                act, 1 if out.dtype == F32 else 0, drop[0], drop[1], drop[2], ptr(drop[3]), ptr(rowscale), ptr(colsum))
+        if row_ids is None:
+            call("x2_gemm_nt", *args)
+        else:
+            call("x2_gemm_nt_rows", *args, ptr(row_ids))
     return out
 
 
@@ -323,7 +328,7 @@
 
 
 def layernorm_bwd(dy, x, mean, rstd, w, dw, db, *, dres=None, dcol=None, period=0, want_f32=True, want_bf16=False, dx=None,
-                  drop_in=NO_DROP, drop_out=NO_DROP, post=None):
+                  drop_in=NO_DROP, drop_out=NO_DROP, post=None, row_ids=None):
     assert dy.dtype in (F32, BF16) and x.dtype == F32 and dy.is_contiguous() and x.is_contiguous()
     D = x.shape[-1]
     R = mean.numel()
@@ -338,9 +343,14 @@
     dxb = torch.empty(x.shape, device=x.device, dtype=BF16) if want_bf16 else None
     nblk = (R + 15) // 16
     ws, defer = _ws_and_defer(x.device, nblk * 3 * D)
-    call("x2_layernorm_bwd", ptr(dy), 1 if dy.dtype == BF16 else 0, ptr(x), ptr(mean), ptr(rstd), ptr(w), ptr(dres), ptr(dx), ptr(dxb), ptr(dw), ptr(db),
-         ptr(dcol), R, D, period, drop_in[0], drop_in[1], drop_in[2], drop_out[0], drop_out[1], drop_out[2],
-         ptr(drop_in[3] if drop_in[3] is not None else drop_out[3]), ptr(ws), defer, 0 if post is None else 1, ptr(prs))
+    assert row_ids is None or (row_ids.dtype == torch.int32 and row_ids.numel() == R and row_ids.is_contiguous() and period == 0)
+    args = (ptr(dy), 1 if dy.dtype == BF16 else 0, ptr(x), ptr(mean), ptr(rstd), ptr(w), ptr(dres), ptr(dx), ptr(dxb), ptr(dw), ptr(db),
+            ptr(dcol), R, D, period, drop_in[0], drop_in[1], drop_in[2], drop_out[0], drop_out[1], drop_out[2],
+            ptr(drop_in[3] if drop_in[3] is not None else drop_out[3]), ptr(ws), defer, 0 if post is None else 1, ptr(prs))
+    if row_ids is None:
+        call("x2_layernorm_bwd", *args)
+    else:
+        call("x2_layernorm_bwd_rows", *args, ptr(row_ids))
     if defer:
         DEFERRED.append((ws, nblk, 3, D, (dw, db, dcol)))
     return dx, dxb
@@ -684,7 +694,7 @@
     return off, order
 
 
-def tail_index(ineg, tneg, text_atts, image_atts, with_match=True):
+def tail_index(ineg, tneg, text_atts, image_atts, with_match=True, masked_pos=None):
     B, L = text_atts.shape
     T = image_atts.shape[1]
     assert text_atts.dtype == torch.int64 and image_atts.dtype == torch.int64 and text_atts.is_contiguous() and image_atts.is_contiguous()
@@ -695,9 +705,16 @@
     kv = torch.empty(R, device=dev, dtype=torch.int32)
     atts = torch.empty(R, L, device=dev, dtype=torch.int64)
     enc = torch.empty(R, T, device=dev, dtype=torch.int64)
-    call("x2_tail_index", ptr(ineg) if with_match else None, ptr(tneg) if with_match else None, ptr(text_atts), ptr(image_atts), B, L, T,
-         1 if with_match else 0, ptr(t_idx), ptr(kv), ptr(atts), ptr(enc))
-    return t_idx, kv, atts, enc
+    args = (ptr(ineg) if with_match else None, ptr(tneg) if with_match else None, ptr(text_atts), ptr(image_atts), B, L, T,
+            1 if with_match else 0, ptr(t_idx), ptr(kv), ptr(atts), ptr(enc))
+    if masked_pos is None:
+        call("x2_tail_index", *args)
+        return t_idx, kv, atts, enc
+    assert masked_pos.dtype == torch.int64 and masked_pos.dim() == 2 and masked_pos.shape[0] == B and masked_pos.is_contiguous()
+    Mm = masked_pos.shape[1]
+    rows = torch.empty((3 * B if with_match else 0) + B * Mm, device=dev, dtype=torch.int32)
+    call("x2_tail_index_rows", *args, ptr(masked_pos), Mm, ptr(rows))
+    return t_idx, kv, atts, enc, rows
 
 
 def droppath_rows(rates, seed, B, T):
diff --git a/x2-vlm_amd/model_pretrain.py b/x2-vlm_amd/model_pretrain.py
--- a/x2-vlm_amd/model_pretrain.py
+++ b/x2-vlm_amd/model_pretrain.py
@@ -1,5 +1,6 @@
 import torch
 
+from . import engine
 from . import kernels as K
 from . import ops
 from .xvlm import XVLMBase
@@ -32,19 +33,27 @@
         text_embeds = both[:B]
         loss_itc = self.get_contrastive_loss(image_feat, text_feat, gathered=gathered)
         ineg, tneg = self.get_hard_negatives(image_feat, text_feat) if ret_match_loss else (None, None)
-        if both.is_cuda:
+        rows = None
+        if both.is_cuda and engine.PRUNE_LAST_ROWS:
+            t_idx, kv, atts, enc_atts, rows = K.tail_index(ineg, tneg, text_atts.contiguous(), image_atts.contiguous(), with_match=ret_match_loss,
+                                                           masked_pos=masked_pos.to(torch.int64).contiguous())
+        elif both.is_cuda:
             t_idx, kv, atts, enc_atts = K.tail_index(ineg, tneg, text_atts.contiguous(), image_atts.contiguous(), with_match=ret_match_loss)
         else:
             ar = torch.arange(B, device=dev, dtype=torch.int32)
             t_idx, kv = (torch.cat([ar, ar, tneg, ar + B]), torch.cat([ar, ineg, ar, ar])) if ret_match_loss else (ar + B, ar)
             atts, enc_atts = torch.cat([text_atts, text_atts])[t_idx.long()], image_atts[kv.long()]
         h0 = ops.gather_rows(both, t_idx)
-        fused = self.get_cross_embeds(image_embeds, enc_atts, text_embeds=h0, text_atts=atts, kv_idx=kv)
+        fused = self.get_cross_embeds(image_embeds, enc_atts, text_embeds=h0, text_atts=atts, kv_idx=kv, out_rows=rows)
+        if rows is not None:
+            cls_rows, mlm_rows = fused.split([3 * B, fused.shape[0] - 3 * B]) if ret_match_loss else (None, fused)
+        else:
+            cls_rows, mlm_rows = (fused[:3 * B, 0, :] if ret_match_loss else None), fused[-B:]
         if ret_match_loss:
-            loss_itm = self._itm_loss(fused[:3 * B, 0, :], B)
+            loss_itm = self._itm_loss(cls_rows, B)
         else:
             loss_itm = torch.tensor(0.0)
-        loss_mlm, self.last_mlm_lse, self.last_mlm_logits = self.text_encoder.mlm_loss_from_hidden(fused[-B:], masked_pos, masked_ids)
+        loss_mlm, self.last_mlm_lse, self.last_mlm_logits = self.text_encoder.mlm_loss_from_hidden(mlm_rows, masked_pos, masked_ids)
         loss = {"loss_itc": loss_itc, "loss_itm": loss_itm, "loss_mlm": loss_mlm}
         self.last = dict(image_embeds=image_embeds.detach(), text_embeds=text_embeds.detach(), image_feat=image_feat.detach(),
                          text_feat=text_feat.detach())
diff --git a/x2-vlm_amd/xbert.py b/x2-vlm_amd/xbert.py
--- a/x2-vlm_amd/xbert.py
+++ b/x2-vlm_amd/xbert.py
@@ -125,7 +125,7 @@
         self.config = config
         self.layer = nn.ModuleList([BertLayer(config, i) for i in range(config.num_hidden_layers)])
 
-    def run(self, hidden, text_atts, enc=None, enc_atts=None, mode="multi_modal", kv_idx=None):
+    def run(self, hidden, text_atts, enc=None, enc_atts=None, mode="multi_modal", kv_idx=None, out_rows=None):
         cfg = self.config
         lo, hi = {"text": (0, cfg.fusion_layer), "fusion": (cfg.fusion_layer, cfg.num_hidden_layers),
                   "multi_modal": (0, cfg.num_hidden_layers)}[mode]
@@ -137,6 +137,8 @@
                     self_mask=None, self_mask2d=None, enc_mask=None, kv_idx=None,
                     seq_off=None, seq_ids=None, drop=drop)
         meta["self_mask"], meta["self_mask2d"] = _text_masks(text_atts)
+        if out_rows is not None:
+            meta["out_rows"] = out_rows
         cross = enc is not None and hi > cfg.fusion_layer
         if cross:
             Bi = enc.shape[0]
@@ -182,7 +184,7 @@
         return self.embeddings.word_embeddings
 
     def forward(self, input_ids=None, attention_mask=None, encoder_embeds=None, encoder_hidden_states=None,
-                encoder_attention_mask=None, return_dict=True, mode="multi_modal", kv_idx=None, position_ids=None, **unused):
+                encoder_attention_mask=None, return_dict=True, mode="multi_modal", kv_idx=None, position_ids=None, out_rows=None, **unused):
         _refuse_unused("BertModel", unused)
         hidden = self.embeddings(input_ids, position_ids) if encoder_embeds is None else encoder_embeds
         S, L = hidden.shape[:2]
@@ -190,7 +192,7 @@
             attention_mask = torch.ones(S, L, device=hidden.device)
         if encoder_hidden_states is not None and encoder_attention_mask is None:
             encoder_attention_mask = torch.ones(S, encoder_hidden_states.shape[1], device=hidden.device)
-        out = self.encoder.run(hidden, attention_mask, encoder_hidden_states, encoder_attention_mask, mode, kv_idx)
+        out = self.encoder.run(hidden, attention_mask, encoder_hidden_states, encoder_attention_mask, mode, kv_idx, out_rows=out_rows)
         return SimpleNamespace(last_hidden_state=out) if return_dict else (out,)
 
 
@@ -226,9 +228,13 @@
         self.cls.predictions.decoder.weight = self.bert.embeddings.word_embeddings.weight
 
     def mlm_loss_from_hidden(self, sequence_output, masked_pos, labels, keep_logits=False):
-        B, L, Hd = sequence_output.shape
-        flat = (torch.arange(B, device=masked_pos.device).unsqueeze(1) * L + masked_pos).reshape(-1)
-        rows = ops.gather_rows(sequence_output.reshape(B * L, Hd), flat)
+        if sequence_output.dim() == 2:
+            assert sequence_output.shape[0] == masked_pos.numel()
+            rows = sequence_output
+        else:
+            B, L, Hd = sequence_output.shape
+            flat = (torch.arange(B, device=masked_pos.device).unsqueeze(1) * L + masked_pos).reshape(-1)
+            rows = ops.gather_rows(sequence_output.reshape(B * L, Hd), flat)
         pr = self.cls.predictions
         return MlmLossFn.apply(rows, labels, self.config.layer_norm_eps, keep_logits, pr.transform.dense.weight, pr.transform.dense.bias,
                                pr.transform.LayerNorm.weight, pr.transform.LayerNorm.bias, pr.bias,
diff --git a/x2-vlm_amd/xvlm.py b/x2-vlm_amd/xvlm.py
--- a/x2-vlm_amd/xvlm.py
+++ b/x2-vlm_amd/xvlm.py
@@ -177,14 +177,14 @@
     def get_text_embeds_12L(self, text_ids, text_atts, **unused):
         return self._bert(text_ids, attention_mask=text_atts).last_hidden_state
 
-    def get_cross_embeds(self, image_embeds, image_atts, text_ids=None, text_embeds=None, text_atts=None, kv_idx=None, **unused):
+    def get_cross_embeds(self, image_embeds, image_atts, text_ids=None, text_embeds=None, text_atts=None, kv_idx=None, out_rows=None, **unused):
         assert text_atts is not None
         if text_embeds is not None:
             return self._bert(encoder_embeds=text_embeds, attention_mask=text_atts, encoder_hidden_states=image_embeds,
-                              encoder_attention_mask=image_atts, mode="fusion", kv_idx=kv_idx).last_hidden_state
+                              encoder_attention_mask=image_atts, mode="fusion", kv_idx=kv_idx, out_rows=out_rows).last_hidden_state
         if text_ids is not None:
             return self._bert(text_ids, attention_mask=text_atts, encoder_hidden_states=image_embeds,
-                              encoder_attention_mask=image_atts, kv_idx=kv_idx).last_hidden_state
+                              encoder_attention_mask=image_atts, kv_idx=kv_idx, out_rows=out_rows).last_hidden_state
         raise ValueError
 
     def get_features(self, image_embeds=None, text_embeds=None):
```

Result: no change. 2927 (median of 6 runs) (+0.5%).
